# broadinstitute/delphy

Hardware: AMD Instinct MI355X
Metric: MCMC moves/sec on 100k-tip SARS-CoV-2 EMAT at 1/2/4/8 MI355X (higher is better)
Workload: dtype f64; 1 GPU; C4: synthetic 100000-tip EMAT, 29903 sites, HKY(kappa=5) + skygrid, 8092 partition parts (199999 nodes), 1000 moves/part/step, move mix 7.5/7.5/15/1/1; parts_per_gpu=8092, parts_requested=8192, max_part_nodes=-1, lds_staging=True, tickets_per_part_and_pass=4, parallelism=parts sharded over 1 GPU(s), one wavefront per part, collectives=none (one rank), emat_build_id=ea4b271524154c43

## Files before the change

### delphy_amd/csrc/emat_debug_host.hpp

```cpp
#ifndef EMAT_DEBUG_HOST_HPP_
#define EMAT_DEBUG_HOST_HPP_

namespace {

emat_status debug_settle(emat_backend* h, bool need_derived) {
  emat_status st = emat_synchronize(h); if (st) return st;
  st = sync_model_to_device(h); if (st) return st;
  st = materialize(h); if (st) return st;
  return need_derived && !h->derived_valid ? launch_recalc(h) : EMAT_OK;
}

}

extern "C" {

emat_status emat_debug_slab_layout(emat_backend* h, int32_t part_id, uint32_t* out8) {
  if (!h || !out8 || part_id < 0 || part_id >= (int)h->parts.size()) return EMAT_ERR_INVALID_ARGUMENT;
  if (!h->have_coal) return fail(h, EMAT_ERR_STATE, "no coalescent parts built");
  const PartHost& ph = h->parts[part_id];
  const int trace_cap = h->cfg.trace_moves > 0 ? h->cfg.trace_moves : 0;
  const uint32_t content = heap_content_bytes(ph.tree);
  const SlabGeo g = slab_geometry(h, ph.tree.num_nodes(), ph.tree.num_muts(), content, (int)ph.coal.k_bar_p.size(), ph.includes_run_root, ph.space_boost, ph.cell_boost);
  out8[0] = (uint32_t)sizeof(SlabHeader); out8[1] = (uint32_t)ph.tree.num_nodes() * (uint32_t)sizeof(NodeRec) + miss_dl_bytes_for((uint32_t)ph.tree.num_nodes()); out8[2] = a16((uint32_t)g.cell_cap * cell_bytes_for(ph.includes_run_root));
  out8[3] = a16((uint32_t)trace_cap * 32u); out8[4] = content; out8[5] = g.heap; out8[6] = g.scratch; out8[7] = (uint32_t)g.cell_cap;
// ... 5 lines not shown
  if (!bind_device(h)) return fail(h, EMAT_ERR_HIP, "hipSetDevice failed");
  if (n == 0) return EMAT_OK;
  DevBuf<double> da, dx, dout;
  HIP_TRY(da.upload(a, (size_t)n)); HIP_TRY(dx.upload(x_or_q, (size_t)n)); HIP_TRY(dout.upload(x_or_q, (size_t)n));
  hipLaunchKernelGGL(k_debug_gamma, dim3((unsigned)((n + 63) / 64)), dim3(64), 0, h->stream, da.p, dx.p, dout.p, n, mode);
  HIP_TRY(hipGetLastError());
  HIP_TRY(hipStreamSynchronize(h->stream));
  HIP_TRY(hipMemcpy(out, dout.p, (size_t)n * sizeof(double), hipMemcpyDeviceToHost));
  return EMAT_OK;
}
emat_status emat_debug_pop(emat_backend* h, const emat_pop_model* pm, int32_t op, int32_t n, const double* a, const double* b, double* out) {
  if (!h || !pm || n < 0 || op < 0 || op > 2 || (n > 0 && (!a || !b || !out))) return EMAT_ERR_INVALID_ARGUMENT;
  if (h->host_only) return no_device(h);
  if (!bind_device(h)) return fail(h, EMAT_ERR_HIP, "hipSetDevice failed");
  if (n == 0) return EMAT_OK;
  HostPopModel hp;
  try { hp = HostPopModel::from_c(*pm); } catch (const std::exception& ex) { return fail(h, EMAT_ERR_INVALID_ARGUMENT, ex.what()); }
  DevBuf<double> dx, dg, da, db, dout;
  HIP_TRY(dx.upload(hp.x.data(), hp.x.size())); HIP_TRY(dg.upload(hp.gamma.data(), hp.gamma.size()));
  HIP_TRY(da.upload(a, (size_t)n)); HIP_TRY(db.upload(b, (size_t)n)); HIP_TRY(dout.alloc((size_t)n));
  PopTable pt{};
  pt.kind = hp.kind; pt.skygrid_type = hp.skygrid_type; pt.skygrid_num_knots = (int)hp.x.size();
  for (int i = 0; i < 4; ++i) pt.p[i] = hp.p[i];
  pt.t_c = hp.t_c; pt.skygrid_x = dx.p; pt.skygrid_gamma = dg.p;
  pt.skygrid_inv_dx = (hp.x.size() >= 2 && hp.x.back() > hp.x.front()) ? (double)(hp.x.size() - 1) / (hp.x.back() - hp.x.front()) : 0.0;
  hipLaunchKernelGGL(k_debug_pop, dim3((unsigned)((n + 63) / 64)), dim3(64), 0, h->stream, pt, (int)op, da.p, db.p, dout.p, (int)n);
  HIP_TRY(hipGetLastError());
  HIP_TRY(hipStreamSynchronize(h->stream));
  HIP_TRY(hipMemcpy(out, dout.p, (size_t)n * sizeof(double), hipMemcpyDeviceToHost));
  return EMAT_OK;
}
emat_status emat_debug_interval_op(emat_backend* h, int32_t op, const int32_t* a, int32_t na, const int32_t* b, int32_t nb, int32_t* out, int32_t* n_out) {
  if (!h || !n_out || na < 0 || nb < 0 || (na > 0 && !a) || (nb > 0 && !b) || !out) return EMAT_ERR_INVALID_ARGUMENT;
  if (h->host_only) return no_device(h);
  if (!bind_device(h)) return fail(h, EMAT_ERR_HIP, "hipSetDevice failed");
  DevBuf<IvRec> dA, dB, dO; DevBuf<int> dn;
  HIP_TRY(dA.upload((const IvRec*)a, (size_t)na)); HIP_TRY(dB.upload((const IvRec*)b, (size_t)(op == 5 ? 0 : nb))); HIP_TRY(dO.alloc(2 * (size_t)(na + nb + 1))); HIP_TRY(dn.alloc(1));
  hipLaunchKernelGGL(k_debug_interval_op, dim3(1), dim3(64), 0, h->stream, (int)op, dA.p, (int)na, dB.p, (int)(op == 5 ? 0 : nb), op == 5 && nb > 0 ? b[0] : 0, dO.p, dn.p);
  HIP_TRY(hipGetLastError());
  HIP_TRY(hipStreamSynchronize(h->stream));
  int cnt = 0;
  HIP_TRY(hipMemcpy(&cnt, dn.p, sizeof(int), hipMemcpyDeviceToHost));
  if (cnt < 0) return fail(h, EMAT_ERR_INVALID_ARGUMENT, "emat_debug_interval_op: unknown op");
  *n_out = cnt;
  if ((op <= 3 || op == 7 || op == 8) && cnt > 0) HIP_TRY(hipMemcpy(out, dO.p, (size_t)cnt * sizeof(IvRec), hipMemcpyDeviceToHost));
  return EMAT_OK;
}
emat_status emat_debug_tree_query(emat_backend* h, int32_t part_id, int32_t op, int32_t n, const int32_t* a, const int32_t* b, int32_t* out) {
  if (!h || n < 0 || (op != 0 && op != 1) || (n > 0 && (!a || !b || !out))) return EMAT_ERR_INVALID_ARGUMENT;
  if (h->host_only) return no_device(h);
  if (!bind_device(h)) return fail(h, EMAT_ERR_HIP, "hipSetDevice failed");
  if (part_id < 0 || part_id >= (int)h->parts.size()) return EMAT_ERR_INVALID_ARGUMENT;
  const int nn = h->parts[part_id].n_nodes;
  for (int i = 0; i < n; ++i) if (a[i] < -1 || a[i] >= nn || b[i] < -1 || b[i] >= nn) return fail(h, EMAT_ERR_INVALID_ARGUMENT, "emat_debug_tree_query: node index out of range");
  if (n == 0) return EMAT_OK;
  emat_status st = debug_settle(h, false); if (st) return st;
  DevBuf<int32_t> da, db, dout;
  HIP_TRY(da.upload(a, (size_t)n)); HIP_TRY(db.upload(b, (size_t)n)); HIP_TRY(dout.alloc((size_t)n));
  KernelArgs ka = make_args(h);
  hipLaunchKernelGGL(k_debug_tree_query, dim3(1), dim3(k_wave), 0, h->stream, ka, (int)part_id, (int)op, da.p, db.p, dout.p, (int)n);
  HIP_TRY(hipGetLastError());
  HIP_TRY(hipStreamSynchronize(h->stream));
  HIP_TRY(hipMemcpy(out, dout.p, (size_t)n * sizeof(int32_t), hipMemcpyDeviceToHost));
  return EMAT_OK;
}
emat_status emat_debug_miss_dl_check(emat_backend* h, int32_t* out_2n) {
  if (!h || !out_2n) return EMAT_ERR_INVALID_ARGUMENT;
  if (h->host_only) return no_device(h);
  if (!bind_device(h)) return fail(h, EMAT_ERR_HIP, "hipSetDevice failed");
  if (h->parts.empty()) return EMAT_OK;
  emat_status st = debug_settle(h, false); if (st) return st;
  DevBuf<int32_t> dout;
  HIP_TRY(dout.alloc(2 * h->parts.size()));
  return run_over_parts(h, k_debug_miss_dl_check, dout.p, out_2n, 2 * h->parts.size(), dout.p);
}
emat_status emat_debug_graft(emat_backend* h, int32_t part_id, int32_t X, double mu_proposal, int32_t mode, int32_t new_sibling, double new_t_P,
                             double* out, int32_t out_cap, int32_t* out_len) {
  if (!h || !out || !out_len || out_cap < 2 || mode < 0 || mode > 3) return EMAT_ERR_INVALID_ARGUMENT;
  if (h->host_only) return no_device(h);
  if (!bind_device(h)) return fail(h, EMAT_ERR_HIP, "hipSetDevice failed");
  if (part_id < 0 || part_id >= (int)h->parts.size()) return EMAT_ERR_INVALID_ARGUMENT;
  const int nn = h->parts[part_id].n_nodes;
  if (X < 0 || X >= nn || (mode == 3 && (new_sibling < 0 || new_sibling >= nn))) return fail(h, EMAT_ERR_INVALID_ARGUMENT, "emat_debug_graft: node index out of range");
  emat_status st = debug_settle(h, true); if (st) return st;
  DevBuf<double> dout; DevBuf<int32_t> dlen;
  HIP_TRY(dout.alloc((size_t)out_cap)); HIP_TRY(dlen.alloc(1));
  KernelArgs ka = make_args(h);
  hipLaunchKernelGGL(k_debug_graft, dim3(1), dim3(k_wave), 0, h->stream, ka, (int)part_id, (int)X, mu_proposal, (int)mode, (int)new_sibling, new_t_P, dout.p, (int)out_cap, dlen.p);
  HIP_TRY(hipGetLastError());
  HIP_TRY(hipStreamSynchronize(h->stream));
  HIP_TRY(hipMemcpy(out_len, dlen.p, sizeof(int32_t), hipMemcpyDeviceToHost));
  HIP_TRY(hipMemcpy(out, dout.p, (size_t)std::min(*out_len, out_cap) * sizeof(double), hipMemcpyDeviceToHost));
  if (mode >= 1) h->device_wrote_slabs();
  if (out[0] != 0.0) return fail(h, EMAT_ERR_INTERNAL, "emat_debug_graft: the device code stopped with part status " + std::to_string((int)out[0]));
  return *out_len > out_cap ? fail(h, EMAT_ERR_CAPACITY, "emat_debug_graft: out_cap too small") : EMAT_OK;
}
emat_status emat_debug_sample_history(emat_backend* h, int32_t part_id, int32_t n, const int32_t* branch, const double* t_end, const uint8_t* start_seq, double T, double mu,
                                      int32_t* counts, double* muts, int32_t muts_cap, int32_t* num_muts) {
  if (!h || n < 0 || !branch || !t_end || !start_seq || !counts || !muts || muts_cap < 0 || !num_muts) return EMAT_ERR_INVALID_ARGUMENT;
  if (h->host_only) return no_device(h);
  if (!bind_device(h)) return fail(h, EMAT_ERR_HIP, "hipSetDevice failed");
  if (part_id < 0 || part_id >= (int)h->parts.size()) return EMAT_ERR_INVALID_ARGUMENT;
  const int nn = h->parts[part_id].n_nodes;
  for (int i = 0; i < n; ++i) if (branch[i] < 0 || branch[i] >= nn) return fail(h, EMAT_ERR_INVALID_ARGUMENT, "emat_debug_sample_history: node index out of range");
  emat_status st = debug_settle(h, true); if (st) return st;
  DevBuf<int32_t> db, dc, ds; DevBuf<double> dt, dm; DevBuf<uint8_t> dseq;
  HIP_TRY(db.upload(branch, (size_t)std::max(n, 1))); HIP_TRY(dt.upload(t_end, (size_t)std::max(n, 1))); HIP_TRY(dseq.upload(start_seq, (size_t)h->cfg.num_sites));
  HIP_TRY(dc.alloc((size_t)std::max(n, 1))); HIP_TRY(dm.alloc((size_t)std::max(muts_cap, 1) * 4)); HIP_TRY(ds.alloc(2));
  KernelArgs ka = make_args(h);
  hipLaunchKernelGGL(k_debug_sample_history, dim3(1), dim3(k_wave), 0, h->stream, ka, (int)part_id, (int)n, db.p, dt.p, dseq.p, T, mu, dc.p, dm.p, (int)muts_cap, ds.p);
  HIP_TRY(hipGetLastError());
  HIP_TRY(hipStreamSynchronize(h->stream));
  int32_t status[2];
  HIP_TRY(hipMemcpy(status, ds.p, sizeof status, hipMemcpyDeviceToHost));
  h->device_wrote_slabs();
  if (status[0] != 0) return fail(h, EMAT_ERR_INTERNAL, "emat_debug_sample_history: the device code stopped with part status " + std::to_string(status[0]));
  *num_muts = status[1];
  if (n > 0) HIP_TRY(hipMemcpy(counts, dc.p, (size_t)n * sizeof(int32_t), hipMemcpyDeviceToHost));
  if (status[1] > 0) HIP_TRY(hipMemcpy(muts, dm.p, (size_t)std::min(status[1], muts_cap) * 4 * sizeof(double), hipMemcpyDeviceToHost));
  return status[1] > muts_cap ? fail(h, EMAT_ERR_CAPACITY, "emat_debug_sample_history: muts_cap too small") : EMAT_OK;
}
emat_status emat_debug_edit(emat_backend* h, int32_t part_id, int32_t X, int32_t n_ops, const int32_t* op_kind, const int32_t* op_node, const double* op_t) {
  if (!h || n_ops < 0 || (n_ops > 0 && (!op_kind || !op_node || !op_t))) return EMAT_ERR_INVALID_ARGUMENT;
  if (h->host_only) return no_device(h);
  if (!bind_device(h)) return fail(h, EMAT_ERR_HIP, "hipSetDevice failed");
  if (part_id < 0 || part_id >= (int)h->parts.size()) return EMAT_ERR_INVALID_ARGUMENT;
  const int nn = h->parts[part_id].n_nodes;
  if (X < 0 || X >= nn) return fail(h, EMAT_ERR_INVALID_ARGUMENT, "emat_debug_edit: node index out of range");
  for (int i = 0; i < n_ops; ++i) if (op_kind[i] < 0 || op_kind[i] > 3 || (op_kind[i] == 3 && (op_node[i] < 0 || op_node[i] >= nn))) return fail(h, EMAT_ERR_INVALID_ARGUMENT, "emat_debug_edit: bad step");
  emat_status st = debug_settle(h, true); if (st) return st;
  DevBuf<int32_t> dk, dn, ds; DevBuf<double> dt;
  HIP_TRY(dk.upload(op_kind, (size_t)std::max(n_ops, 1))); HIP_TRY(dn.upload(op_node, (size_t)std::max(n_ops, 1))); HIP_TRY(dt.upload(op_t, (size_t)std::max(n_ops, 1))); HIP_TRY(ds.alloc(1));
  KernelArgs ka = make_args(h);
  hipLaunchKernelGGL(k_debug_edit, dim3(1), dim3(k_wave), 0, h->stream, ka, (int)part_id, (int)X, (int)n_ops, dk.p, dn.p, dt.p, ds.p);
  HIP_TRY(hipGetLastError());
  HIP_TRY(hipStreamSynchronize(h->stream));
  int32_t status = 0;
  HIP_TRY(hipMemcpy(&status, ds.p, sizeof status, hipMemcpyDeviceToHost));
  h->device_wrote_slabs();
  if (status != 0) return fail(h, EMAT_ERR_INTERNAL, "emat_debug_edit: the device code stopped with part status " + std::to_string(status));
  return EMAT_OK;
}
emat_status emat_debug_variant_counts(emat_backend* h, int32_t* out3) {
  if (!h || !out3 || h->host_only) return EMAT_ERR_INVALID_ARGUMENT;
  emat_status st = sync_model_to_device(h); if (st) return st;
  st = materialize(h); if (st) return st;
  st = pull_from_device(h); if (st) return st;
  out3[0] = out3[1] = out3[2] = 0;
  const uint32_t area = h->class_lds[h->num_classes - 1];
  const bool tables = h->num_partitions <= k_max_lds_partitions;
  for (auto& ph : h->parts) {
    const SlabHeader* H = (const SlabHeader*)(h->h_slabs.data() + ph.slab_off);
    const bool can = tables && area != 0 && H->off_nodes == (uint32_t)sizeof(SlabHeader);
    if (can && (H->heap_end <= area || H->heap_top + k_lds_heap_room <= area)) ++out3[0]; else if (can && H->heap_begin <= area) ++out3[1]; else ++out3[2];
  }
  return EMAT_OK;
}
emat_status emat_debug_arena_sites(emat_backend* h, uint64_t* out_4096) {
  if (!h || !out_4096 || h->host_only) return EMAT_ERR_INVALID_ARGUMENT;
#ifdef EMAT_PROFILE_PHASES
  HIP_TRY(hipStreamSynchronize(h->stream));
  HIP_TRY(hipMemcpyFromSymbol(out_4096, HIP_SYMBOL(::emat::g_arena_site_bytes), sizeof(unsigned long long) * 4096));
  return EMAT_OK;
#else
  return fail(h, EMAT_ERR_STATE, "built without -DEMAT_PROFILE_PHASES");
#endif
}
emat_status emat_debug_fn_ticks(emat_backend* h, uint64_t* out_12288) {
  if (!h || !out_12288 || h->host_only) return EMAT_ERR_INVALID_ARGUMENT;
#if defined(EMAT_PROFILE_PHASES) || defined(EMAT_COUNT_CALLS)
  HIP_TRY(hipStreamSynchronize(h->stream));
  std::vector<unsigned long long> z((size_t)12288 * ::emat::k_fn_replicas, 0);
  HIP_TRY(hipMemcpyFromSymbol(z.data(), HIP_SYMBOL(::emat::g_fn_ticks), sizeof(unsigned long long) * z.size()));
  for (int k = 0; k < 12288; ++k) { unsigned long long sum = 0; for (int r = 0; r < ::emat::k_fn_replicas; ++r) sum += z[(size_t)r * 12288 + k]; out_12288[k] = sum; }
  std::fill(z.begin(), z.end(), 0ull);
  HIP_TRY(hipMemcpyToSymbol(HIP_SYMBOL(::emat::g_fn_ticks), z.data(), sizeof(unsigned long long) * z.size()));
  const unsigned min_lists = h->cfg_fn_min_lists;
  HIP_TRY(hipMemcpyToSymbol(HIP_SYMBOL(::emat::g_fn_min_list_bytes), &min_lists, sizeof(min_lists)));
  return EMAT_OK;
#else
  return fail(h, EMAT_ERR_STATE, "built without -DEMAT_PROFILE_PHASES");
#endif
}
emat_status emat_debug_arena_bytes(emat_backend* h, int32_t* out_n) {
  if (!h || !out_n || h->host_only) return EMAT_ERR_INVALID_ARGUMENT;
  emat_status st = sync_model_to_device(h); if (st) return st;
  st = materialize(h); if (st) return st;
  st = pull_from_device(h); if (st) return st;
  const uint32_t area = h->class_lds[h->num_classes - 1];
  for (size_t p = 0; p < h->parts.size(); ++p) {
    const SlabHeader* H = (const SlabHeader*)(h->h_slabs.data() + h->parts[p].slab_off);
    if (h->class_of[p] != h->num_classes - 1) { out_n[p] = -1; continue; }
    const uint32_t want = (H->heap_top + k_lds_heap_room + 15u) & ~15u;
    uint32_t used;
    if (H->heap_end <= area) used = std::min(H->heap_end, want); else if (want <= area) used = want; else used = (H->heap_begin + 15u) & ~15u;
    out_n[p] = used <= area ? (int32_t)(area - ((used + 15u) & ~15u)) : 0;
  }
  return EMAT_OK;
}
emat_status emat_debug_part_ticks(emat_backend* h, int64_t* out_2n) {
  if (!h || !out_2n || h->host_only || !h->slabs_on_device) return EMAT_ERR_INVALID_ARGUMENT;
  if (!bind_device(h)) return fail(h, EMAT_ERR_HIP, "hipSetDevice failed");
  { emat_status js = wait_for_side_classes(h); if (js) return js; }
  HIP_TRY(hipStreamSynchronize(h->stream));
  HIP_TRY(hipMemcpy(out_2n, h->d_part_ticks.p, sizeof(int64_t) * 2 * h->parts.size(), hipMemcpyDeviceToHost));
  return EMAT_OK;
}
emat_status emat_debug_ticket_ticks(emat_backend* h, int64_t* out_16n) {
  if (!h || !out_16n || h->host_only || !h->slabs_on_device) return EMAT_ERR_INVALID_ARGUMENT;
  if (!bind_device(h)) return fail(h, EMAT_ERR_HIP, "hipSetDevice failed");
  { emat_status js = wait_for_side_classes(h); if (js) return js; }
  HIP_TRY(hipStreamSynchronize(h->stream));
  HIP_TRY(hipMemcpy(out_16n, h->d_part_ticks.p + 2 * h->parts.size(), sizeof(int64_t) * 2 * k_ticket_log * h->parts.size(), hipMemcpyDeviceToHost));
  return EMAT_OK;
}
emat_status emat_debug_phase_ticks(emat_backend* h, int32_t part_id, int64_t* out16) {
  if (!h || !out16 || part_id < 0 || part_id >= (int)h->parts.size()) return EMAT_ERR_INVALID_ARGUMENT;
  emat_status st = pull_from_device(h); if (st) return st;
  const SlabHeader* H = (const SlabHeader*)(h->h_slabs.data() + h->parts[part_id].slab_off);
#ifdef EMAT_PROFILE_PHASES
  for (int i = 0; i < 16; ++i) out16[i] = H->phase_ticks[i];
  if (h->cfg_phase_extra) for (int i = 0; i < 16; ++i) out16[i] = ((const int64_t*)H->reserved)[i];
#else
  (void)H; for (int i = 0; i < 16; ++i) out16[i] = 0;
#endif
  return EMAT_OK;
}

}

#endif
```

### delphy_amd/csrc/emat_device_core.hpp

```cpp
#ifndef EMAT_DEV_NS
#error "define EMAT_DEV_NS and EMAT_VARIANT_LDS before including the device headers"
#endif

#include <hip/hip_runtime.h>
#include <cfloat>
#include <cstdint>

#include "emat_slab.hpp"
#include "emat_reform_pure.hpp"
#include "emat_rng_pos.hpp"
#include "emat_gamma_pure.hpp"

#ifndef EMAT_DEVICE_COMMON_ONCE_
#define EMAT_DEVICE_COMMON_ONCE_
namespace emat {
extern __shared__ __attribute__((aligned(16))) uint8_t emat_lds[];
constexpr uint32_t k_lds_tables_bytes = k_max_lds_partitions * (1 + 4 + 16) * 8;
constexpr uint32_t k_lds_ctx_bytes = 288;
#ifndef EMAT_RNG_BLOCKS
#define EMAT_RNG_BLOCKS 32
#endif
constexpr uint32_t k_rng_blocks = EMAT_RNG_BLOCKS;
static_assert(k_rng_blocks == 0 || (k_rng_blocks <= 64 && (k_rng_blocks & (k_rng_blocks - 1)) == 0), "one block per lane, a power of two");
constexpr uint32_t k_lds_rng_bytes = k_rng_blocks * 16;
constexpr uint32_t k_lds_static_bytes = k_lds_tables_bytes + k_lds_ctx_bytes + k_lds_rng_bytes + k_max_lds_partitions * 16 * 8;
__shared__ __attribute__((aligned(16))) uint8_t emat_lds_tables[k_lds_tables_bytes];
__shared__ __attribute__((aligned(16))) uint8_t emat_lds_ctx[k_lds_ctx_bytes];
__shared__ __attribute__((aligned(16))) uint32_t emat_lds_rng[k_rng_blocks ? k_rng_blocks * 4 : 4];
constexpr uint32_t k_lds_logq_bytes = k_max_lds_partitions * 16 * 8;
__shared__ __attribute__((aligned(16))) double emat_lds_logq[k_max_lds_partitions * 16];
__shared__ __attribute__((aligned(16))) uint8_t emat_lds_hdr[sizeof(SlabHeader)];
constexpr uint32_t k_lds_dyn_base = k_lds_tables_bytes + k_lds_ctx_bytes + (k_rng_blocks ? k_rng_blocks * 16 : 16) + k_lds_logq_bytes + (uint32_t)sizeof(SlabHeader);
}
#if defined(EMAT_PROFILE_PHASES) || defined(EMAT_COUNT_CALLS)
#define EMAT_DYN_LDS ::emat::emat_lds
#else
#define EMAT_DYN_LDS ((uint8_t*)(__attribute__((address_space(3))) uint8_t*)(uintptr_t)::emat::k_lds_dyn_base)
#endif
#define EMAT_D static __device__ inline
#define EMAT_DN static __device__ __noinline__
#define EMAT_DF static __device__ __forceinline__
#define EMAT_NOTAIL __attribute__((disable_tail_calls))
#ifdef EMAT_COUNT_CALLS
#define EMAT_CALLED(file_id) do { if (threadIdx.x == 0) atomicAdd(&::emat::g_fn_ticks[(blockIdx.x & 63) * (3 * 2048) + (file_id) * 2048 + (__LINE__ & 2047)][1], 1ull); } while (0)
#endif
#endif

namespace emat {
namespace EMAT_DEV_NS {

constexpr double k_neg_dbl_max = -1.7976931348623157e308;
constexpr double k_inf = __builtin_huge_val();
constexpr int k_no_node = -1;

#ifndef EMAT_CONST_AS
#define EMAT_CONST_AS __attribute__((address_space(4)))
#endif
template <class T> EMAT_DF const EMAT_CONST_AS T* uniform_const_ptr(const T* p) {
  const uint64_t a = (uint64_t)p;
  const uint32_t lo = __builtin_amdgcn_readfirstlane((uint32_t)a), hi = __builtin_amdgcn_readfirstlane((uint32_t)(a >> 32));
  return (const EMAT_CONST_AS T*)(((uint64_t)hi << 32) | lo);
}

EMAT_DF uint32_t uniform_u32(uint32_t v) { return __builtin_amdgcn_readfirstlane(v); }
EMAT_DF bool uniform_flag(bool b) { return __builtin_amdgcn_ballot_w64(b) != 0ull; }

struct Ctx {
  uint8_t* S;
  uint8_t* G;
  SlabHeader* H;
  NodeRec* N;
  int L;
  uint32_t heap_limit;
  const __attribute__((address_space(1))) uint8_t* ref;
  const __attribute__((address_space(1))) uint8_t* part;
  const __attribute__((address_space(1))) double* nu;
  const __attribute__((address_space(1))) double* cumQ;
  const double* mu;
  const double* pi;
  const double* q;
  const PopTable* pop;
  double t_max_tip;
  bool only_displacing_inner_nodes;
  bool topology_moves_enabled;
  bool includes_run_root;
  bool uniform_sites;
  bool have_logq;
  uint8_t phase, svc;
  uint64_t rng_key;
  uint32_t rng_pos;
  uint32_t mv_rng_pos;
  uint64_t rng_base;
  uint64_t rng_spare;
  uint8_t* frame;
  double mu_prop;
  uint8_t* A;
  uint32_t a_top, a_end;
  uint32_t sc_top;
  bool failed;
  int64_t bytes;
  int64_t bytes_w;
  double tr_log_mh; int32_t tr_node; int16_t tr_kind, tr_acc;
  int64_t moves_left;
  double mix_total;
  const double* sh_ktw; const double* sh_tsop; const int32_t* sh_nact;
};

static_assert(sizeof(Ctx) + 16 <= k_lds_ctx_bytes, "context outgrew its LDS slot (the last 16 bytes are the kernel's flag word)");
#if EMAT_VARIANT_LDS
EMAT_DF uint8_t* slab_at(const Ctx&, uint32_t off) { return EMAT_DYN_LDS + (off - (uint32_t)sizeof(SlabHeader)); }
EMAT_DF SlabHeader* hdr_of(const Ctx&) { return (SlabHeader*)emat_lds_hdr; }
EMAT_DF NodeRec* nodes_of(const Ctx&) { return (NodeRec*)EMAT_DYN_LDS; }
EMAT_DF const double* mu_of(const Ctx&) { return (const double*)emat_lds_tables; }
EMAT_DF const double* pi_of(const Ctx&) { return (const double*)emat_lds_tables + k_max_lds_partitions; }
EMAT_DF const double* q_of(const Ctx&) { return (const double*)emat_lds_tables + k_max_lds_partitions * 5; }
#if EMAT_VARIANT_LDS == 2
EMAT_DF uint8_t* heap_at(const Ctx& c, uint32_t off) { return c.G + off; }
#else
EMAT_DF uint8_t* heap_at(const Ctx& c, uint32_t off) { return slab_at(c, off); }
#endif
#else
EMAT_DF uint8_t* heap_at(const Ctx& c, uint32_t off) { return c.S + off; }
EMAT_DF uint8_t* slab_at(const Ctx& c, uint32_t off) { return c.S + off; }
EMAT_DF SlabHeader* hdr_of(const Ctx& c) { return c.H; }
EMAT_DF NodeRec* nodes_of(const Ctx& c) { return c.N; }
EMAT_DF const double* mu_of(const Ctx& c) { return c.mu; }
EMAT_DF const double* pi_of(const Ctx& c) { return c.pi; }
EMAT_DF const double* q_of(const Ctx& c) { return c.q; }
#endif

EMAT_D void fail_at(Ctx& c, int status, int line) {
  if (!c.failed) { c.failed = true; if (hdr_of(c)->status == 0) { hdr_of(c)->status = status; hdr_of(c)->fail_line = line; } }
}
#ifndef EMAT_FAIL
#define EMAT_FAIL(c, st) fail_at((c), (st), __LINE__)
#define EMAT_CHECK(c, cond) do { if (!(cond)) fail_at((c), ::emat::k_part_internal, __LINE__); } while (0)
#ifdef EMAT_PROFILE_PHASES
#define EMAT_SITE(line, hbm, v) atomicAdd(&::emat::g_arena_site_bytes[(line) & 2047][(hbm) ? 1 : 0], (unsigned long long)(v))
#define EMAT_COUNT(c, k, v) (((int64_t*)hdr_of(c)->reserved)[k] += (int64_t)(v))
#define EMAT_PHASE_BEGIN() long long _ph_t0 = clock64()
#define EMAT_PHASE(c, k) do { long long _t = clock64(); hdr_of(c)->phase_ticks[k] += _t - _ph_t0; _ph_t0 = _t; } while (0)
#define EMAT_TIMED(file_id) ::emat::FnTimer _fn_timer((file_id) * 2048 + (__LINE__ & 2047))
#define EMAT_TIMED_BLOCK(file_id, name) ::emat::FnTimer name((file_id) * 2048 + (__LINE__ & 2047))
#define EMAT_TIMED_END(name) name.stop()
#else
#define EMAT_TIMED(file_id) do {} while (0)
#define EMAT_TIMED_BLOCK(file_id, name) do {} while (0)
#define EMAT_TIMED_END(name) do {} while (0)
#define EMAT_SITE(line, hbm, v) do {} while (0)
#define EMAT_COUNT(c, k, v) do {} while (0)
#define EMAT_PHASE_BEGIN() do {} while (0)
#define EMAT_PHASE(c, k) do {} while (0)
#endif
#endif

EMAT_DN double m_log(double x) { return ::log(x); }
EMAT_DN double m_exp(double x) { return ::exp(x); }
EMAT_DN double m_log1p(double x) { return ::log1p(x); }
EMAT_DN double m_expm1(double x) { return ::expm1(x); }
EMAT_D void philox4x32_10(uint64_t ctr, uint64_t key, uint32_t out[4]) {
  uint32_t c0 = (uint32_t)ctr, c1 = (uint32_t)(ctr >> 32), c2 = 0, c3 = 0;
  uint32_t k0 = (uint32_t)key, k1 = (uint32_t)(key >> 32);
#pragma unroll
  for (int r = 0; r < 10; ++r) {
    const uint32_t M0 = 0xD2511F53u, M1 = 0xCD9E8D57u;
    uint32_t hi0 = __umulhi(M0, c0), lo0 = M0 * c0;
    uint32_t hi1 = __umulhi(M1, c2), lo1 = M1 * c2;
    uint32_t n0 = hi1 ^ c1 ^ k0, n1 = lo1, n2 = hi0 ^ c3 ^ k1, n3 = lo0;
    c0 = n0; c1 = n1; c2 = n2; c3 = n3;
    k0 += 0x9E3779B9u; k1 += 0xBB67AE85u;
  }
  out[0] = c0; out[1] = c1; out[2] = c2; out[3] = c3;
}
constexpr uint32_t k_rng_fold_at = 1u << 30;
EMAT_DN uint64_t rng_next64_computed(Ctx& c) {
  const RngPos at = rng_pos_folded(c.rng_base, c.rng_pos, k_rng_blocks, k_rng_fold_at);
  if (at.pos != c.rng_pos) c.rng_base = at.base;
  c.rng_pos = at.pos + 1u;
  if (at.pos & 1u) return c.rng_spare;
  uint32_t w[4];
  philox4x32_10(rng_pos_block(at.base, at.pos), c.rng_key, w);
  c.rng_spare = (uint64_t)w[2] | ((uint64_t)w[3] << 32);
  return (uint64_t)w[0] | ((uint64_t)w[1] << 32);
}
EMAT_DF uint64_t rng_buffer_word(uint32_t i) { return ((const uint64_t*)emat_lds_rng)[i]; }
EMAT_D uint64_t rng_next64(Ctx& c) {
  const uint32_t pos = c.rng_pos;
  if (rng_pos_in_buffer(pos, k_rng_blocks)) { c.rng_pos = pos + 1u; return rng_buffer_word(pos); }
  return rng_next64_computed(c);
}
EMAT_D void rng_fill(Ctx& c, int lane) {
  if (k_rng_blocks == 0) return;
  const uint32_t pos = c.rng_pos;
  const RngPos to = rng_pos_after_fill(c.rng_base, pos);
  if (lane == 0 && (pos & 1u) == 0 && rng_pos_in_buffer(rng_pos_spare_word(pos), k_rng_blocks)) c.rng_spare = rng_buffer_word(rng_pos_spare_word(pos));
  if (lane < (int)k_rng_blocks) { uint32_t w[4]; philox4x32_10(to.base + (uint64_t)lane, c.rng_key, w); *(uint4*)&emat_lds_rng[(uint32_t)lane * 4u] = make_uint4(w[0], w[1], w[2], w[3]); }
  if (lane == 0) { c.rng_base = to.base; c.rng_pos = to.pos; }
}
#ifndef EMAT_RNG_MARGIN
#define EMAT_RNG_MARGIN 8
#endif
EMAT_D bool rng_wants_fill(const Ctx& c) { return rng_pos_wants_fill(c.rng_pos, k_rng_blocks, (uint32_t)EMAT_RNG_MARGIN); }
EMAT_D void rng_rewind_to_move_start(Ctx& c) {
  const uint32_t pos = c.mv_rng_pos;
  c.rng_pos = pos;
  if ((pos & 1u) != 0 && !rng_pos_in_buffer(pos, k_rng_blocks)) { uint32_t w[4]; philox4x32_10(rng_pos_block(c.rng_base, pos), c.rng_key, w); c.rng_spare = (uint64_t)w[2] | ((uint64_t)w[3] << 32); }
}
EMAT_D void rng_enter_leg(Ctx& c, const SlabHeader& h) {
  const RngPos at = rng_pos_enter(h.rng_counter, h.rng_has_spare, k_rng_blocks);
  c.rng_key = h.rng_key; c.rng_base = at.base; c.rng_pos = at.pos; c.mv_rng_pos = at.pos; c.rng_spare = h.rng_spare;
}
EMAT_D void rng_leave_leg(const Ctx& c, SlabHeader& h) {
  const uint32_t pos = c.rng_pos, sw = rng_pos_spare_word(pos);
  h.rng_counter = rng_pos_counter(c.rng_base, pos); h.rng_has_spare = rng_pos_has_spare(pos);
  h.rng_spare = rng_pos_in_buffer(sw, k_rng_blocks) ? rng_buffer_word(sw) : c.rng_spare;
}
using ::emat::to_co; using ::emat::to_oo; using ::emat::to_oc;
EMAT_D double u01_co(Ctx& c) { return to_co(rng_next64(c)); }
EMAT_D double u01_oo(Ctx& c) { return to_oo(rng_next64(c)); }
EMAT_D double u01_oc(Ctx& c) { return to_oc(rng_next64(c)); }
EMAT_D double uniform_co(Ctx& c, double lo, double hi) { return lo + (hi - lo) * u01_co(c); }
EMAT_D double uniform_oc(Ctx& c, double lo, double hi) { return lo + (hi - lo) * u01_oc(c); }
EMAT_D int uniform_int(Ctx& c, int n) { return (int)__umul64hi(rng_next64(c), (uint64_t)n); }
EMAT_D double gaussian(Ctx& c, double mean, double sigma) {
  uint64_t a = rng_next64(c), b = rng_next64(c);
  double u1 = to_oc(a), u2 = to_co(b);
  double r = sqrt(-2.0 * m_log(u1));
  return mean + sigma * (r * cos(6.283185307179586476925 * u2));
}
EMAT_D double exponential(Ctx& c, double rate) { return -m_log(u01_oc(c)) / rate; }
EMAT_D int poisson(Ctx& c, double lambda) {
  double u = u01_co(c);
  double p = m_exp(-lambda), F = p;
  int k = 0;
  while (u >= F && k < 100000) { ++k; p *= lambda / k; F += p; }
  return k;
}

struct ByteCount { int all = 0, written = 0; };
EMAT_DF void count_bytes(Ctx& c, const ByteCount& n) { c.bytes += n.all; if (n.written != 0) c.bytes_w += n.written; }

template <class T> struct SVec { T* p; int n; int cap; };
struct ScMark { uint32_t a, g; };
EMAT_D ScMark sc_mark(const Ctx& c) { ScMark m; m.a = c.a_top; m.g = c.sc_top; return m; }
EMAT_D void sc_release(Ctx& c, ScMark m) { c.a_top = m.a; c.sc_top = m.g; }
EMAT_D void sc_reset(Ctx& c) { c.a_top = 0; c.sc_top = hdr_of(c)->scratch_begin; }
EMAT_D bool sc_in_lds(const Ctx& c, const void* p) { return c.A != nullptr && (const uint8_t*)p >= c.A && (const uint8_t*)p < c.A + c.a_end; }
EMAT_D uint8_t* sc_alloc(Ctx& c, uint32_t bytes, int line = __builtin_LINE()) {
  uint32_t b = (bytes + 15u) & ~15u;
  if (c.a_top + b <= c.a_end) { uint8_t* p = c.A + c.a_top; c.a_top += b; EMAT_COUNT(c, 9, b); EMAT_SITE(line, 0, b); return p; }
  if (c.sc_top + b > hdr_of(c)->scratch_end) { EMAT_FAIL(c, k_part_overflow); return c.G + hdr_of(c)->scratch_begin; }
  EMAT_COUNT(c, 8, b); EMAT_SITE(line, 1, b);
  uint8_t* p = c.G + c.sc_top;
  c.sc_top += b;
  return p;
}
template <class T> EMAT_D SVec<T> sc_vec(Ctx& c, int cap, int line = __builtin_LINE()) {
  SVec<T> v; v.n = 0;
  uint32_t bytes = (uint32_t)cap * (uint32_t)sizeof(T);
  uint32_t b = (bytes + 15u) & ~15u;
  if (cap >= 0 && c.a_top + b <= c.a_end) { v.p = (T*)(c.A + c.a_top); v.cap = cap; c.a_top += b; EMAT_COUNT(c, 9, b); EMAT_SITE(line, 0, b); return v; }
  if (cap < 0 || c.sc_top + b > hdr_of(c)->scratch_end) { EMAT_FAIL(c, k_part_overflow); v.p = (T*)(c.G + hdr_of(c)->scratch_begin); v.cap = 0; return v; }
  EMAT_COUNT(c, 8, b); EMAT_SITE(line, 1, b);
  v.p = (T*)(c.G + c.sc_top); v.cap = cap; c.sc_top += b;
  return v;
}
template <class T> EMAT_DF void push(Ctx& c, SVec<T>& v, const T& x, int line = __builtin_LINE()) { if (v.n < v.cap) v.p[v.n++] = x; else fail_at(c, k_part_overflow, line); }
template <class T> EMAT_D SVec<T> sc_open(Ctx& c, int max_elems, int min_lds_elems) {
  SVec<T> v; v.n = 0;
  uint32_t a0 = (c.a_top + 15u) & ~15u;
  int room_a = c.a_end > a0 ? (int)((c.a_end - a0) / sizeof(T)) : 0;
  if (room_a >= min_lds_elems) { v.p = (T*)(c.A + a0); v.cap = room_a < max_elems ? room_a : max_elems; c.a_top = c.a_end; return v; }
  uint32_t g0 = (c.sc_top + 15u) & ~15u;
  int room_g = hdr_of(c)->scratch_end > g0 ? (int)((hdr_of(c)->scratch_end - g0) / sizeof(T)) : 0;
  v.p = (T*)(c.G + g0); v.cap = room_g < max_elems ? room_g : max_elems; c.sc_top = hdr_of(c)->scratch_end;
  if (v.cap <= 0) { v.cap = 0; EMAT_FAIL(c, k_part_overflow); }
  return v;
}
template <class T> EMAT_DF bool sc_open_migrate(Ctx& c, SVec<T>& v, int max_elems) {
  if (!sc_in_lds(c, v.p)) return false;
  uint32_t g0 = (c.sc_top + 15u) & ~15u;
  int room_g = hdr_of(c)->scratch_end > g0 ? (int)((hdr_of(c)->scratch_end - g0) / sizeof(T)) : 0;
// ... 771 lines not shown
```

### delphy_amd/csrc/emat_device_moves.hpp

```cpp

#include "emat_device_spr.hpp"

namespace emat {
namespace EMAT_DEV_NS {

#ifndef EMAT_HOT_BYTES
#define EMAT_HOT_BYTES 1536
#endif
enum { k_inner_node_displace = 0, k_tip_displace = 1, k_branch_reform = 2, k_subtree_slide = 3, k_spr1 = 4 };

EMAT_D void trace_nothing(Ctx& c, int kind) { c.tr_node = -1; c.tr_kind = (int16_t)kind; c.tr_acc = -1; }
EMAT_D void begin_move(Ctx& c, int kind) { hdr_of(c)->proposed[kind]++; trace_nothing(c, kind); }
EMAT_D void note_move(Ctx& c, double log_mh, bool acc, int kind) { c.tr_log_mh = log_mh; c.tr_acc = acc ? 1 : 0; if (acc) hdr_of(c)->accepted[kind]++; }
EMAT_D bool mh_accept(Ctx& c, double log_mh) { return log_mh >= 0.0 || uniform_co(c, 0.0, 1.0) < m_exp(log_mh); }

EMAT_DF double bounded_exponential(Ctx& c, double lambda, double a, double b) {
  double u = u01_oo(c);
  double ltr = lambda * (b - a);
  double x;
  if (lambda == 0.0) x = a + u * (b - a);
  else if (lambda > 0 && ltr > 100) x = b + m_log(u) / lambda;
  else if (lambda < 0 && ltr < -100) x = a + m_log(u) / lambda;
  else x = a + m_log1p(u * (m_exp(ltr) - 1)) / lambda;
  return x < a ? a : (b < x ? b : x);
}
EMAT_DF int pick_random_node(Ctx& c) { return uniform_int(c, hdr_of(c)->n_nodes); }

struct CoreFrame {
  int X, new_branch, P, old_S;
  double new_t, alpha_ratio, old_t_P, d_prior, log_mh;
  Graft old_graft, new_graft;
};
#ifndef EMAT_CF
#define EMAT_CF(c) (*(CoreFrame*)(c).frame)
#endif
EMAT_NOTAIL EMAT_DN void spr_move_core(Ctx& c, int X, int new_branch, double new_t, double alpha_ratio) { EMAT_TIMED(2);
  if (X == hdr_of(c)->root) return;
  if (!c.includes_run_root) if (nodes_of(c)[X].parent == hdr_of(c)->root || new_branch == hdr_of(c)->root) return;
  {
    const double t_X = nodes_of(c)[X].t;
    const int P = nodes_of(c)[X].parent;
    const double new_t_P = new_t;
    if (new_t_P == t_X || new_t_P == nodes_of(c)[new_branch].t || (P != hdr_of(c)->root && new_t_P == nodes_of(c)[nodes_of(c)[P].parent].t)) return;
    if (coal_needs_cells(c, new_t_P)) { stop_for_cells(c, c.tr_kind); return; }
    CoreFrame* f = (CoreFrame*)sc_alloc(c, (uint32_t)sizeof(CoreFrame));
    if (c.failed) return;
    c.frame = (uint8_t*)f;
    f->X = X; f->new_branch = new_branch; f->P = P; f->old_S = sibling_of(c, P, X);
    f->new_t = new_t; f->alpha_ratio = alpha_ratio; f->old_t_P = nodes_of(c)[P].t;
  }
  c.mu_prop = nodes_of(c)[hdr_of(c)->root].lambda / (c.L - nodes_of(c)[hdr_of(c)->root].n_missing);
  EMAT_PHASE_BEGIN();
  analyze_graft(c, EMAT_CF(c).X, EMAT_CF(c).old_graft);
  peel_graft(c, EMAT_CF(c).old_graft);
  EMAT_PHASE(c, 0);
  spr_move_topology(c, EMAT_CF(c).X, EMAT_CF(c).new_branch, EMAT_CF(c).new_t);
  EMAT_PHASE(c, 1);
  propose_new_graft(c, EMAT_CF(c).X, EMAT_CF(c).new_graft);
  EMAT_PHASE(c, 2);
  if (c.failed) return;
  EMAT_CF(c).d_prior = coal_delta_displace_coalescence(c, EMAT_CF(c).old_t_P, EMAT_CF(c).new_t);
  {
    const CoreFrame& f = EMAT_CF(c);
    EMAT_CF(c).log_mh = (f.new_graft.delta_log_G - f.new_graft.log_alpha_mut) - (f.old_graft.delta_log_G - f.old_graft.log_alpha_mut) + m_log(f.alpha_ratio) + f.d_prior;
  }
  if (c.failed) return;
  const bool acc = mh_accept(c, EMAT_CF(c).log_mh);
  if (c.tr_kind == k_subtree_slide) note_move(c, EMAT_CF(c).log_mh, acc, k_subtree_slide);
  if (acc) {
    apply_graft(c, EMAT_CF(c).new_graft);
    hdr_of(c)->log_G -= EMAT_CF(c).old_graft.delta_log_G; hdr_of(c)->log_G += EMAT_CF(c).new_graft.delta_log_G;
    hdr_of(c)->log_aug_prior += EMAT_CF(c).d_prior;
    coal_coalescence_displaced(c, EMAT_CF(c).old_t_P, EMAT_CF(c).new_t);
  } else {
    spr_move_topology(c, EMAT_CF(c).X, EMAT_CF(c).old_S, EMAT_CF(c).old_t_P);
    apply_graft(c, EMAT_CF(c).old_graft);
  }
  EMAT_PHASE(c, 4);
}

template <bool kRoot> EMAT_DF void inner_node_displace_body(Ctx& c, ByteCount& n) {
  begin_move(c, k_inner_node_displace);
  int node;
  { EMAT_TIMED(2);
    int guard = 0; do { node = pick_random_node(c); } while (is_tip(c, node) && guard++ < (1 << 26)); }
  c.tr_node = node;
  const int root = hdr_of(c)->root;
  if (!kRoot && node == root) return;
  const NodeRec nd = nodes_of(c)[node];
  double t_min = -k_inf;
  if (!kRoot || node != root) {
    t_min = nodes_of(c)[nd.parent].t;
    const MutRec* m = muts_of(c, node);
    for (int i = 0; i < (int)nd.muts.cnt; ++i) t_min = t_min > m[i].t ? t_min : m[i].t;
  }
  double t_max = k_inf;
  const int ch[2] = {nd.child0, nd.child1};
  const double lambda_at_node = nd.lambda;
  double d_logG_dt = 0.0;
  if (!kRoot || node != root) d_logG_dt += -lambda_at_node;
  for (int k = 0; k < 2; ++k) {
    const int cc = ch[k];
    t_max = t_max < nodes_of(c)[cc].t ? t_max : nodes_of(c)[cc].t;
    const MutRec* m = muts_of(c, cc);
    const int nm = nmuts(c, cc);
    for (int i = 0; i < nm; ++i) t_max = t_max < m[i].t ? t_max : m[i].t;
    n.all += 64 + 16 * nm + 24 * (int)nodes_of(c)[cc].miss.cnt;
  }
  { EMAT_TIMED(2);
  for (int k = 0; k < 2; ++k) {
    double lambda_just_below = lambda_at_node + delta_lambda_across_node_missations(c, ch[k]);
    d_logG_dt -= -lambda_just_below;
  } }
  n.all += 2 * 64 + 16 * (int)nd.muts.cnt;
  const double old_t = nd.t;
  double log_alpha_ratio = 0.0, new_t = old_t;
  if (kRoot && node == root) {
    double tree_span = c.t_max_tip - t_max;
    EMAT_CHECK(c, tree_span >= 0.0);
    double ds = (1 / nd.lambda) / 2;
    double delta_scale;
    if (tree_span < ds) delta_scale = tree_span; else delta_scale = ds;
    new_t = old_t + gaussian(c, 0.0, delta_scale);
    if (new_t < t_min || new_t > t_max) return;
    log_alpha_ratio = 0.0;
  } else {
    EMAT_TIMED(2);
    new_t = bounded_exponential(c, d_logG_dt, t_min, t_max);
    log_alpha_ratio = d_logG_dt * (new_t - old_t);
  }
  if (new_t == t_min || new_t == t_max) return;
  if (kRoot) { if (coal_needs_cells(c, new_t)) { stop_for_cells(c, k_inner_node_displace); return; } }
  double delta_log_G = d_logG_dt * (new_t - old_t);
  double delta_log_prior = coal_delta_displace_coalescence<kRoot>(c, old_t, new_t, n);
  if (c.failed) return;
  double log_mh = delta_log_G + delta_log_prior - log_alpha_ratio;
  bool acc;
  { EMAT_TIMED(2);
  acc = mh_accept(c, log_mh);
  note_move(c, log_mh, acc, k_inner_node_displace); }
  if (acc) {
    EMAT_TIMED(2);
    coal_coalescence_displaced<kRoot>(c, old_t, new_t, n);
    nodes_of(c)[node].t = new_t;
    hdr_of(c)->log_G += d_logG_dt * (new_t - old_t);
    hdr_of(c)->log_aug_prior += delta_log_prior;
  }
}
template <bool kRoot> EMAT_NOTAIL EMAT_DN void inner_node_displace_move(Ctx& c) { EMAT_TIMED(2); ByteCount n; inner_node_displace_body<kRoot>(c, n); count_bytes(c, n); }

template <bool kRoot> EMAT_DF void tip_displace_body(Ctx& c, ByteCount& n) {
  begin_move(c, k_tip_displace);
  int node;
  { int guard = 0; do { node = pick_random_node(c); } while (!is_tip(c, node) && guard++ < (1 << 26)); }
  c.tr_node = node;
  const NodeRec nd = nodes_of(c)[node];
  if (nd.t_min == nd.t_max) return;
  double t_min;
  if ((double)nd.t_min < nodes_of(c)[nd.parent].t) t_min = nodes_of(c)[nd.parent].t; else t_min = (double)nd.t_min;
  const MutRec* m = muts_of(c, node);
  for (int i = 0; i < (int)nd.muts.cnt; ++i) t_min = t_min > m[i].t ? t_min : m[i].t;
  const double t_max = (double)nd.t_max;
  const double d_logG_dt = -nd.lambda;
  const double old_t = nd.t;
  n.all += 2 * 64 + 16 * (int)nd.muts.cnt;
  double new_t = bounded_exponential(c, d_logG_dt, t_min, t_max);
  double log_alpha_ratio = d_logG_dt * (new_t - old_t);
  if (new_t == t_min || new_t == t_max) return;
  double delta_log_G = d_logG_dt * (new_t - old_t);
  double delta_log_prior = coal_delta_displace_tip<kRoot>(c, old_t, new_t, n);
  if (c.failed) return;
  double log_mh = delta_log_G + delta_log_prior - log_alpha_ratio;
  bool acc = mh_accept(c, log_mh);
  note_move(c, log_mh, acc, k_tip_displace);
  if (acc) {
    coal_tip_displaced<kRoot>(c, old_t, new_t, n);
    nodes_of(c)[node].t = new_t;
    hdr_of(c)->log_G += d_logG_dt * (new_t - old_t);
    hdr_of(c)->log_aug_prior += delta_log_prior;
  }
}
template <bool kRoot> EMAT_NOTAIL EMAT_DN void tip_displace_move(Ctx& c) { EMAT_TIMED(2); ByteCount n; tip_displace_body<kRoot>(c, n); count_bytes(c, n); }

EMAT_DF SVec<MutRec> randomize_branch_mutation_times(Ctx& c, int X) { EMAT_TIMED(2);
  const int n = nmuts(c, X);
  SVec<MutRec> out = sc_vec<MutRec>(c, n);
  if (c.failed) return out;
  const MutRec* old = muts_of(c, X);
  if (X == hdr_of(c)->root) { for (int i = 0; i < n; ++i) push(c, out, old[i]); return out; }
  const double t_X = nodes_of(c)[X].t, t_P = nodes_of(c)[nodes_of(c)[X].parent].t;
  bool complicated = false;
  for (int i = 0; i < n && !complicated; ++i) for (int j = i + 1; j < n; ++j) if (old[i].site == old[j].site) { complicated = true; break; }
  if (!complicated) {
    for (int i = 0; i < n; ++i) { MutRec r = make_mut(old[i].from, old[i].site, old[i].to, uniform_oc(c, t_P, t_X)); r.pad = (uint16_t)i; push(c, out, r); }
  } else {
    int prev_site = -1;
    while (true) {
      int l = 0x7fffffff;
      for (int i = 0; i < n; ++i) if (old[i].site > prev_site && old[i].site < l) l = old[i].site;
      if (l == 0x7fffffff) break;
      prev_site = l;
      int first = out.n, k = 0;
      for (int i = 0; i < n; ++i) if (old[i].site == l) { MutRec r = make_mut(old[i].from, old[i].site, old[i].to, uniform_oc(c, t_P, t_X)); r.pad = (uint16_t)i; push(c, out, r); ++k; }
      for (int a = first + 1; a < first + k && a < out.n; ++a) { double x = out.p[a].t; int b = a - 1; while (b >= first && out.p[b].t > x) { out.p[b + 1].t = out.p[b].t; --b; } out.p[b + 1].t = x; }
    }
  }
  sort_muts(out.p, out.n);
  return out;
}

struct ReformFactors { double* A; double* B; };
EMAT_DF bool mut_factors(const Ctx& c, int pa, double nu, int from, int to, double& A, double& B) {
  const double mn = mu_of(c)[pa] * nu;
  const double* q = q_of(c) + pa * 16;
  A = mn * (-q[from * 5] - -q[to * 5]);
  if (c.have_logq && nu == 1.0) { B = emat_lds_logq[pa * 16 + from * 4 + to]; return false; }
// ... 54 lines not shown
  hdr_of(c)->log_G += delta_log_G;
  return 16 * N;
}
#ifndef EMAT_REFORM_SMALL_MAX
#define EMAT_REFORM_SMALL_MAX 4
#endif
template <bool kRoot> EMAT_DF void branch_reform_body(Ctx& c, ByteCount& n_bytes) {
  begin_move(c, k_branch_reform);
  if (hdr_of(c)->n_nodes < 3) return;
  const int X = pick_random_node(c);
  c.tr_node = X;
  if (X == hdr_of(c)->root) return;
  const int P = nodes_of(c)[X].parent;
  const int S = sibling_of(c, P, X);
  const double t_X = nodes_of(c)[X].t, t_P = nodes_of(c)[P].t;
  if (kRoot) { if (P == hdr_of(c)->root) { spr_move_core(c, X, S, t_P, 1.0); if (c.failed) return; } }
  const double lam = nodes_of(c)[X].lambda;
  const int n = nmuts(c, X);
  if (n == 0) {
    const double g = -lam * (t_X - t_P), delta_log_G = g - g;
    n_bytes.all += 2 * 64;
    const bool acc = mh_accept(c, delta_log_G);
    note_move(c, delta_log_G, acc, k_branch_reform);
    if (acc) hdr_of(c)->log_G += delta_log_G;
    return;
  }
  if (n <= EMAT_REFORM_SMALL_MAX) {
    int stored = -1;
    switch (n) {
#if EMAT_REFORM_SMALL_MAX >= 1
      case 1: stored = branch_reform_small<1>(c, X, lam, t_X, t_P); break;
#endif
#if EMAT_REFORM_SMALL_MAX >= 2
      case 2: stored = branch_reform_small<2>(c, X, lam, t_X, t_P); break;
#endif
#if EMAT_REFORM_SMALL_MAX >= 3
      case 3: stored = branch_reform_small<3>(c, X, lam, t_X, t_P); break;
#endif
#if EMAT_REFORM_SMALL_MAX >= 4
      case 4: stored = branch_reform_small<4>(c, X, lam, t_X, t_P); break;
#endif
      default: break;
    }
    if (stored >= 0) { n_bytes.all += 2 * 64 + 2 * 16 * n + stored; n_bytes.written += stored; return; }
  }
  const ReformFactors f = reform_factors(c, muts_of(c, X), n);
  SVec<MutRec> nm = randomize_branch_mutation_times(c, X);
  if (c.failed) return;
  double g_new = -lam * (t_X - t_P), g_old = g_new;
  { const MutRec* m = nm.p; for (int i = nm.n - 1; i >= 0; --i) { const int j = (int)m[i].pad; g_new -= f.A[j] * (m[i].t - t_P); g_new += f.B[j]; } }
  { const MutRec* m = muts_of(c, X); for (int i = n - 1; i >= 0; --i) { g_old -= f.A[i] * (m[i].t - t_P); g_old += f.B[i]; } }
  const double delta_log_G = g_new - g_old;
  n_bytes.all += 2 * 64 + 2 * 16 * nm.n;
  double log_mh = delta_log_G;
  bool acc = mh_accept(c, log_mh);
  note_move(c, log_mh, acc, k_branch_reform);
  if (acc) {
    for (int i = 0; i < nm.n; ++i) nm.p[i].pad = 0;
    list_assign<MutRec>(c, nodes_of(c)[X].muts, nm.p, nm.n); hdr_of(c)->log_G += delta_log_G; n_bytes.all += 16 * nm.n; n_bytes.written += 16 * nm.n;
  }
}
template <bool kRoot> EMAT_NOTAIL EMAT_DN void branch_reform_move(Ctx& c) { EMAT_TIMED(2); ByteCount n; branch_reform_body<kRoot>(c, n); count_bytes(c, n); }

EMAT_DN SVec<int> enumerate_descendant_branches_straddling(Ctx& c, int P, double t, int X) {
  SVec<int> out; out.n = 0;
  ScSpan span = sc_span(c, 512);
  out.p = (int*)span.lo; out.cap = 0;
  int* stack_base = (int*)span.hi;
  int sp = 0;
  auto room = [&](int er, int es) -> bool {
    if (span.lo + (size_t)(out.n + er) * 4 + 16 <= span.hi - (size_t)(sp + es) * 4) return true;
    if (!span.lds) return false;
    ScSpan big = sc_span_hbm(c);
    if (big.lo + (size_t)(out.n + er) * 4 + 16 > big.hi - (size_t)(sp + es) * 4) return false;
    int* no = (int*)big.lo; int* nb = (int*)big.hi;
    for (int i = 0; i < out.n; ++i) no[i] = out.p[i];
    for (int i = 1; i <= sp; ++i) nb[-i] = stack_base[-i];
    span = big; out.p = no; stack_base = nb;
    return true;
  };
  if (!room(0, 1)) { EMAT_FAIL(c, k_part_overflow); return out; }
  stack_base[-(++sp)] = P;
  while (sp > 0 && !c.failed) {
    int n = stack_base[-sp]; --sp;
    if (n == X) continue;
    if (t <= nodes_of(c)[n].t) { if (!room(1, 0)) { EMAT_FAIL(c, k_part_overflow); break; } out.p[out.n++] = n; }
    else if (!is_tip(c, n)) {
      if (!room(0, 2)) { EMAT_FAIL(c, k_part_overflow); break; }
      stack_base[-(++sp)] = nodes_of(c)[n].child1;
      stack_base[-(++sp)] = nodes_of(c)[n].child0;
    }
  }
  out.cap = out.n;
  sc_span_commit(c, span, (uint32_t)out.n * 4u);
  return out;
}

EMAT_NOTAIL EMAT_DN void subtree_slide_move(Ctx& c) { EMAT_TIMED(2);
  begin_move(c, k_subtree_slide);
  if (hdr_of(c)->n_nodes < 2) return;
  const int X = pick_random_node(c);
  c.tr_node = X;
  const int root = hdr_of(c)->root;
  if (X == root) return;
  const int P = nodes_of(c)[X].parent, S = sibling_of(c, P, X);
  double t_early = (P == root) ? (nodes_of(c)[X].t < nodes_of(c)[S].t ? nodes_of(c)[X].t : nodes_of(c)[S].t) : nodes_of(c)[root].t;
  if (P == root) { if (nodes_of(c)[S].t < nodes_of(c)[X].t) t_early = nodes_of(c)[S].t; else t_early = nodes_of(c)[X].t; }
  double tree_span = c.t_max_tip - t_early;
  EMAT_CHECK(c, tree_span >= 0.0);
  double ds = (1 / nodes_of(c)[X].lambda) / 2;
  double delta_scale = tree_span < ds ? tree_span : ds;
  double delta_t = gaussian(c, 0.0, delta_scale);
  const double old_P_t = nodes_of(c)[P].t, new_P_t = old_P_t + delta_t;
  if (delta_t < 0.0) {
    if (P != root && new_P_t < nodes_of(c)[nodes_of(c)[P].parent].t) {
      int GG = nodes_of(c)[P].parent, SS = P;
      while (new_P_t < nodes_of(c)[GG].t) { SS = GG; GG = nodes_of(c)[GG].parent; if (GG == k_no_node) break; }
      SVec<int> branches = enumerate_descendant_branches_straddling(c, SS, old_P_t, X);
      if (c.failed) return;
      double a_o2n = 1.0, a_n2o = 1.0 / (double)branches.n;
      spr_move_core(c, X, SS, new_P_t, a_n2o / a_o2n);
    } else spr_move_core(c, X, S, new_P_t, 1.0);
  } else {
    if (new_P_t > nodes_of(c)[X].t) return;
    if (new_P_t > nodes_of(c)[S].t) {
      SVec<int> branches = enumerate_descendant_branches_straddling(c, P, new_P_t, X);
      if (c.failed) return;
      if (branches.n == 0) return;
      int bi = uniform_int(c, branches.n);
      int SS = branches.p[bi];
      double a_o2n = 1.0 / (double)branches.n, a_n2o = 1.0;
      spr_move_core(c, X, SS, new_P_t, a_n2o / a_o2n);
    } else spr_move_core(c, X, S, new_P_t, 1.0);
  }
}

EMAT_D void spr1_park(Ctx& c, int phase) { c.phase = (uint8_t)phase; c.svc = 1; }
EMAT_NOTAIL EMAT_DN void spr1_move_begin(Ctx& c) { EMAT_TIMED(2);
  begin_move(c, k_spr1);
  c.phase = 0;
  if (hdr_of(c)->n_nodes < 2) return;
  const double chooser = uniform_co(c, 0.0, 1.0);
  const int limit = chooser < 0.01 ? 0x7fffffff : 1;
  const int root0 = hdr_of(c)->root;
  c.mu_prop = nodes_of(c)[root0].lambda / (c.L - nodes_of(c)[root0].n_missing);
  int X;
  { int guard = 0; do { X = pick_random_node(c); } while (hdr_of(c)->root == X && guard++ < (1 << 26)); }
  c.tr_node = X;
  if (nodes_of(c)[X].lambda == 0.0) return;
  const int P = nodes_of(c)[X].parent;
  const bool pruning_changes_root = P == hdr_of(c)->root;
  if (pruning_changes_root && !c.includes_run_root) return;
  EMAT_PHASE_BEGIN();
  Spr1Frame* frp = (Spr1Frame*)sc_alloc(c, (uint32_t)sizeof(Spr1Frame));
  if (c.failed) return;
  Spr1Frame& fr = *frp;
  c.frame = (uint8_t*)frp;
  fr.X = X; fr.t_X = nodes_of(c)[X].t; fr.P = P; fr.old_t_P = nodes_of(c)[P].t; fr.old_S = sibling_of(c, P, X); fr.old_G = nodes_of(c)[P].parent;
  fr.limit = limit; fr.f = 0.8 ; fr.t_max_tip = c.t_max_tip; fr.can_change_root = c.includes_run_root;
  {
    const uint32_t a0 = (c.a_top + 15u) & ~15u, free_b = c.a_end > a0 ? c.a_end - a0 : 0u;
    uint32_t hot_b = EMAT_HOT_BYTES;
    if (free_b / 2 > hot_b) hot_b = (free_b / 2 < 32768u ? free_b / 2 : 32768u) & ~15u;
    fr.hot = (limit == 1) ? sc_reserve_hot(c, hot_b) : HotBlock{nullptr, 0};
  }
  analyze_graft(c, X, fr.old_graft);
  peel_graft(c, fr.old_graft);
  EMAT_PHASE(c, 5);
  if (c.failed) return;
  fr.old_min_muts = count_min_mutations(c, fr.old_graft);
  int extra = 4;
  if (limit != 1) { extra = 8; for (int n = 0; n < hdr_of(c)->n_nodes; ++n) if (c.includes_run_root || n != hdr_of(c)->root) extra += nmuts(c, n); }
  fr.extra = extra;
  fr.deltas = summarize_closed_mutations(c, fr.old_graft, extra);
  fr.missing_at_X = reconstruct_missing_sites_at(c, X);
  fr.n_missing_at_X = iv_num_sites(fr.missing_at_X.p, fr.missing_at_X.n);
  fr.lambda_X = nodes_of(c)[X].lambda;
  fr.init_branch = fr.old_S;
  if (c.failed) return;
  spr1_park(c, 1);
}
EMAT_NOTAIL EMAT_DN void spr1_move_propose(Ctx& c) { EMAT_TIMED(2);
  Spr1Frame& fr = *(Spr1Frame*)c.frame;
  c.phase = 0;
  if (c.failed) return;
  EMAT_PHASE_BEGIN();
  const Study& pre = fr.study;
  const int X = fr.X, P = fr.P;
  int new_region; double new_t_P;
  { EMAT_TIMED(2);
  new_region = study_pick_nexus_region(c, pre);
  new_t_P = study_pick_time_in_region(c, pre, new_region);
  fr.log_alpha_o2n = study_log_alpha_in_region(c, pre, new_region, new_t_P); }
  const int new_S = pre.regions.p[new_region].branch;
  EMAT_CHECK(c, new_S != P);
  fr.pre_new_region_min_muts = pre.regions.p[new_region].min_muts;
  fr.new_S = new_S; fr.new_t_P = new_t_P;
  const double t_new_S = nodes_of(c)[new_S].t;
  int new_G = nodes_of(c)[new_S].parent;
  if (new_G == P) new_G = fr.old_G;
  const double t_new_G = (new_G == k_no_node) ? k_neg_dbl_max : nodes_of(c)[new_G].t;
  if (c.failed) return;
  EMAT_PHASE(c, 7);
  if (new_t_P == fr.t_X || new_t_P == t_new_S || new_t_P == t_new_G) { apply_graft(c, fr.old_graft); return; }
  if (coal_needs_cells(c, new_t_P)) { apply_graft(c, fr.old_graft); if (!c.failed) stop_for_cells(c, k_spr1); return; }
  spr_move_topology(c, X, new_S, new_t_P);
  EMAT_PHASE(c, 8);
  propose_new_graft(c, X, fr.new_graft);
  EMAT_PHASE(c, 9);
  if (c.failed) return;
  EMAT_CHECK(c, nodes_of(c)[X].parent == P);
  fr.new_min_muts = count_min_mutations(c, fr.new_graft);
  fr.deltas = summarize_closed_mutations(c, fr.new_graft, fr.extra);
  fr.init_branch = new_S;
  if (c.failed) return;
  spr1_park(c, 2);
}
EMAT_NOTAIL EMAT_DN void spr1_move_finish(Ctx& c) { EMAT_TIMED(2);
  Spr1Frame& fr = *(Spr1Frame*)c.frame;
  c.phase = 0;
  if (c.failed) return;
  EMAT_PHASE_BEGIN();
  const Study& post = fr.study;
  const int X = fr.X;
  const int old_region = study_find_region(post, fr.old_S, fr.old_t_P);
  EMAT_CHECK(c, old_region != -1);
  if (c.failed) return;
  const double log_alpha_n2o = study_log_alpha_in_region(c, post, old_region, fr.old_t_P);
  EMAT_CHECK(c, fr.new_min_muts == fr.pre_new_region_min_muts);
  EMAT_CHECK(c, fr.old_min_muts == post.regions.p[old_region].min_muts);
  EMAT_PHASE(c, 11);
  const double d_prior = coal_delta_displace_coalescence(c, fr.old_t_P, fr.new_t_P);
  if (c.failed) return;
  const double log_mh = (fr.new_graft.delta_log_G - fr.new_graft.log_alpha_mut) - (fr.old_graft.delta_log_G - fr.old_graft.log_alpha_mut)
      + log_alpha_n2o - fr.log_alpha_o2n + d_prior;
  const bool acc = mh_accept(c, log_mh);
  note_move(c, log_mh, acc, k_spr1);
  if (acc) {
    apply_graft(c, fr.new_graft);
    hdr_of(c)->log_G -= fr.old_graft.delta_log_G; hdr_of(c)->log_G += fr.new_graft.delta_log_G;
    hdr_of(c)->log_aug_prior += d_prior;
    coal_coalescence_displaced(c, fr.old_t_P, fr.new_t_P);
  } else {
    EMAT_TIMED(2);
    spr_move_topology(c, X, fr.old_S, fr.old_t_P);
    apply_graft(c, fr.old_graft);
  }
  EMAT_PHASE(c, 12);
}

EMAT_DN bool compact_heap(Ctx& c) {
  uint32_t live = 0;
  const int n = hdr_of(c)->n_nodes;
  for (int i = 0; i < n; ++i) {
    live += (((uint32_t)nodes_of(c)[i].muts.cnt * 16u) + 15u) & ~15u;
    live += (((uint32_t)nodes_of(c)[i].miss.cnt * 8u) + 15u) & ~15u;
    live += (((uint32_t)nodes_of(c)[i].mfs.cnt * 8u) + 15u) & ~15u;
  }
  if (live > hdr_of(c)->scratch_end - hdr_of(c)->scratch_begin) return false;
  uint8_t* stage = c.G + hdr_of(c)->scratch_begin;
  uint32_t w = 0;
  for (int i = 0; i < n; ++i) {
    ListRef* refs[3] = {&nodes_of(c)[i].muts, &nodes_of(c)[i].miss, &nodes_of(c)[i].mfs};
    const uint32_t es[3] = {16u, 8u, 8u};
    for (int k = 0; k < 3; ++k) {
      uint32_t bytes = (uint32_t)refs[k]->cnt * es[k];
      const uint64_t* src = (const uint64_t*)heap_at(c, refs[k]->off); uint64_t* dst = (uint64_t*)(stage + w);
      for (uint32_t q = 0; q < bytes / 8; ++q) dst[q] = src[q];
      w += (bytes + 15u) & ~15u;
    }
  }
  uint32_t top = hdr_of(c)->heap_begin, r = 0;
  for (int i = 0; i < n; ++i) {
    ListRef* refs[3] = {&nodes_of(c)[i].muts, &nodes_of(c)[i].miss, &nodes_of(c)[i].mfs};
    const uint32_t es[3] = {16u, 8u, 8u};
    for (int k = 0; k < 3; ++k) {
      uint32_t bytes = (uint32_t)refs[k]->cnt * es[k], padded = (bytes + 15u) & ~15u;
      const uint64_t* src = (const uint64_t*)(stage + r); uint64_t* dst = (uint64_t*)heap_at(c, top);
      for (uint32_t q = 0; q < bytes / 8; ++q) dst[q] = src[q];
      refs[k]->off = top; refs[k]->cap = list_cap_for(padded, es[k]);
      top += padded; r += padded;
    }
  }
  hdr_of(c)->heap_top = top;
  return true;
}

EMAT_D uint32_t heap_reserve(const Ctx& c) {
  const uint32_t heap_size = hdr_of(c)->heap_end - hdr_of(c)->heap_begin;
  uint32_t reserve = heap_size / 4 > 1024u ? heap_size / 4 : 1024u;
  if (reserve > heap_size / 2) reserve = heap_size / 2;
  return reserve;
}
EMAT_D void begin_leg(Ctx& c) {
  c.heap_limit = hdr_of(c)->heap_end - heap_reserve(c);
  double total_weight = 15.0 + 15.0;
  if (c.topology_moves_enabled) total_weight += 1.0 + 1.0;
  c.mix_total = total_weight;
}
EMAT_DN bool make_heap_room(Ctx& c) {
  const uint32_t reserve = heap_reserve(c), free_b = hdr_of(c)->heap_end - hdr_of(c)->heap_top;
  if (free_b < reserve) {
    if (!compact_heap(c) || hdr_of(c)->heap_end - hdr_of(c)->heap_top < reserve) { if (hdr_of(c)->status == 0) hdr_of(c)->status = k_part_need_space; return false; }
  }
  return true;
}

template <bool kRoot> EMAT_NOTAIL EMAT_D bool mcmc_sub_iteration(Ctx& c) {
#ifdef EMAT_PROFILE_PHASES
  const long long _mv0 = clock64();
#endif
  const uint32_t phase = uniform_u32(c.phase);
  if (phase == 1) spr1_move_propose(c);
  else if (phase == 2) spr1_move_finish(c);
  else {
  if (uniform_flag(hdr_of(c)->heap_top > c.heap_limit)) { if (!uniform_flag(make_heap_room(c))) return false; }
  sc_reset(c);
  if (kRoot) c.mv_rng_pos = c.rng_pos;
  if (c.only_displacing_inner_nodes) inner_node_displace_move<kRoot>(c);
  else {
    double r = uniform_co(c, 0.0, c.mix_total);
    if (r < 7.5) inner_node_displace_move<kRoot>(c);
    else if (r < 15.0) tip_displace_move<kRoot>(c);
    else if (r < 30.0) branch_reform_move<kRoot>(c);
    else if (c.topology_moves_enabled) { if (r < 31.0) subtree_slide_move(c); else spr1_move_begin(c); }
    else trace_nothing(c, -1);
  }
  }
#ifdef EMAT_PROFILE_PHASES
  { const long long _dt = clock64() - _mv0; hdr_of(c)->phase_ticks[(c.tr_kind >= 3) ? 15 : 14] += _dt; if (c.tr_kind == 0) EMAT_COUNT(c, 10, _dt); else if (c.tr_kind == 1) EMAT_COUNT(c, 15, _dt); }
#endif
  if (uniform_u32(c.svc) != 0 && !uniform_flag(c.failed)) return true;
  c.phase = 0; c.svc = 0;
  if (uniform_flag(hdr_of(c)->status == k_part_need_cells)) return false;
  if (uniform_flag(hdr_of(c)->trace_len < hdr_of(c)->trace_cap)) {
    double* tr = (double*)slab_at(c, hdr_of(c)->off_trace) + 4 * hdr_of(c)->trace_len;
    const bool noted = c.tr_acc >= 0;
    tr[0] = (double)c.tr_kind; tr[1] = (double)c.tr_node; tr[2] = noted ? (double)c.tr_acc : 0.0; tr[3] = noted ? c.tr_log_mh : __builtin_nan("");
    hdr_of(c)->trace_len++;
  }
  hdr_of(c)->moves_done++;
  return !uniform_flag(c.failed);
}

template <bool kRoot> EMAT_NOTAIL EMAT_DN void run_chain(Ctx& c) {
  c.svc = 0;
  for (;;) {
    if (uniform_u32(c.phase) == 0) {
      if (uniform_flag(c.moves_left <= 0)) return;
      if (uniform_flag(rng_wants_fill(c))) { c.svc = 2; return; }
      c.moves_left -= 1;
    }
    if (!uniform_flag(mcmc_sub_iteration<kRoot>(c))) { c.moves_left = 0; c.phase = 0; c.svc = 0; return; }
    if (uniform_u32(c.svc) != 0) return;
  }
}
EMAT_DF void run_chain_loop(Ctx& c) { if (c.includes_run_root) run_chain<true>(c); else run_chain<false>(c); }

EMAT_DN double calc_log_root_prior(Ctx& c, const int32_t* ref_freqs, int P) {
  const int root = hdr_of(c)->root;
  double result = 0.0;
  for (int p = 0; p < P; ++p) {
    for (int a = 0; a < 4; ++a) {
      int f = ref_freqs[p * 4 + a];
      const MutRec* m = muts_of(c, root);
      for (int i = 0; i < nmuts(c, root); ++i) if (site_part(c, m[i].site) == p) { if (m[i].from == a) --f; if (m[i].to == a) ++f; }
      const IvRec* iv = miss_of(c, root);
      for (int i = 0; i < (int)nodes_of(c)[root].miss.cnt; ++i) for (int l = iv[i].start; l < iv[i].end; ++l) if (site_part(c, l) == p && (int)c.ref[l] == a) --f;
      const FsRec* fs = mfs_of(c, root);
      for (int i = 0; i < (int)nodes_of(c)[root].mfs.cnt; ++i) if (site_part(c, fs[i].site) == p) { if ((int)c.ref[fs[i].site] == a) ++f; if ((int)fs[i].state == a) --f; }
      double pa = pi_of(c)[p * 4 + a];
      if (pa != 0.0) result += f * m_log(pa);
      else if (f != 0) return -k_inf;
    }
  }
  return result;
// ... 5 lines not shown
```

### delphy_amd/csrc/emat_device_spr.hpp

```cpp

#include "emat_device_core.hpp"

namespace emat {
namespace EMAT_DEV_NS {

EMAT_DN SVec<FsRec> fsv_set_v(Ctx& c, SVec<FsRec> v, int l, int from) {
  int k = fs_lower_bound(v.p, v.n, l);
  bool present = (k < v.n && v.p[k].site == l);
  if (from != (int)c.ref[l]) {
    if (present) { v.p[k].state = (uint8_t)from; return v; }
    if (v.n >= v.cap) { EMAT_FAIL(c, k_part_overflow); return v; }
    for (int i = v.n; i > k; --i) v.p[i] = v.p[i - 1];
    v.p[k].site = l; v.p[k].state = (uint8_t)from; v.p[k].pad[0] = v.p[k].pad[1] = v.p[k].pad[2] = 0; v.n++;
  } else if (present) { for (int i = k; i + 1 < v.n; ++i) v.p[i] = v.p[i + 1]; v.n--; }
  return v;
}
EMAT_DF void fsv_set(Ctx& c, SVec<FsRec>& v, int l, int from) { v = fsv_set_v(c, v, l, from); }

EMAT_DN void set_root_muts_from_deltas(Ctx& c, int root, const SVec<SdRec> d) { EMAT_TIMED(1);
  ListRef& r = nodes_of(c)[root].muts;
  list_reserve<MutRec>(c, r, d.n);
  if (c.failed) return;
  MutRec* m = list_ptr<MutRec>(c, r);
  for (int i = 0; i < d.n; ++i) { EMAT_CHECK(c, c.ref[d.p[i].site] == d.p[i].from); m[i] = make_mut(d.p[i].from, d.p[i].site, d.p[i].to, k_neg_dbl_max); }
// ... 267 lines not shown
  edit_end(c, e);
  sc_release(c, mark);
}

EMAT_D int choose_different_state(Ctx& c, int s) { int delta = 1 + uniform_int(c, 3); return (s + delta) % 4; }

struct KTruncPoisson { double lambda; int min_k; double normalization, term_before_min_k, max_k; };
EMAT_DF KTruncPoisson ktp_make(double lambda, int min_k) {
  KTruncPoisson d; d.lambda = lambda; d.min_k = min_k; d.normalization = 0.0; d.term_before_min_k = 0.0; d.max_k = 0.0;
  if ((double)min_k <= lambda) return d;
  d.max_k = (10.0 * min_k > 10.0 * lambda) ? 10.0 * min_k : 10.0 * lambda;
  double last_term = 1.0, em1 = m_expm1(lambda);
  d.normalization = em1;
  for (int k = 1; k < min_k; ++k) { last_term *= lambda / k; d.normalization -= last_term; }
  d.term_before_min_k = last_term;
  if (d.normalization <= 0.0 || fabs(d.normalization) < 1e-10 * em1) {
    d.normalization = 0.0;
    double nlt = last_term;
    for (int k = min_k; k < d.max_k; ++k) { nlt *= lambda / k; d.normalization += nlt; }
  }
  return d;
}
EMAT_DF int ktp_sample_s(Ctx& c, double lambda, int min_k, double normalization, double term_before_min_k, double max_k) {
  KTruncPoisson d; d.lambda = lambda; d.min_k = min_k; d.normalization = normalization; d.term_before_min_k = term_before_min_k; d.max_k = max_k;
  if (d.normalization == 0.0) { int guard = 0; while (guard++ < (1 << 26)) { int k = poisson(c, d.lambda); if (k >= d.min_k) return k; } return d.min_k; }
  double u = uniform_co(c, 0.0, d.normalization);
  double cum = 0.0; int k = d.min_k; double term = d.term_before_min_k;
  while (k < d.max_k) { term *= d.lambda / k; cum += term; if (cum > u) break; ++k; }
  return k;
}
EMAT_DF int ktp_sample(Ctx& c, const KTruncPoisson& d) { return ktp_sample_s(c, d.lambda, d.min_k, d.normalization, d.term_before_min_k, d.max_k); }

constexpr int k_open_max = 1 << 20;
EMAT_DF bool open_room(Ctx& c, SVec<MutRec>& out, int extra) {
  if (out.cap - out.n >= extra) return true;
  if (sc_open_migrate(c, out, k_open_max) && out.cap - out.n >= extra) return true;
  EMAT_FAIL(c, k_part_overflow); return false;
}
EMAT_DF SVec<MutRec> sample_site_trajectory_v(Ctx& c, SVec<MutRec> out, int l, int from, int to, double d_lambda, int d_min_k, double d_normalization, double d_term_before_min_k, double d_max_k,
                                              double T, bool accept_only_if_match) {
  int n = 0; int s = from;
  int guard = 0;
  while (guard++ < (1 << 26)) { EMAT_TIMED(1);
    { EMAT_TIMED(1);
    n = ktp_sample_s(c, d_lambda, d_min_k, d_normalization, d_term_before_min_k, d_max_k); }
    if (!open_room(c, out, n)) return out;
    MutRec* rec = out.p + out.n;
    s = from;
    for (int i = 0; i < n; ++i) { s = choose_different_state(c, s); rec[i].to = (uint8_t)s; }
    if (s == to) break;
    if (!accept_only_if_match) return out;
  }
  MutRec* rec = out.p + out.n;
  EMAT_TIMED(1);
  for (int i = 0; i < n; ++i) rec[i].t = uniform_co(c, -T, 0.0);
  for (int i = 1; i < n; ++i) { double x = rec[i].t; int j = i - 1; while (j >= 0 && rec[j].t > x) { rec[j + 1].t = rec[j].t; --j; } rec[j + 1].t = x; }
  int prev = from;
  for (int i = 0; i < n; ++i) { const int st = rec[i].to; rec[i] = make_mut((uint8_t)prev, l, (uint8_t)st, rec[i].t); prev = st; }
  out.n += n;
  return out;
}
EMAT_DF void sample_site_trajectory(Ctx& c, SVec<MutRec>& out, int l, int from, int to, const KTruncPoisson& dist, double T, bool accept_only_if_match, bool& accepted) {
  const SVec<MutRec> r = sample_site_trajectory_v(c, out, l, from, to, dist.lambda, dist.min_k, dist.normalization, dist.term_before_min_k, dist.max_k, T, accept_only_if_match);
  accepted = r.n > out.n;
  out = r;
}
EMAT_DF SVec<MutRec> sample_mutational_history(Ctx& c, int L, double T, double mu, const SVec<SdRec>& deltas) { EMAT_TIMED(1);
  const double twice = 0.5 * (double)L * (mu * T) * (mu * T);
  const int want = 2 * deltas.n + 8 + (twice < 1e6 ? (int)(3.0 * twice + 6.0 * sqrt(3.0 * twice)) : (1 << 20));
  SVec<MutRec> out = sc_open<MutRec>(c, k_open_max, want);
  if (c.failed) return out;
  if (deltas.n != 0) { EMAT_TIMED(1);
    KTruncPoisson ge1 = ktp_make(mu * T, 1);
    for (int i = 0; i < deltas.n && !c.failed; ++i) { EMAT_TIMED(1);
      bool acc; sample_site_trajectory(c, out, deltas.p[i].site, deltas.p[i].from, deltas.p[i].to, ge1, T, true, acc); }
  }
  double muT = mu * T;
  int l = 0;
  if ((double)L * muT * muT < 2e-6) l = L;
  double log_one_minus_p_tricky = 0.0;
  if (l < L) { const double p_0 = m_exp(-muT), p_1 = muT * p_0; log_one_minus_p_tricky = (muT < 1e-4) ? -0.5 * muT * muT : -muT - m_log1p(-p_1); }
  int guard = 0;
  EMAT_TIMED_BLOCK(1, skip_timer);
  while (l < L && !c.failed && guard++ < (1 << 26)) {
    double u = exponential(c, -log_one_minus_p_tricky);
    if (!(u >= 0 && u < (double)L)) break;
    l += (int)floor(u);
    if (l >= L) break;
    if (sd_contains(deltas, l)) { ++l; continue; }
    KTruncPoisson ge2 = ktp_make(mu * T, 2);
    bool acc = false;
    sample_site_trajectory(c, out, l, 0, 0, ge2, T, false, acc);
    if (acc) ++l;
  }
  EMAT_TIMED_END(skip_timer);
  sort_muts(out.p, out.n);
  sc_trim(c, out);
  return out;
}
EMAT_DN SVec<MutRec> sample_unconstrained_mutational_history(Ctx& c, int L, double T, double mu) { EMAT_TIMED(1);
  const double expect = mu * (double)L * T;
  const int want = expect < 1e6 ? (int)(expect + 6.0 * sqrt(expect)) + 8 : (1 << 20);
  SVec<MutRec> out = sc_open<MutRec>(c, k_open_max, want);
  if (c.failed) return out;
  double t = 0.0;
  int guard = 0;
  while (!c.failed && guard++ < (1 << 26)) {
    t -= exponential(c, mu * (double)L);
    if (t <= -T) break;
    int l = uniform_int(c, L);
    int s = 0;
    for (int i = out.n - 1; i >= 0; --i) if (out.p[i].site == l) { s = out.p[i].from; break; }
    int ns = choose_different_state(c, s);
    if (out.n == out.cap && !sc_open_migrate(c, out, k_open_max)) { EMAT_FAIL(c, k_part_overflow); break; }
    push(c, out, make_mut((uint8_t)ns, l, (uint8_t)s, t));
  }
  for (int i = 0, j = out.n - 1; i < j; ++i, --j) { MutRec tmp = out.p[i]; out.p[i] = out.p[j]; out.p[j] = tmp; }
  sc_trim(c, out);
  return out;
}
EMAT_DF void adjust_mutational_history(Ctx& c, const SVec<MutRec> h, const SVec<SdRec> deltas, int end_branch, double end_t) { EMAT_TIMED(1);
  for (int i = h.n - 1; i >= 0; --i) {
    MutRec& m = h.p[i];
    m.t += end_t;
    if (!sd_contains(deltas, m.site)) {
      int end_state = calc_site_state_at(c, end_branch, end_t, m.site);
      int delta = end_state;
      m.from = (uint8_t)((m.from + delta) % 4);
      m.to = (uint8_t)((m.to + delta) % 4);
    }
  }
}

struct BranchInfo {
  int A, B; bool is_open; double T_to_X, pl_A, pl_X;
  SVec<IvRec> warm, hot;
  SVec<MutRec> hot_muts;
  SVec<SdRec> hot_deltas;
};
struct Graft { int X, S; double t_P; BranchInfo* bi; int nbi; double delta_log_G, log_alpha_mut; bool rooty; };
enum { k_PX = 0, k_PS = 1, k_SPX = 2 };

EMAT_D void bi_init(BranchInfo& b) { b.A = b.B = k_no_node; b.is_open = false; b.T_to_X = b.pl_A = b.pl_X = 0.0; b.warm.p = nullptr; b.warm.n = b.warm.cap = 0; b.hot = b.warm; b.hot_muts.p = nullptr; b.hot_muts.n = b.hot_muts.cap = 0; b.hot_deltas.p = nullptr; b.hot_deltas.n = b.hot_deltas.cap = 0; }
EMAT_D double log_alpha_mut_term(double mu_p, int L, double T, int M, bool is_open, int d) {
  const double a3 = mu_p / 3;
  double r = -mu_p * L * T + ((M != 0 || !(a3 > 0.0 && a3 < k_inf)) ? M * m_log(a3) : (a3 < 1.0 ? -0.0 : 0.0));
  if (!is_open) {
    double P_AC = -0.25 * m_expm1(-4. / 3. * mu_p * T);
    r -= (L - d) * m_log1p(-3 * P_AC) + ((d != 0 || !(P_AC > 0.0 && P_AC < 1.0)) ? d * m_log(P_AC) : -0.0);
  }
  return r;
}

EMAT_DN void start_rooty_graft_analysis(Ctx& c, int X, Graft& g) { EMAT_TIMED(1);
  g.X = X; g.rooty = true; g.delta_log_G = g.log_alpha_mut = 0.0;
  const int P = nodes_of(c)[X].parent, S = sibling_of(c, P, X);
  const double t_X = nodes_of(c)[X].t, t_P = nodes_of(c)[P].t, t_S = nodes_of(c)[S].t;
  g.S = S; g.t_P = t_P;
  EMAT_CHECK(c, P == hdr_of(c)->root && c.includes_run_root);
  g.bi = (BranchInfo*)sc_alloc(c, 3 * sizeof(BranchInfo)); g.nbi = 3;
  if (c.failed) { g.nbi = 0; return; }
  for (int i = 0; i < 3; ++i) bi_init(g.bi[i]);
  const MutRec* mX = muts_of(c, X); const int nX = nmuts(c, X);
  const MutRec* mS = muts_of(c, S); const int nS = nmuts(c, S);
  BranchInfo& PX = g.bi[k_PX];
  PX.A = P; PX.B = X; PX.is_open = true; PX.T_to_X = t_X - t_P;
  PX.pl_A = -1 * delta_lambda_across_node_missations(c, S);
  PX.warm = iv_copy_sc(c, miss_of(c, S), (int)nodes_of(c)[S].miss.cnt); PX.hot = PX.warm;
  PX.pl_X = PX.pl_A;
  PX.hot_muts = sc_vec<MutRec>(c, nX);
  for (int i = 0; i < nX; ++i) if (iv_contains(PX.hot.p, PX.hot.n, mX[i].site)) { push(c, PX.hot_muts, mX[i]); PX.pl_X += dq(c, mX[i].site, mX[i].from, mX[i].to); }
  BranchInfo& PS = g.bi[k_PS];
  PS.A = P; PS.B = S; PS.is_open = true; PS.T_to_X = t_S - t_P;
  PS.pl_A = -1 * delta_lambda_across_node_missations(c, X);
  PS.warm = iv_copy_sc(c, miss_of(c, X), (int)nodes_of(c)[X].miss.cnt); PS.hot = PS.warm;
  PS.pl_X = PS.pl_A;
  PS.hot_muts = sc_vec<MutRec>(c, nS);
  for (int i = 0; i < nS; ++i) if (iv_contains(PS.hot.p, PS.hot.n, mS[i].site)) { push(c, PS.hot_muts, mS[i]); PS.pl_X += dq(c, mS[i].site, mS[i].from, mS[i].to); }
  BranchInfo& SPX = g.bi[k_SPX];
  SPX.A = S; SPX.B = P; SPX.is_open = false; SPX.T_to_X = (t_S - t_P) + (t_X - t_P);
  SPX.pl_X = nodes_of(c)[X].lambda - PX.pl_X;
  SPX.pl_A = nodes_of(c)[S].lambda - PS.pl_X;
  {
    IvRec all; all.start = 0; all.end = c.L;
    SVec<IvRec> s1 = iv_subtract_sc(c, &all, 1, miss_of(c, P), (int)nodes_of(c)[P].miss.cnt);
    SVec<IvRec> s2 = iv_subtract_sc(c, s1.p, s1.n, miss_of(c, X), (int)nodes_of(c)[X].miss.cnt);
    SVec<IvRec> s3 = iv_subtract_sc(c, s2.p, s2.n, miss_of(c, S), (int)nodes_of(c)[S].miss.cnt);
    SPX.warm = s3; SPX.hot = s3;
  }
  SPX.hot_muts = sc_vec<MutRec>(c, nS + nX);
  SPX.hot_deltas = sc_vec<SdRec>(c, nS + nX);
  for (int i = nS - 1; i >= 0; --i) if (iv_contains(SPX.hot.p, SPX.hot.n, mS[i].site)) {
    MutRec rm = make_mut(mS[i].to, mS[i].site, mS[i].from, t_P - (mS[i].t - t_P));
    push(c, SPX.hot_muts, rm); sd_push_back(c, SPX.hot_deltas, rm.site, rm.from, rm.to);
  }
  for (int i = 0; i < nX; ++i) if (iv_contains(SPX.hot.p, SPX.hot.n, mX[i].site)) { push(c, SPX.hot_muts, mX[i]); sd_push_back(c, SPX.hot_deltas, mX[i].site, mX[i].from, mX[i].to); }
  c.bytes += 3 * 64 + 16 * (nX + nS) + 24 * ((int)nodes_of(c)[X].miss.cnt + (int)nodes_of(c)[S].miss.cnt + (int)nodes_of(c)[P].miss.cnt);
  return;
}
EMAT_D void filter_not_hot(SVec<MutRec>& v, const SVec<IvRec>& hot) { int w = 0; for (int i = 0; i < v.n; ++i) if (iv_contains(hot.p, hot.n, v.p[i].site)) v.p[w++] = v.p[i]; v.n = w; }
EMAT_DN SVec<MutRec> sample_history_for(Ctx& c, const BranchInfo& bi) {
  return bi.is_open ? sample_unconstrained_mutational_history(c, c.L, bi.T_to_X, c.mu_prop)
                    : sample_mutational_history(c, c.L, bi.T_to_X, c.mu_prop, bi.hot_deltas);
}
EMAT_D void recompute_open_pl_A(Ctx& c, BranchInfo& bi) {
  if (!bi.is_open) return;
  bi.pl_A = bi.pl_X;
  for (int i = bi.hot_muts.n - 1; i >= 0; --i) bi.pl_A += dq(c, bi.hot_muts.p[i].site, bi.hot_muts.p[i].to, bi.hot_muts.p[i].from);
}
EMAT_DN void propose_new_rooty_graft_mutations(Ctx& c, Graft& g) { EMAT_TIMED(1);
  const int X = g.X, P = nodes_of(c)[X].parent, S = sibling_of(c, P, X);
  for (int idx = 0; idx < g.nbi && !c.failed; ++idx) {
    BranchInfo& bi = g.bi[idx];
    EMAT_CHECK(c, !bi.is_open || bi.hot_deltas.n == 0);
    if (bi.hot.n != 0) {
      SVec<MutRec> nm = sample_history_for(c, bi);
      if (nm.n != 0) {
        filter_not_hot(nm, bi.hot);
        int end_branch = (idx == k_PS) ? S : X;
        adjust_mutational_history(c, nm, bi.hot_deltas, end_branch, nodes_of(c)[end_branch].t);
      }
      bi.hot_muts = nm;
      recompute_open_pl_A(c, bi);
    }
  }
}
EMAT_D double log_pi_ratio(const Ctx& c, const MutRec& m) { return m_log(pi_a(c, m.site, m.from) / pi_a(c, m.site, m.to)); }
EMAT_DN void finish_rooty_graft_analysis(Ctx& c, Graft& g) { EMAT_TIMED(1);
  if (c.failed) return;
  const int X = g.X, P = nodes_of(c)[X].parent, S = sibling_of(c, P, X);
  const double t_X = nodes_of(c)[X].t, t_P = nodes_of(c)[P].t, t_S = nodes_of(c)[S].t;
  BranchInfo& PX = g.bi[k_PX]; BranchInfo& PS = g.bi[k_PS]; BranchInfo& SPX = g.bi[k_SPX];
  g.delta_log_G = 0.0;
  g.delta_log_G += branch_log_G(c, t_P, t_X, PX.pl_X, PX.hot_muts.p, PX.hot_muts.n);
  g.delta_log_G += branch_log_G(c, t_P, t_S, PS.pl_X, PS.hot_muts.p, PS.hot_muts.n);
  ScMark mark = sc_mark(c);
  SVec<MutRec> on_PS = sc_vec<MutRec>(c, SPX.hot_muts.n), on_PX = sc_vec<MutRec>(c, SPX.hot_muts.n);
  for (int i = SPX.hot_muts.n - 1; i >= 0; --i) { const MutRec& m = SPX.hot_muts.p[i]; if (m.t < t_P) push(c, on_PS, make_mut(m.to, m.site, m.from, t_P + (t_P - m.t))); }
  for (int i = 0; i < SPX.hot_muts.n; ++i) if (SPX.hot_muts.p[i].t >= t_P) push(c, on_PX, SPX.hot_muts.p[i]);
  g.delta_log_G += branch_log_G(c, t_P, t_X, SPX.pl_X, on_PX.p, on_PX.n);
  g.delta_log_G += branch_log_G(c, t_P, t_S, SPX.pl_A, on_PS.p, on_PS.n);
  for (int i = 0; i < PX.hot_muts.n; ++i) g.delta_log_G += log_pi_ratio(c, PX.hot_muts.p[i]);
  for (int i = 0; i < PS.hot_muts.n; ++i) g.delta_log_G += log_pi_ratio(c, PS.hot_muts.p[i]);
  for (int i = 0; i < on_PS.n; ++i) g.delta_log_G += log_pi_ratio(c, on_PS.p[i]);
  sc_release(c, mark);
  g.log_alpha_mut = 0.0;
  for (int i = 0; i < g.nbi; ++i) {
    BranchInfo& bi = g.bi[i];
    g.log_alpha_mut += log_alpha_mut_term(c.mu_prop, iv_num_sites(bi.hot.p, bi.hot.n), bi.T_to_X, bi.hot_muts.n, bi.is_open, bi.hot_deltas.n);
  }
}
EMAT_DN void peel_rooty_graft(Ctx& c, const Graft& g) { EMAT_TIMED(1);
  if (c.failed) return;
  const int X = g.X, P = nodes_of(c)[X].parent, S = sibling_of(c, P, X);
  const double t_X = nodes_of(c)[X].t, t_P = nodes_of(c)[P].t;
  const BranchInfo& PX = g.bi[k_PX]; const BranchInfo& PS = g.bi[k_PS]; const BranchInfo& SPX = g.bi[k_SPX];
  ScMark mark = sc_mark(c);
  const int nX = nmuts(c, X), nS = nmuts(c, S);
  SVec<SdRec> r2r = deltas_from_root_muts(c, P, nX + 2 * nS);
  const MutRec* mX = muts_of(c, X); const MutRec* mS = muts_of(c, S);
  for (int i = 0; i < nX && !c.failed; ++i) if (iv_contains(PX.hot.p, PX.hot.n, mX[i].site)) { sd_push_back(c, r2r, mX[i].site, mX[i].from, mX[i].to); miss_set_from_state(c, S, mX[i].site, mX[i].to); }
  for (int i = 0; i < nS && !c.failed; ++i) if (iv_contains(PS.hot.p, PS.hot.n, mS[i].site)) { sd_push_back(c, r2r, mS[i].site, mS[i].from, mS[i].to); miss_set_from_state(c, X, mS[i].site, mS[i].to); }
  for (int i = 0; i < nS && !c.failed; ++i) if (iv_contains(SPX.hot.p, SPX.hot.n, mS[i].site)) sd_push_back(c, r2r, mS[i].site, mS[i].from, mS[i].to);
  nodes_of(c)[X].muts.cnt = 0; nodes_of(c)[S].muts.cnt = 0; nodes_of(c)[P].muts.cnt = 0;
  const double t_mut_X = 0.5 * (t_P + t_X);
  list_reserve<MutRec>(c, nodes_of(c)[X].muts, SPX.hot_deltas.n);
  if (!c.failed) {
    MutRec* m = muts_of(c, X);
    for (int i = 0; i < SPX.hot_deltas.n; ++i) m[i] = make_mut(SPX.hot_deltas.p[i].from, SPX.hot_deltas.p[i].site, SPX.hot_deltas.p[i].to, t_mut_X);
    set_list_cnt(c, nodes_of(c)[X].muts, SPX.hot_deltas.n);
  }
  set_root_muts_from_deltas(c, P, r2r);
  nodes_of(c)[P].lambda = calc_lambda_at_node(c, P);
  sc_release(c, mark);
}
EMAT_DN void apply_rooty_graft(Ctx& c, const Graft& g) { EMAT_TIMED(1);
  if (c.failed) return;
  const int X = g.X, P = nodes_of(c)[X].parent, S = sibling_of(c, P, X);
  const double t_X = nodes_of(c)[X].t, t_P = nodes_of(c)[P].t, t_S = nodes_of(c)[S].t;
  const BranchInfo& PX = g.bi[k_PX]; const BranchInfo& PS = g.bi[k_PS]; const BranchInfo& SPX = g.bi[k_SPX];
  EMAT_CHECK(c, nmuts(c, S) == 0);
  ScMark mark = sc_mark(c);
  nodes_of(c)[X].muts.cnt = 0;
  SVec<SdRec> r2r = deltas_from_root_muts(c, P, PX.hot_muts.n + PS.hot_muts.n + SPX.hot_muts.n);
  nodes_of(c)[P].muts.cnt = 0;
  for (int i = PX.hot_muts.n - 1; i >= 0 && !c.failed; --i) {
    const MutRec& m = PX.hot_muts.p[i];
    list_push<MutRec>(c, nodes_of(c)[X].muts, m);
    sd_push_back(c, r2r, m.site, m.to, m.from);
    miss_set_from_state(c, S, m.site, m.from);
  }
  for (int i = PS.hot_muts.n - 1; i >= 0 && !c.failed; --i) {
    const MutRec& m = PS.hot_muts.p[i];
    list_push<MutRec>(c, nodes_of(c)[S].muts, m);
    sd_push_back(c, r2r, m.site, m.to, m.from);
    miss_set_from_state(c, X, m.site, m.from);
  }
  for (int i = 0; i < SPX.hot_muts.n && !c.failed; ++i) {
    const MutRec& m = SPX.hot_muts.p[i];
    if (m.t > t_P) list_push<MutRec>(c, nodes_of(c)[X].muts, m);
    else { list_push<MutRec>(c, nodes_of(c)[S].muts, make_mut(m.to, m.site, m.from, t_P + (t_P - m.t))); sd_push_back(c, r2r, m.site, m.from, m.to); }
  }
  sort_muts(muts_of(c, X), nmuts(c, X)); sort_muts(muts_of(c, S), nmuts(c, S));
  set_root_muts_from_deltas(c, P, r2r);
  clamp_mut_times(muts_of(c, X), nmuts(c, X), t_P, t_X); clamp_mut_times(muts_of(c, S), nmuts(c, S), t_P, t_S);
  nodes_of(c)[P].lambda = nodes_of(c)[X].lambda - delta_lambda_across_branch(c, X);
  sc_release(c, mark);
}

EMAT_DN void start_inner_graft_analysis(Ctx& c, int X, Graft& g) { EMAT_TIMED(1);
  g.X = X; g.rooty = false; g.delta_log_G = g.log_alpha_mut = 0.0; g.nbi = 0; g.bi = nullptr;
  const int P = nodes_of(c)[X].parent;
  EMAT_CHECK(c, X != hdr_of(c)->root && P != hdr_of(c)->root);
  if (c.failed) return;
  const int S = sibling_of(c, P, X);
  const double t_X = nodes_of(c)[X].t, t_P = nodes_of(c)[P].t;
  g.S = S; g.t_P = t_P;
  int bi_cap = 4;
  EMAT_TIMED_BLOCK(1, setup_timer);
  g.bi = (BranchInfo*)sc_alloc(c, (uint32_t)bi_cap * (uint32_t)sizeof(BranchInfo));
  if (c.failed) return;
  auto bi_room = [&]() {
    if (g.nbi < bi_cap) return;
    const int ncap = 2 * bi_cap;
    BranchInfo* nb = (BranchInfo*)sc_alloc(c, (uint32_t)ncap * (uint32_t)sizeof(BranchInfo));
    if (c.failed) return;
    for (int i = 0; i < g.nbi; ++i) nb[i] = g.bi[i];
    g.bi = nb; bi_cap = ncap;
  };
  SVec<IvRec> sl_iv;
  {
    BranchInfo& PX = g.bi[g.nbi++]; bi_init(PX);
    PX.A = P; PX.B = X; PX.is_open = false; PX.T_to_X = t_X - t_P;
    PX.warm = sc_vec<IvRec>(c, 1); { IvRec all; all.start = 0; all.end = c.L; push(c, PX.warm, all); }
    iv_split_sc(c, PX.hot, sl_iv, PX.warm.p, PX.warm.n, miss_of(c, S), (int)nodes_of(c)[S].miss.cnt);
  }
  int path_muts = nmuts(c, X);
  SVec<FsRec> sl_fs;
  { const int nf = (int)nodes_of(c)[S].mfs.cnt;
    sl_fs = sc_vec<FsRec>(c, nf + nmuts(c, P) + 1);
    if (!c.failed) { const FsRec* f = mfs_of(c, S); for (int i = 0; i < nf; ++i) sl_fs.p[i] = f[i]; sl_fs.n = nf; } }
  auto fs_room = [&](int more) {
    if (sl_fs.n + more <= sl_fs.cap) return;
    SVec<FsRec> nv = sc_vec<FsRec>(c, 2 * sl_fs.cap > sl_fs.n + more ? 2 * sl_fs.cap : sl_fs.n + more);
    if (c.failed) return;
    for (int i = 0; i < sl_fs.n; ++i) nv.p[i] = sl_fs.p[i];
    nv.n = sl_fs.n; sl_fs = nv;
  };
  {
    BranchInfo& PX = g.bi[0];
    PX.pl_A = nodes_of(c)[X].lambda;
    const MutRec* m = muts_of(c, X);
    for (int i = nmuts(c, X) - 1; i >= 0; --i) PX.pl_A += dq(c, m[i].site, m[i].to, m[i].from);
  }
  EMAT_TIMED_END(setup_timer);
  if (c.failed) return;
  double next_pl_B;
  { EMAT_TIMED(1);
  next_pl_B = -1 * delta_lambda_across_node_missations(c, S); }
  g.bi[0].pl_A -= next_pl_B;
  int cur = P, parent = nodes_of(c)[cur].parent, sibling = sibling_of(c, parent, cur);
  double partial_lambda = next_pl_B;
  { EMAT_TIMED(1);
  while (sl_iv.n != 0 && !c.failed) {
    bi_room(); if (c.failed) break;
    BranchInfo& bi = g.bi[g.nbi++]; bi_init(bi);
    bi.A = parent; bi.B = cur; bi.is_open = false; bi.T_to_X = t_X - nodes_of(c)[parent].t;
    bi.warm = sl_iv;
    const MutRec* mc = muts_of(c, cur); const int nc = nmuts(c, cur);
    path_muts += nc;
    fs_room(nc); if (c.failed) break;
    for (int i = nc - 1; i >= 0; --i) {
      if (iv_contains(sl_iv.p, sl_iv.n, mc[i].site)) { partial_lambda += dq(c, mc[i].site, mc[i].to, mc[i].from); fsv_set(c, sl_fs, mc[i].site, mc[i].from); }
    }
    iv_split_sc(c, bi.hot, sl_iv, bi.warm.p, bi.warm.n, miss_of(c, sibling), (int)nodes_of(c)[sibling].miss.cnt);
    { int w = 0, k = 0;
      for (int i = 0; i < sl_fs.n; ++i) {
        const int l = sl_fs.p[i].site;
        while (k < sl_iv.n && sl_iv.p[k].end <= l) ++k;
        if (k < sl_iv.n && sl_iv.p[k].start <= l) sl_fs.p[w++] = sl_fs.p[i];
      }
      sl_fs.n = w; }
    next_pl_B = -1 * delta_lambda_across_missations(c, sl_iv.p, sl_iv.n, sl_fs.p, sl_fs.n);
    bi.pl_A = partial_lambda - next_pl_B;
    partial_lambda = next_pl_B;
    c.bytes += 64 + 16 * nc + 24 * ((int)nodes_of(c)[sibling].miss.cnt + bi.warm.n);
    if (parent != hdr_of(c)->root) {
      cur = parent; parent = nodes_of(c)[cur].parent; sibling = sibling_of(c, parent, cur);
    } else {
      if (!c.includes_run_root) { bi.hot = bi.warm; bi.pl_A += partial_lambda; }
      else if (sl_iv.n != 0) {
        bi_room(); if (c.failed) break;
        BranchInfo& fo = g.bi[g.nbi++]; bi_init(fo);
        fo.A = k_no_node; fo.B = hdr_of(c)->root; fo.is_open = true; fo.T_to_X = t_X - nodes_of(c)[parent].t;
        fo.warm = sl_iv; fo.hot = sl_iv; fo.pl_A = partial_lambda;
      }
      sl_iv.n = 0; sl_fs.n = 0;
    }
  } }
  if (c.failed) return;
  { EMAT_TIMED(1);
  struct Owned { MutRec m; int owner; int pad; };
  SVec<Owned> tmp = sc_vec<Owned>(c, path_muts + 1);
  for (int i = 0; i < g.nbi; ++i) {
    BranchInfo& bi_i = g.bi[i];
    if (bi_i.B == hdr_of(c)->root) continue;
    const MutRec* mb = muts_of(c, bi_i.B);
    for (int k = nmuts(c, bi_i.B) - 1; k >= 0; --k) {
      if (iv_contains(bi_i.warm.p, bi_i.warm.n, mb[k].site)) {
        bool found = false;
        for (int j = i; j < g.nbi; ++j) if (iv_contains(g.bi[j].hot.p, g.bi[j].hot.n, mb[k].site)) { Owned o; o.m = mb[k]; o.owner = j; o.pad = 0; push(c, tmp, o); ++g.bi[j].hot_muts.cap; found = true; break; }
        EMAT_CHECK(c, found);
      }
    }
  }
  if (tmp.n == 0) {
    for (int j = 0; j < g.nbi; ++j) { BranchInfo& bi = g.bi[j]; bi.hot_muts.p = nullptr; bi.hot_muts.n = bi.hot_muts.cap = 0; bi.hot_deltas.p = nullptr; bi.hot_deltas.n = bi.hot_deltas.cap = 0; bi.pl_X = bi.pl_A; }
  } else if (!c.failed) {
    for (int j = 0; j < g.nbi; ++j) {
      BranchInfo& bi = g.bi[j];
      const int cnt = bi.hot_muts.cap;
      bi.hot_muts = sc_vec<MutRec>(c, cnt);
      bi.hot_deltas = sc_vec<SdRec>(c, cnt);
    }
    if (c.failed) return;
    for (int k = tmp.n - 1; k >= 0; --k) { SVec<MutRec>& v = g.bi[tmp.p[k].owner].hot_muts; v.p[v.n++] = tmp.p[k].m; }
    for (int j = 0; j < g.nbi && !c.failed; ++j) {
      BranchInfo& bi = g.bi[j];
      bi.pl_X = bi.pl_A;
      for (int k = 0; k < bi.hot_muts.n; ++k) {
        const MutRec& m = bi.hot_muts.p[k];
        if (!bi.is_open) sd_push_back(c, bi.hot_deltas, m.site, m.from, m.to);
        bi.pl_X += dq(c, m.site, m.from, m.to);
      }
    }
  } }
  return;
}
EMAT_DF void propose_new_inner_graft_mutations(Ctx& c, Graft& g) { EMAT_TIMED(1);
  const int X = g.X;
  for (int idx = 0; idx < g.nbi && !c.failed; ++idx) {
    BranchInfo& bi = g.bi[idx];
    if (bi.hot.n == 0) { EMAT_CHECK(c, bi.hot_muts.n == 0); continue; }
    SVec<MutRec> nm = sample_history_for(c, bi);
    if (nm.n != 0) { EMAT_TIMED(1);
      filter_not_hot(nm, bi.hot);
      if (bi.B == X) {
        int w = 0;
        for (int i = 0; i < nm.n; ++i) {
          bool drop = !sd_contains(bi.hot_deltas, nm.p[i].site) && is_site_missing_at(c, X, nm.p[i].site);
          if (!drop) nm.p[w++] = nm.p[i];
        }
        nm.n = w;
      }
      adjust_mutational_history(c, nm, bi.hot_deltas, X, nodes_of(c)[X].t);
    }
    bi.hot_muts = nm;
    recompute_open_pl_A(c, bi);
  }
}
EMAT_DF void finish_inner_graft_analysis(Ctx& c, Graft& g) { EMAT_TIMED(1);
  if (c.failed || g.nbi == 0) return;
  const int X = g.X; const double t_X = nodes_of(c)[X].t;
  g.delta_log_G = 0.0;
  for (int i = 0; i < g.nbi; ++i) { BranchInfo& bi = g.bi[i]; g.delta_log_G += branch_log_G(c, t_X - bi.T_to_X, t_X, bi.pl_X, bi.hot_muts.p, bi.hot_muts.n); }
  BranchInfo& last = g.bi[g.nbi - 1];
  if (last.is_open) for (int i = 0; i < last.hot_muts.n; ++i) g.delta_log_G += log_pi_ratio(c, last.hot_muts.p[i]);
  g.log_alpha_mut = 0.0;
  for (int i = 0; i < g.nbi; ++i) {
    BranchInfo& bi = g.bi[i];
    int Ls = iv_num_sites(bi.hot.p, bi.hot.n);
    if (bi.B == X) Ls = (c.L - nodes_of(c)[X].n_missing) - (iv_num_sites(bi.warm.p, bi.warm.n) - iv_num_sites(bi.hot.p, bi.hot.n));
    g.log_alpha_mut += log_alpha_mut_term(c.mu_prop, Ls, bi.T_to_X, bi.hot_muts.n, bi.is_open, bi.hot_deltas.n);
  }
}
EMAT_D void recalc_lambda_along_hot_path(Ctx& c, const Graft& g) {
  for (int i = 0; i + 1 < g.nbi; ++i) { int A = g.bi[i].A, B = g.bi[i].B; nodes_of(c)[A].lambda = nodes_of(c)[B].lambda - delta_lambda_across_branch(c, B); }
}
EMAT_D void erase_marked_muts(Ctx& c, int node) { MutRec* m = muts_of(c, node); int n = nmuts(c, node), w = 0; for (int i = 0; i < n; ++i) if (m[i].site != -1) m[w++] = m[i]; set_list_cnt(c, nodes_of(c)[node].muts, w); }
EMAT_DF void peel_inner_graft(Ctx& c, const Graft& g) { EMAT_TIMED(1);
  if (c.failed || g.nbi == 0) return;
  const int X = g.X, P = nodes_of(c)[X].parent, root = hdr_of(c)->root;
  const double t_X = nodes_of(c)[X].t, t_P = nodes_of(c)[P].t;
  const BranchInfo& fin = g.bi[g.nbi - 1];
  ScMark mark = sc_mark(c);
  SVec<SdRec> r2r; r2r.p = nullptr; r2r.n = r2r.cap = 0;
  if (fin.is_open) r2r = deltas_from_root_muts(c, root, path_mut_count(c, X));
  for (int i = 0; i < g.nbi && !c.failed; ++i) {
    const BranchInfo& bi = g.bi[i];
    if (bi.B == root) continue;
    if (bi.B == X && !fin.is_open) { nodes_of(c)[X].muts.cnt = 0; continue; }
    MutRec* mb = muts_of(c, bi.B);
    for (int k = nmuts(c, bi.B) - 1; k >= 0 && !c.failed; --k) {
      MutRec& m = mb[k];
      if (m.site < 0) continue;
      if (iv_contains(bi.warm.p, bi.warm.n, m.site) && (!fin.is_open || !iv_contains(fin.hot.p, fin.hot.n, m.site))) {
        for (int cur = X; cur != bi.B; cur = nodes_of(c)[cur].parent) { int par = nodes_of(c)[cur].parent; miss_set_from_state(c, sibling_of(c, par, cur), m.site, m.from); }
        m.site = -1;
      }
    }
  }
  if (fin.is_open) {
    for (int i = g.nbi - 1; i >= 0 && !c.failed; --i) {
      const BranchInfo& bi = g.bi[i];
      if (bi.B == root) continue;
      MutRec* mb = muts_of(c, bi.B);
      for (int k = 0; k < nmuts(c, bi.B) && !c.failed; ++k) {
        MutRec& m = mb[k];
        if (m.site < 0) continue;
        if (iv_contains(fin.hot.p, fin.hot.n, m.site)) {
          for (int cur = bi.B; cur != root; cur = nodes_of(c)[cur].parent) { int par = nodes_of(c)[cur].parent; miss_set_from_state(c, sibling_of(c, par, cur), m.site, m.to); }
          sd_push_back(c, r2r, m.site, m.from, m.to);
          m.site = -1;
        }
      }
    }
  }
  for (int i = 0; i < g.nbi; ++i) if (g.bi[i].B != root) erase_marked_muts(c, g.bi[i].B);
  const double t_mut_X = 0.5 * (t_P + t_X);
  for (int i = 0; i < g.nbi && !c.failed; ++i) {
    const BranchInfo& bi = g.bi[i];
    if (bi.B == root) continue;
    for (int k = 0; k < bi.hot_deltas.n; ++k) list_push<MutRec>(c, nodes_of(c)[X].muts, make_mut(bi.hot_deltas.p[k].from, bi.hot_deltas.p[k].site, bi.hot_deltas.p[k].to, t_mut_X));
  }
  if (fin.is_open) set_root_muts_from_deltas(c, root, r2r);
  recalc_lambda_along_hot_path(c, g);
  sc_release(c, mark);
}
EMAT_DF void apply_inner_graft(Ctx& c, const Graft& g) { EMAT_TIMED(1);
  if (c.failed || g.nbi == 0) return;
  const int X = g.X, root = hdr_of(c)->root;
  const BranchInfo& fin = g.bi[g.nbi - 1];
  ScMark mark = sc_mark(c);
  nodes_of(c)[X].muts.cnt = 0;
  SVec<SdRec> r2r; r2r.p = nullptr; r2r.n = r2r.cap = 0;
  if (fin.is_open) r2r = deltas_from_root_muts(c, root, fin.hot_muts.n);
  for (int i = 0; i < g.nbi && !c.failed; ++i) {
    const BranchInfo& bi = g.bi[i];
    if (bi.B == X) { list_assign<MutRec>(c, nodes_of(c)[X].muts, bi.hot_muts.p, bi.hot_muts.n); continue; }
    if (!bi.is_open) {
      for (int k = 0; k < bi.hot_muts.n && !c.failed; ++k) {
        const MutRec m = bi.hot_muts.p[k];
        for (int cur = X; cur != bi.A; cur = nodes_of(c)[cur].parent) {
          int par = nodes_of(c)[cur].parent;
          if (nodes_of(c)[par].t <= m.t && m.t < nodes_of(c)[cur].t) { list_push<MutRec>(c, nodes_of(c)[cur].muts, m); break; }
          miss_set_from_state(c, sibling_of(c, par, cur), m.site, m.to);
        }
      }
    } else {
      for (int k = bi.hot_muts.n - 1; k >= 0 && !c.failed; --k) {
        const MutRec m = bi.hot_muts.p[k];
        for (int cur = X; cur != root; cur = nodes_of(c)[cur].parent) {
          int par = nodes_of(c)[cur].parent;
          if (nodes_of(c)[par].t <= m.t && m.t < nodes_of(c)[cur].t) list_push<MutRec>(c, nodes_of(c)[cur].muts, m);
          if (nodes_of(c)[par].t <= m.t) miss_set_from_state(c, sibling_of(c, par, cur), m.site, m.from);
        }
        sd_push_back(c, r2r, m.site, m.to, m.from);
      }
    }
  }
  for (int i = 0; i < g.nbi; ++i) {
    const BranchInfo& bi = g.bi[i];
    if (!bi.is_open) { sort_muts(muts_of(c, bi.B), nmuts(c, bi.B)); clamp_mut_times(muts_of(c, bi.B), nmuts(c, bi.B), nodes_of(c)[bi.A].t, nodes_of(c)[bi.B].t); }
  }
  if (fin.is_open) set_root_muts_from_deltas(c, root, r2r);
  recalc_lambda_along_hot_path(c, g);
  sc_release(c, mark);
}

EMAT_D bool is_rooty(const Ctx& c, int X) { return nodes_of(c)[X].parent == hdr_of(c)->root; }
EMAT_D void analyze_graft(Ctx& c, int X, Graft& g) {
  if (is_rooty(c, X)) { start_rooty_graft_analysis(c, X, g); finish_rooty_graft_analysis(c, g); }
  else { start_inner_graft_analysis(c, X, g); finish_inner_graft_analysis(c, g); }
}
EMAT_D void propose_new_graft(Ctx& c, int X, Graft& g) {
  if (is_rooty(c, X)) { start_rooty_graft_analysis(c, X, g); if (!c.failed) propose_new_rooty_graft_mutations(c, g); finish_rooty_graft_analysis(c, g); }
  else { start_inner_graft_analysis(c, X, g); if (!c.failed) propose_new_inner_graft_mutations(c, g); finish_inner_graft_analysis(c, g); }
}
EMAT_D void peel_graft(Ctx& c, const Graft& g) { if (is_rooty(c, g.X)) peel_rooty_graft(c, g); else peel_inner_graft(c, g); }
EMAT_D void apply_graft(Ctx& c, const Graft& g) { if (is_rooty(c, g.X)) apply_rooty_graft(c, g); else apply_inner_graft(c, g); }
EMAT_D int count_min_mutations(const Ctx& c, const Graft& g) {
  if (g.rooty) return g.bi[k_SPX].hot_deltas.n;
  int r = 0; for (int i = 0; i < g.nbi; ++i) if (!g.bi[i].is_open) r += g.bi[i].hot_deltas.n; return r;
}
EMAT_DF SVec<SdRec> summarize_closed_mutations(Ctx& c, const Graft& g, int extra) { EMAT_TIMED(1);
  int tot = 0;
  if (g.rooty) tot = g.bi[k_SPX].hot_deltas.n; else for (int i = 0; i < g.nbi; ++i) if (!g.bi[i].is_open) tot += g.bi[i].hot_deltas.n;
  SVec<SdRec> r = sc_vec<SdRec>(c, tot + extra + 1);
  if (g.rooty) { const SVec<SdRec>& d = g.bi[k_SPX].hot_deltas; for (int k = 0; k < d.n; ++k) sd_push_back(c, r, d.p[k].site, d.p[k].from, d.p[k].to); }
  else for (int i = 0; i < g.nbi; ++i) if (!g.bi[i].is_open) { const SVec<SdRec>& d = g.bi[i].hot_deltas; for (int k = 0; k < d.n; ++k) sd_push_back(c, r, d.p[k].site, d.p[k].from, d.p[k].to); }
  return r;
}

struct alignas(16) Region { int branch, mut_idx, min_muts, pad; double t_min, t_max; double logW, W; };
struct Study {
  SVec<Region> regions;
  double lambda_X, mu, f, t_X, t_max_tip, log_Wmax, sum_W;
};
typedef uint64_t WorkItem;
EMAT_DF WorkItem wi_make(int branch, int mut_idx, int backtracking) { return ((uint64_t)(uint32_t)branch << 32) | ((uint64_t)(uint32_t)mut_idx << 1) | (uint64_t)(backtracking & 1); }
EMAT_DF int wi_branch(WorkItem w) { return (int)(uint32_t)(w >> 32); }
EMAT_DF int wi_mut_idx(WorkItem w) { return (int)((uint32_t)w >> 1); }
EMAT_DF int wi_backtracking(WorkItem w) { return (int)(w & 1u); }

EMAT_D double region_t_min(Ctx& c, int b, int mi) { if (b == hdr_of(c)->root) return k_neg_dbl_max; if (mi == 0) return nodes_of(c)[nodes_of(c)[b].parent].t; return muts_of(c, b)[mi - 1].t; }
EMAT_D double region_t_max(Ctx& c, int b, int mi) { if (b == hdr_of(c)->root) return nodes_of(c)[b].t; if (mi == nmuts(c, b)) return nodes_of(c)[b].t; return muts_of(c, b)[mi].t; }

EMAT_DN SVec<Region> study_seed_fill(Ctx& c, int X, double t_X, const SVec<IvRec>& missing_at_X_in, int max_muts_from_start,
                                    int init_branch, int init_mut_idx, SVec<SdRec>& deltas_in, bool can_change_root, HotBlock hot) {
  SVec<Region> res; res.p = nullptr; res.n = 0; res.cap = 0;
  if (c.failed) return res;
  SVec<IvRec> missing_at_X = missing_at_X_in;
  SVec<SdRec> deltas_local = deltas_in;
  const bool local_scan = (max_muts_from_start == 1);
  ScSpan span;
  uint32_t front = 0;
  bool in_block = false;
  if (local_scan && hot.p != nullptr) {
    const uint32_t need = (((uint32_t)missing_at_X_in.n * (uint32_t)sizeof(IvRec) + 15u) & ~15u) + (((uint32_t)deltas_in.n * (uint32_t)sizeof(SdRec) + 15u) & ~15u);
    if (need + 512u <= hot.bytes) {
      IvRec* mi = (IvRec*)hot.p; for (int i = 0; i < missing_at_X_in.n; ++i) mi[i] = missing_at_X_in.p[i];
      front = ((uint32_t)missing_at_X_in.n * (uint32_t)sizeof(IvRec) + 15u) & ~15u;
      SdRec* di = (SdRec*)(hot.p + front); for (int i = 0; i < deltas_in.n; ++i) di[i] = deltas_in.p[i];
      missing_at_X.p = mi; deltas_local.p = di; deltas_local.cap = deltas_in.n;
      front = need; in_block = true;
    }
  }
  SVec<SdRec>& deltas = in_block ? deltas_local : deltas_in;
  if (in_block) { span.lo = hot.p + front; span.hi = hot.p + (hot.bytes & ~15u); span.lds = true; span.reserved = true; }
  else span = local_scan ? sc_span(c, 1024) : sc_span_hbm(c);
#ifdef EMAT_PROFILE_PHASES
  if (span.lds) hdr_of(c)->phase_ticks[3] += 1;
#endif
  res.p = (Region*)span.lo;
  const int root = hdr_of(c)->root;
  if (local_scan && deltas.n < k_scan_max_deltas) {
    int4* stack_top = (int4*)span.hi;
    int sp = 0;
    auto room = [&](int extra_regions, int extra_items) -> bool {
      const uint8_t* lo = span.lo + (size_t)(res.n + extra_regions) * sizeof(Region);
      const uint8_t* hi = span.hi - (size_t)(sp + extra_items) * sizeof(int4);
      if (lo + 16 <= hi) return true;
      if (!span.lds) return false;
      ScSpan big = sc_span_hbm(c);
      if (big.lo + (size_t)(res.n + extra_regions) * sizeof(Region) + 16 > big.hi - (size_t)(sp + extra_items) * sizeof(int4)) return false;
      Region* nr = (Region*)big.lo; int4* nb = (int4*)big.hi;
      for (int i = 0; i < res.n; ++i) nr[i] = res.p[i];
      for (int i = 1; i <= sp; ++i) nb[-i] = stack_top[-i];
      span = big; res.p = nr; stack_top = nb;
      return true;
    };
    auto push_item = [&](int tb, int tmi, int pb, int pmi, int fs, int size) {
      if (!room(0, 1)) { EMAT_FAIL(c, k_part_overflow); return; }
      ++sp; stack_top[-sp] = make_int4(tb, tmi, pb, (pmi & 0xffff) | (fs << 16) | (size << 18));
    };
    push_item(init_branch, init_mut_idx, k_no_node, -1, 0, deltas.n);
    while (sp > 0 && !c.failed) {
      const int4 it = stack_top[-sp]; --sp;
      const int branch = it.x, mut_idx = it.y, pb = it.z, pmi = (int)(it.w & 0xffff);
      int fs = (it.w >> 16) & 3, size = (int)((uint32_t)it.w >> 18);
      if (pb != k_no_node && branch == pb) {
        const MutRec* m = muts_of(c, branch);
        const bool down = (mut_idx == pmi + 1);
        if (!down && mut_idx != pmi - 1) EMAT_FAIL(c, k_part_internal);
        const MutRec mm = m[down ? pmi : mut_idx];
        if (!iv_contains(missing_at_X.p, missing_at_X.n, mm.site)) {
          if (fs == 0) {
            const int new_from = down ? (int)mm.to : (int)mm.from;
            const int kk = sd_lower_bound(deltas.p, deltas.n, mm.site);
            const bool present = kk < deltas.n && deltas.p[kk].site == mm.site;
            size = deltas.n + (present ? (new_from == (int)deltas.p[kk].to ? -1 : 0) : +1);
          }
          fs += 1;
        }
      }
      if (branch == X || fs > 1) continue;
      if (!room(1, 0)) { EMAT_FAIL(c, k_part_overflow); break; }
      {
        Region* r = &res.p[res.n++];
        const int4 head = make_int4(branch, mut_idx, size, 0);
        const double2 times = make_double2(region_t_min(c, branch, mut_idx), region_t_max(c, branch, mut_idx));
        *(int4*)r = head; *(double2*)&r->t_min = times;
      }
      c.bytes += 64 + 16;
      const int nm = nmuts(c, branch);
      if (branch != root) {
        if (mut_idx > 0) { if (!(branch == pb && mut_idx - 1 == pmi)) push_item(branch, mut_idx - 1, branch, mut_idx, fs, size); }
        else { const int ub = nodes_of(c)[branch].parent, umi = nmuts(c, ub); if (!(ub == pb && umi == pmi)) push_item(ub, umi, branch, mut_idx, fs, size); }
      }
      if (mut_idx < nm) { if (!(branch == pb && mut_idx + 1 == pmi)) push_item(branch, mut_idx + 1, branch, mut_idx, fs, size); }
      else if (!is_tip(c, branch)) {
        const int c0 = nodes_of(c)[branch].child0, c1 = nodes_of(c)[branch].child1;
        if (!(c0 == pb && 0 == pmi)) push_item(c0, 0, branch, mut_idx, fs, size);
        if (!(c1 == pb && 0 == pmi)) push_item(c1, 0, branch, mut_idx, fs, size);
      }
    }
  } else {
  WorkItem* stack_base = (WorkItem*)span.hi;
  int sp = 0;
  auto room = [&](int extra_regions, int extra_items) -> bool {
    const uint8_t* lo = span.lo + (size_t)(res.n + extra_regions) * sizeof(Region);
    const uint8_t* hi = span.hi - (size_t)(sp + extra_items) * sizeof(WorkItem);
    if (lo + 16 <= hi) return true;
    if (!span.lds) return false;
    ScSpan big = sc_span_hbm(c);
    if (big.lo + (size_t)(res.n + extra_regions) * sizeof(Region) + 16 > big.hi - (size_t)(sp + extra_items) * sizeof(WorkItem)) return false;
    Region* nr = (Region*)big.lo; WorkItem* nb = (WorkItem*)big.hi;
    for (int i = 0; i < res.n; ++i) nr[i] = res.p[i];
    for (int i = 1; i <= sp; ++i) nb[-i] = stack_base[-i];
    span = big; res.p = nr; stack_base = nb;
    return true;
  };
  int cur_branch = k_no_node, cur_mut_idx = -1, cur_from_start = 0;
  int cur_size = deltas.n;
  auto add_forward = [&](int tb, int tmi) {
    if (!room(0, 2)) { EMAT_FAIL(c, k_part_overflow); return; }
    stack_base[-(sp + 1)] = wi_make(cur_branch, cur_mut_idx, 1);
    stack_base[-(sp + 2)] = wi_make(tb, tmi, 0);
    sp += 2;
  };
  add_forward(init_branch, init_mut_idx);
  while (sp > 0 && !c.failed) {
    const WorkItem wi = stack_base[-sp]; --sp;
    struct { int branch, mut_idx, backtracking; } w = {wi_branch(wi), wi_mut_idx(wi), wi_backtracking(wi)};
    const int ob = cur_branch, omi = cur_mut_idx;
    if (cur_branch != k_no_node && w.branch == cur_branch) {
      const MutRec* m = muts_of(c, cur_branch);
      const bool down = (w.mut_idx == cur_mut_idx + 1);
      if (!down && w.mut_idx != cur_mut_idx - 1) EMAT_FAIL(c, k_part_internal);
      const MutRec mm = m[down ? cur_mut_idx : w.mut_idx];
      if (!iv_contains(missing_at_X.p, missing_at_X.n, mm.site)) {
        if (down) sd_pop_front(c, deltas, mm.site, mm.from, mm.to); else sd_push_front(c, deltas, mm.site, mm.from, mm.to);
        cur_from_start += w.backtracking ? -1 : +1;
        cur_size = deltas.n;
      }
    }
    cur_branch = w.branch; cur_mut_idx = w.mut_idx;
    if (!w.backtracking && cur_branch != X && cur_from_start <= max_muts_from_start) {
      if (!room(1, 0)) { EMAT_FAIL(c, k_part_overflow); break; }
      {
        Region* r = &res.p[res.n++];
        const int4 head = make_int4(cur_branch, cur_mut_idx, cur_size, 0);
        const double2 times = make_double2(region_t_min(c, cur_branch, cur_mut_idx), region_t_max(c, cur_branch, cur_mut_idx));
        *(int4*)r = head; *(double2*)&r->t_min = times;
      }
      c.bytes += 64 + 16;
      if (cur_branch != root) {
        if (cur_mut_idx > 0) { if (!(cur_branch == ob && cur_mut_idx - 1 == omi)) add_forward(cur_branch, cur_mut_idx - 1); }
        else { int pb = nodes_of(c)[cur_branch].parent, pmi = nmuts(c, pb); if (!(pb == ob && pmi == omi)) add_forward(pb, pmi); }
      }
      if (cur_mut_idx < nmuts(c, cur_branch)) { if (!(cur_branch == ob && cur_mut_idx + 1 == omi)) add_forward(cur_branch, cur_mut_idx + 1); }
      else if (!is_tip(c, cur_branch)) {
        int c0 = nodes_of(c)[cur_branch].child0, c1 = nodes_of(c)[cur_branch].child1;
        if (!(c0 == ob && 0 == omi)) add_forward(c0, 0);
        if (!(c1 == ob && 0 == omi)) add_forward(c1, 0);
      }
    }
  }
  }
  int w = 0;
  {
    const bool have_X = X != k_no_node;
    const int P = have_X ? nodes_of(c)[X].parent : k_no_node, S = have_X ? sibling_of(c, P, X) : k_no_node;
    const int nGP = have_X ? nmuts(c, P) : 0;
    const int nS = (have_X && P == root) ? nmuts(c, S) : 0;
    const double t_min_P_end = (have_X && P != root) ? region_t_min(c, P, nGP) : 0.0;
    for (int i = 0; i < res.n; ++i) {
      int4 head = *(const int4*)&res.p[i];
      double2 times = *(const double2*)&res.p[i].t_min;
      int branch = head.x, mut_idx = head.y;
      if (!can_change_root && branch == root) continue;
      if (have_X && (branch == S || branch == P)) {
        if (P != root) {
          if (branch == S) { if (mut_idx == 0) times.x = t_min_P_end; mut_idx += nGP; }
          else { if (mut_idx == nGP) continue; branch = S; }
        } else {
          if (!can_change_root) { if (branch == P) continue; }
          else {
            if (branch == S && mut_idx == nS) { mut_idx += nGP; times.x = k_neg_dbl_max; }
            else continue;
          }
        }
      }
      if (times.x >= t_X) continue;
      if (times.y > t_X) times.y = t_X;
      head.x = branch; head.y = mut_idx;
      *(int4*)&res.p[w] = head; *(double2*)&res.p[w].t_min = times;
      ++w;
    }
  }
  res.n = w; res.cap = w;
  sc_span_commit(c, span, (uint32_t)w * (uint32_t)sizeof(Region));
  return res;
}
struct RootRegionParams { double f, t_S, s_min, s_max, x_min, x_max; int m; };
EMAT_D RootRegionParams root_region_params(Ctx& c, const Study& st, const Region& r) {
  RootRegionParams p; p.f = st.f; p.m = r.min_muts; p.t_S = nodes_of(c)[r.branch].t;
  p.s_min = fabs(st.t_X - p.t_S);
  double t_early = st.t_X < p.t_S ? st.t_X : p.t_S;
  double tree_span = st.t_max_tip - t_early;
  EMAT_CHECK(c, tree_span >= 0.0);
  p.s_max = p.s_min + 20.0 * tree_span;
  p.x_min = st.lambda_X * p.f * p.s_min; p.x_max = st.lambda_X * p.f * p.s_max;
  return p;
}
EMAT_D double safe_log_gamma_integral(Ctx& c, double a, double x_min, double x_max) {
  EMAT_CHECK(c, x_min < x_max);
  double Q_hi = gamma_q(a, x_min), Q_lo = gamma_q(a, x_max);
  return m_log(Q_hi - Q_lo);
}
constexpr double k_ln2 = 0.693147180559945309417232121458176568;
EMAT_DN double root_region_log_weight(Ctx& c, const Study& st, const Region& r) {
  const double f = st.f, lambda_X = st.lambda_X;
  const int m = r.min_muts;
  RootRegionParams p = root_region_params(c, st, r);
  if (p.x_max < 0.01) {
    double alpha = f * m + 1;
    return -k_ln2 + m_log(f * lambda_X) + f * m * m_log(st.mu / 3) + alpha * m_log(p.s_max) + m_log1p(-pow(p.s_min / p.s_max, alpha)) - m_log(alpha);
  }
  return -k_ln2 + f * m * m_log(st.mu / (3 * lambda_X * f)) + lgamma(f * m + 1) + safe_log_gamma_integral(c, f * m + 1, p.x_min, p.x_max);
}
EMAT_DN Study make_study(Ctx& c, SVec<Region> regions, int num_missing_at_X, double lambda_X, double f, double t_X, double t_max_tip) { EMAT_TIMED(1);
  Study st; st.regions = regions; st.lambda_X = lambda_X; st.f = f; st.t_X = t_X; st.t_max_tip = t_max_tip; st.log_Wmax = 0.0; st.sum_W = 0.0;
  st.mu = lambda_X / (c.L - num_missing_at_X);
  if (c.failed) return st;
  EMAT_CHECK(c, regions.n > 0);
  double log_Wmax = 0.0;
  for (int i = 0; i < regions.n; ++i) {
    const Region r = regions.p[i];
    const int m = r.min_muts;
    double logW;
    if (r.t_min != k_neg_dbl_max) {
      double t_prime = 0.5 * (r.t_min + r.t_max);
      logW = m_log(f * lambda_X * (r.t_max - r.t_min)) + f * (-lambda_X * (t_X - t_prime) + m * m_log(st.mu * (t_X - t_prime) / 3));
    } else logW = root_region_log_weight(c, st, r);
    regions.p[i].logW = logW;
    if (i == 0) log_Wmax = logW; else if (log_Wmax < logW) log_Wmax = logW;
  }
  if (regions.n > 0) {
    st.log_Wmax = log_Wmax;
    for (int i = 0; i < regions.n; ++i) {
      const double lw = regions.p[i].logW - log_Wmax, W = m_exp(lw);
      *(double2*)&regions.p[i].logW = make_double2(lw, W);
      st.sum_W += W;
    }
  }
  c.bytes += 2 * 48 * (int64_t)regions.n; c.bytes_w += 48 * (int64_t)regions.n;
  return st;
}
EMAT_D int study_pick_nexus_region(Ctx& c, const Study& st) {
  double r = uniform_co(c, 0.0, st.sum_W);
  for (int i = 0; i < st.regions.n; ++i) { if (st.regions.p[i].W >= r) return i; r -= st.regions.p[i].W; }
  return 0;
}
EMAT_DF double study_pick_time_in_region(Ctx& c, const Study& st, int idx) {
  const Region& r = st.regions.p[idx];
  if (r.t_min != k_neg_dbl_max) return uniform_oc(c, r.t_min, r.t_max);
  RootRegionParams p = root_region_params(c, st, r);
  double rand_s;
  if (p.x_max < 0.01) {
    double alpha = p.f * p.m + 1;
    double U = u01_oo(c);
    double smin_a = pow(p.s_min, alpha), smax_a = pow(p.s_max, alpha);
    rand_s = pow(smin_a + U * (smax_a - smin_a), 1.0 / alpha);
  } else {
    double alpha = p.f * p.m + 1, beta = st.lambda_X * p.f;
    double y_lo = beta * p.s_min, y_hi = beta * p.s_max;
    double Q_hi = gamma_q(alpha, y_lo), Q_lo = gamma_q(alpha, y_hi);
    EMAT_CHECK(c, Q_lo < Q_hi);
    double rand_Q = uniform_oc(c, Q_lo, Q_hi);
    double y = gamma_q_inv(alpha, rand_Q);
    double x = y / beta;
    rand_s = x < p.s_min ? p.s_min : (p.s_max < x ? p.s_max : x);
  }
  double rand_t = 0.5 * (st.t_X + p.t_S - rand_s);
  double lo = r.t_max < rand_t ? r.t_max : rand_t;
  return r.t_min > lo ? r.t_min : lo;
}
EMAT_D int study_find_region(const Study& st, int branch, double t) {
  for (int i = 0; i < st.regions.n; ++i) { const Region& r = st.regions.p[i]; if (r.branch == branch && r.t_min < t && t <= r.t_max) return i; }
  return -1;
}
EMAT_DF double study_log_alpha_in_region(Ctx& c, const Study& st, int idx, double t) {
  const Region& r = st.regions.p[idx];
  double log_p_region = r.logW - m_log(st.sum_W);
  if (r.t_min != k_neg_dbl_max) return log_p_region - m_log(r.t_max - r.t_min);
  RootRegionParams p = root_region_params(c, st, r);
  double s = st.t_X - t + p.t_S - t;
  if (s > p.s_max + 1e-6) return -k_inf;
  if (p.x_max < 0.01) {
    double alpha = p.f * p.m + 1;
    return log_p_region + k_ln2 + m_log(alpha) + (alpha - 1) * m_log(s) + -alpha * m_log(p.s_max) + -m_log1p(-pow(p.s_min / p.s_max, alpha));
  }
  return log_p_region + k_ln2 + m_log(st.lambda_X * p.f) + p.f * p.m * m_log(st.lambda_X * p.f * s) + -st.lambda_X * p.f * s
      + -lgamma(p.f * p.m + 1) - safe_log_gamma_integral(c, p.f * p.m + 1, p.x_min, p.x_max);
}

struct Spr1Frame {
  int X, init_branch, limit, n_missing_at_X;
  double t_X, lambda_X, f, t_max_tip;
  SVec<IvRec> missing_at_X;
  SVec<SdRec> deltas;
  HotBlock hot;
  bool can_change_root;
  Study study;
  int P, old_S, old_G, extra, old_min_muts, new_min_muts, new_S, pre_new_region_min_muts;
  double old_t_P, new_t_P, log_alpha_o2n;
  Graft old_graft, new_graft;
};
EMAT_DF int wave_lane() { return (int)__builtin_amdgcn_mbcnt_hi(~0u, __builtin_amdgcn_mbcnt_lo(~0u, 0u)); }
EMAT_DF double wave_bcast(double x, int src) { return __shfl(x, src, 64); }

EMAT_D void wave_make_study(Ctx& c, Spr1Frame& fr, SVec<Region> regions) {
  const int lane = wave_lane();
  Study& st = fr.study;
  if (lane == 0) {
    st.regions = regions; st.lambda_X = fr.lambda_X; st.f = fr.f; st.t_X = fr.t_X; st.t_max_tip = fr.t_max_tip; st.log_Wmax = 0.0; st.sum_W = 0.0;
    st.mu = fr.lambda_X / (c.L - fr.n_missing_at_X);
    EMAT_CHECK(c, regions.n > 0);
  }
  __syncthreads();
  if (c.failed || regions.n <= 0) return;
  const double f = fr.f, lambda_X = fr.lambda_X, t_X = fr.t_X, mu = st.mu;
  double my_max = -k_inf; bool any = false;
  for (int i = lane; i < regions.n; i += 64) {
    const Region r = regions.p[i];
    const int m = r.min_muts;
    double logW;
    if (r.t_min != k_neg_dbl_max) {
      double t_prime = 0.5 * (r.t_min + r.t_max);
      logW = m_log(f * lambda_X * (r.t_max - r.t_min)) + f * (-lambda_X * (t_X - t_prime) + m * m_log(mu * (t_X - t_prime) / 3));
    } else logW = root_region_log_weight(c, st, r);
    regions.p[i].logW = logW;
    if (logW == logW) { if (!any || my_max < logW) my_max = logW; any = true; }
  }
  for (int off = 32; off > 0; off >>= 1) { const double o = __shfl_down(my_max, off, 64); if (my_max < o) my_max = o; }
  __syncthreads();
  double log_Wmax = wave_bcast(my_max, 0);
  { const double first = regions.p[0].logW; if (first != first) log_Wmax = first; }
  for (int i = lane; i < regions.n; i += 64) {
    const double lw = regions.p[i].logW - log_Wmax, W = m_exp(lw);
    *(double2*)&regions.p[i].logW = make_double2(lw, W);
  }
  __syncthreads();
  if (lane == 0) {
    double sum_W = 0.0;
    for (int i = 0; i < regions.n; ++i) sum_W += regions.p[i].W;
    st.log_Wmax = log_Wmax; st.sum_W = sum_W;
    c.bytes += 2 * 48 * (int64_t)regions.n; c.bytes_w += 48 * (int64_t)regions.n;
  }
  __syncthreads();
}

struct alignas(16) ScanItem {
  int branch, mut_idx, pb, w;
  int child_begin, nch_vis, sz, pos;
};
static_assert(sizeof(ScanItem) == 32, "ScanItem must be two 16-byte groups");

EMAT_D bool wave_local_scan(Ctx& c, Spr1Frame& fr) {
  const int lane = wave_lane();
  const uint64_t below = lane == 0 ? 0ull : (~0ull >> (64 - lane));
  const int X = fr.X, root = hdr_of(c)->root;
  SVec<IvRec> miss = fr.missing_at_X;
  SVec<SdRec> del = fr.deltas;
  if (del.n >= k_scan_max_deltas) return false;
  uint32_t front = 0;
  bool in_block = false;
  if (fr.hot.p != nullptr) {
    const uint32_t b_miss = ((uint32_t)miss.n * (uint32_t)sizeof(IvRec) + 15u) & ~15u, b_del = ((uint32_t)del.n * (uint32_t)sizeof(SdRec) + 15u) & ~15u;
    if (b_miss + b_del + 512u <= fr.hot.bytes) {
      IvRec* mi = (IvRec*)fr.hot.p; SdRec* di = (SdRec*)(fr.hot.p + b_miss);
      for (int i = lane; i < miss.n; i += 64) mi[i] = miss.p[i];
      for (int i = lane; i < del.n; i += 64) di[i] = del.p[i];
      miss.p = mi; del.p = di; front = b_miss + b_del; in_block = true;
      __syncthreads();
    }
  }
  bool done = false;
  ScanItem* items = nullptr; int* lvl = nullptr; int total = 0, nlev = 0;
  uint8_t* hbm_lo = nullptr;
  for (int attempt = 0; attempt < 2 && !done; ++attempt) {
    uint8_t* base; uint32_t bytes;
    if (attempt == 0) {
      if (fr.hot.p == nullptr || !in_block || fr.hot.bytes - front < 24u * 36u) continue;
      base = fr.hot.p + front; bytes = (fr.hot.bytes - front) & ~15u;
    } else {
      const uint32_t g0 = (c.sc_top + 15u) & ~15u, g1 = hdr_of(c)->scratch_end & ~15u;
      if (g1 < g0 + 8192u) return false;
      const uint32_t span = g1 - g0, skip = (span / 96u * 48u) & ~15u;
      base = c.G + g0 + skip; bytes = span - skip; hbm_lo = c.G + g0;
    }
    const int cap = (int)(bytes / 36u);
    items = (ScanItem*)base; lvl = (int*)(base + (size_t)cap * sizeof(ScanItem));
    if (lane == 0) { ScanItem it; it.branch = fr.init_branch; it.mut_idx = 0; it.pb = k_no_node; it.w = 0xffff | (0 << 16) | (del.n << 18); it.child_begin = 0; it.nch_vis = 0; it.sz = 0; it.pos = 0; items[0] = it; }
    __syncthreads();
    total = 1; nlev = 0;
    int lo = 0, hi = 1; bool overflow = false;
    while (lo < hi && !overflow) {
      if (nlev >= cap) { overflow = true; break; }
      if (lane == 0) lvl[nlev] = lo;
      ++nlev;
      int new_total = total;
      for (int chunk = lo; chunk < hi && !overflow; chunk += 64) {
        const int k = chunk + lane;
        const bool act = k < hi;
        int nch = 0, tb[3], tmi[3], branch = 0, mut_idx = 0, fs = 0, size = 0; bool visited = false;
        if (act) {
          const int4 a4 = *(const int4*)&items[k];
          branch = a4.x; mut_idx = a4.y;
          const int pb = a4.z, pmi = (int)(a4.w & 0xffff);
          fs = (a4.w >> 16) & 3; size = (int)((uint32_t)a4.w >> 18);
          if (pb != k_no_node && branch == pb) {
            const MutRec* m = muts_of(c, branch);
            const bool down = (mut_idx == pmi + 1);
            if (!down && mut_idx != pmi - 1) EMAT_FAIL(c, k_part_internal);
            const MutRec mm = m[down ? pmi : mut_idx];
            if (!iv_contains(miss.p, miss.n, mm.site)) {
              if (fs == 0) {
                const int new_from = down ? (int)mm.to : (int)mm.from;
                const int kk = sd_lower_bound(del.p, del.n, mm.site);
                const bool present = kk < del.n && del.p[kk].site == mm.site;
                size = del.n + (present ? (new_from == (int)del.p[kk].to ? -1 : 0) : +1);
              }
              fs += 1;
            }
          }
          visited = !(branch == X || fs > 1);
          if (visited) {
            const int nm = nmuts(c, branch);
            if (branch != root) {
              if (mut_idx > 0) { if (!(branch == pb && mut_idx - 1 == pmi)) { tb[nch] = branch; tmi[nch] = mut_idx - 1; ++nch; } }
              else { const int ub = nodes_of(c)[branch].parent, umi = nmuts(c, ub); if (!(ub == pb && umi == pmi)) { tb[nch] = ub; tmi[nch] = umi; ++nch; } }
            }
            if (mut_idx < nm) { if (!(branch == pb && mut_idx + 1 == pmi)) { tb[nch] = branch; tmi[nch] = mut_idx + 1; ++nch; } }
            else if (!is_tip(c, branch)) {
              const int c0 = nodes_of(c)[branch].child0, c1 = nodes_of(c)[branch].child1;
              if (!(c0 == pb && 0 == pmi)) { tb[nch] = c0; tmi[nch] = 0; ++nch; }
              if (!(c1 == pb && 0 == pmi)) { tb[nch] = c1; tmi[nch] = 0; ++nch; }
            }
          }
        }
        const uint64_t b0 = __ballot(act && (nch & 1)), b1 = __ballot(act && (nch & 2));
        const int off = __popcll(b0 & below) + 2 * __popcll(b1 & below);
        const int tot = __popcll(b0) + 2 * __popcll(b1);
        if (new_total + tot > cap) { overflow = true; break; }
        if (act) {
          const int w_own = (mut_idx & 0xffff) | (fs << 16) | (size << 18);
          for (int j = 0; j < nch; ++j) {
            ScanItem* ch = &items[new_total + off + j];
            *(int4*)ch = make_int4(tb[j], tmi[j], branch, w_own);
            *((int4*)ch + 1) = make_int4(0, 0, 0, 0);
          }
          items[k].w = w_own;
          *((int4*)&items[k] + 1) = make_int4(new_total + off, nch | (visited ? 256 : 0), 0, 0);
        }
        new_total += tot;
      }
      __syncthreads();
      lo = hi; hi = new_total; total = new_total;
    }
    done = !overflow;
  }
#ifdef EMAT_PROFILE_PHASES
  if (lane == 0) { int64_t* ex = (int64_t*)hdr_of(c)->reserved; ex[0] += 1; ex[1] += miss.n; ex[2] += del.n; ex[3] += total; ex[4] += nlev; ex[5] += (hbm_lo != nullptr) ? 1 : 0; ex[6] += done ? 0 : 1; ex[7] += in_block ? 0 : 1; }
#endif
  if (!done || c.failed) return false;
  for (int l = nlev - 1; l >= 0; --l) {
    const int lo = lvl[l], hi = l + 1 < nlev ? lvl[l + 1] : total;
    for (int k = lo + lane; k < hi; k += 64) {
      const int4 b4 = *((const int4*)&items[k] + 1);
      int sz = 0;
      if (b4.y & 256) { sz = 1; for (int j = 0; j < (b4.y & 3); ++j) sz += items[b4.x + j].sz; }
      items[k].sz = sz;
    }
    __syncthreads();
  }
  for (int l = 0; l < nlev; ++l) {
    const int lo = lvl[l], hi = l + 1 < nlev ? lvl[l + 1] : total;
    for (int k = lo + lane; k < hi; k += 64) {
      const int4 b4 = *((const int4*)&items[k] + 1);
      if (!(b4.y & 256)) continue;
      int running = b4.w + 1;
      for (int j = (b4.y & 3) - 1; j >= 0; --j) { const int szc = items[b4.x + j].sz; if (szc > 0) { items[b4.x + j].pos = running; running += szc; } }
    }
    __syncthreads();
  }
  const int V = items[0].sz;
  SVec<Region>* shared = &fr.study.regions;
  if (lane == 0) {
    SVec<Region> r; r.n = 0; r.cap = 0; r.p = nullptr;
    if (hbm_lo != nullptr) {
      if ((size_t)V * sizeof(Region) + 16 <= (size_t)((uint8_t*)items - hbm_lo)) { r.p = (Region*)hbm_lo; r.cap = V; c.sc_top = (uint32_t)(hbm_lo - c.G) + (((uint32_t)V * (uint32_t)sizeof(Region) + 15u) & ~15u); }
      else EMAT_FAIL(c, k_part_overflow);
    } else r = sc_vec<Region>(c, V);
    *shared = r;
  }
  __syncthreads();
  if (c.failed) return true;
  Region* res = shared->p;
  for (int k = lane; k < total; k += 64) {
    const ScanItem it = items[k];
    if (!(it.nch_vis & 256)) continue;
    Region* r = &res[it.pos];
    *(int4*)r = make_int4(it.branch, it.mut_idx, (int)((uint32_t)it.w >> 18), 0);
    *(double2*)&r->t_min = make_double2(region_t_min(c, it.branch, it.mut_idx), region_t_max(c, it.branch, it.mut_idx));
  }
  __syncthreads();
  int w = 0;
  {
    const bool can_change_root = fr.can_change_root;
    const int P = nodes_of(c)[X].parent, S = sibling_of(c, P, X);
    const int nGP = nmuts(c, P);
    const int nS = (P == root) ? nmuts(c, S) : 0;
    const double t_min_P_end = (P != root) ? region_t_min(c, P, nGP) : 0.0;
    const double t_X = fr.t_X;
    for (int chunk = 0; chunk < V; chunk += 64) {
      const int i = chunk + lane;
      bool keep = false; int4 head = make_int4(0, 0, 0, 0); double2 times = make_double2(0.0, 0.0);
      if (i < V) {
        head = *(const int4*)&res[i]; times = *(const double2*)&res[i].t_min;
        int branch = head.x, mut_idx = head.y;
        keep = true;
        if (!can_change_root && branch == root) keep = false;
        else if (branch == S || branch == P) {
          if (P != root) {
            if (branch == S) { if (mut_idx == 0) times.x = t_min_P_end; mut_idx += nGP; }
            else { if (mut_idx == nGP) keep = false; else branch = S; }
          } else {
            if (!can_change_root) { if (branch == P) keep = false; }
            else {
              if (branch == S && mut_idx == nS) { mut_idx += nGP; times.x = k_neg_dbl_max; }
              else keep = false;
            }
          }
        }
        if (keep) { if (times.x >= t_X) keep = false; else { if (times.y > t_X) times.y = t_X; head.x = branch; head.y = mut_idx; } }
      }
      const uint64_t m = __ballot(keep);
      if (keep) { Region* r = &res[w + __popcll(m & below)]; *(int4*)r = head; *(double2*)&r->t_min = times; }
      w += __popcll(m);
    }
  }
  __syncthreads();
  if (lane == 0) {
    shared->n = w;
    sc_trim(c, *shared);
    c.bytes += (int64_t)(64 + 16) * V;
  }
  __syncthreads();
  return true;
}

EMAT_DN void wave_scan_and_study(Ctx& c) {
  Spr1Frame& fr = *(Spr1Frame*)c.frame;
  const int lane = wave_lane();
  SVec<Region>* shared = &fr.study.regions;
#ifdef EMAT_PROFILE_PHASES
  const long long ph0 = clock64();
#endif
  bool scanned = false;
#ifndef EMAT_SERIAL_SCAN
  if (fr.limit == 1) scanned = wave_local_scan(c, fr);
#endif
  if (!scanned) {
    if (lane == 0) *shared = study_seed_fill(c, fr.X, fr.t_X, fr.missing_at_X, fr.limit, fr.init_branch, 0, fr.deltas, fr.can_change_root, fr.hot);
    __syncthreads();
  }
#ifdef EMAT_PROFILE_PHASES
  if (lane == 0) { hdr_of(c)->phase_ticks[6] += clock64() - ph0; hdr_of(c)->phase_ticks[13] += shared->n; }
#endif
  const SVec<Region> regions = *shared;
  wave_make_study(c, fr, regions);
}

}
}
```

### delphy_amd/csrc/emat_part_kernels.hpp

```cpp
#ifndef EMAT_PART_KERNELS_HPP_
#define EMAT_PART_KERNELS_HPP_

#if defined(EMAT_PROFILE_PHASES) || defined(EMAT_COUNT_CALLS)
namespace emat {
constexpr int k_fn_replicas = 64;
__device__ unsigned long long g_fn_ticks[k_fn_replicas * 3 * 2048][2];
__device__ unsigned g_fn_min_list_bytes = 0;
__shared__ int s_fn_count_me;
struct FnTimer {
  int key; long long t0;
  __device__ FnTimer(int k) : key(k), t0(clock64()) {}
  __device__ void stop() { if (key >= 0) { this->~FnTimer(); key = -1; } }
  __device__ ~FnTimer() { if (key >= 0 && threadIdx.x == 0 && s_fn_count_me) { const long long dt = clock64() - t0; unsigned long long* e = g_fn_ticks[(blockIdx.x & (k_fn_replicas - 1)) * (3 * 2048) + key]; atomicAdd(&e[0], (unsigned long long)dt); atomicAdd(&e[1], 1ull); } }
};
}
#endif
#ifdef EMAT_PROFILE_PHASES
namespace emat { __device__ unsigned long long g_arena_site_bytes[2048][2]; }
#endif
#define EMAT_DEV_NS dev_lds
#define EMAT_VARIANT_LDS 1
#include "emat_device_moves.hpp"
#undef EMAT_DEV_NS
#undef EMAT_VARIANT_LDS
#define EMAT_DEV_NS dev_mix
#define EMAT_VARIANT_LDS 2
#include "emat_device_moves.hpp"
#undef EMAT_DEV_NS
#undef EMAT_VARIANT_LDS
#define EMAT_DEV_NS dev
#define EMAT_VARIANT_LDS 0
#include "emat_device_moves.hpp"

namespace emat {

struct KernelArgs {
  uint8_t* slabs;
  const uint64_t* slab_off;
  const int32_t* order;
  int64_t* part_ticks;
  const int32_t* ref_freqs;
  const double* cum_nu;
  double* stats_out;
  EvoTable evo;
  const PopTable* pop;
  SharedCells shared;
  RunFlags flags;
  int32_t num_parts;
  uint32_t lds_slab_bytes;
  uint32_t lds_scratch_bytes;
  int64_t moves_per_part;
  const int64_t* moves_for_part;
  int32_t* part_status;
  int64_t extra_moves_part0;
  int32_t one_more_below;
  int32_t chunks, class_count, class_stride, taper;
  int32_t* side_started;
  int32_t single_below;
  int32_t full_release;
  int32_t cum_w[8];
  int32_t* chunk_done;
  uint8_t* snaps;
};

constexpr int k_wave = 64;
constexpr int k_ticket_log = 8;

__device__ inline void wave_copy16(uint8_t* dst, const uint8_t* src, uint32_t bytes, int lane) {
  const uint4* s = (const uint4*)src; uint4* d = (uint4*)dst;
  for (uint32_t i = lane; i < bytes / 16; i += k_wave) d[i] = s[i];
}
__device__ inline void wave_copy8_through(uint8_t* dst, const uint8_t* src, uint32_t bytes, int lane) {
  const uint64_t* s = (const uint64_t*)src; uint64_t* d = (uint64_t*)dst;
  for (uint32_t i = lane; i < bytes / 8; i += k_wave) __hip_atomic_store(&d[i], s[i], __ATOMIC_RELAXED, __HIP_MEMORY_SCOPE_AGENT);
}
__device__ inline double wave_sum(double x) {
  for (int off = 32; off > 0; off >>= 1) x += __shfl_down(x, off, k_wave);
  return __shfl(x, 0, k_wave);
}

template <class CtxT> __device__ inline void init_ctx(CtxT& c, uint8_t* slab, uint8_t* gslab, const KernelArgs& a, const double* lds_tables, SlabHeader* H = nullptr) {
  c.S = slab; c.G = gslab; c.H = H != nullptr ? H : (SlabHeader*)slab; c.N = (NodeRec*)(slab + c.H->off_nodes);
  c.L = a.evo.num_sites;
  c.ref = (const __attribute__((address_space(1))) uint8_t*)a.evo.ref_sequence; c.part = (const __attribute__((address_space(1))) uint8_t*)a.evo.partition_for_site;
  c.nu = (const __attribute__((address_space(1))) double*)a.evo.nu_l; c.cumQ = (const __attribute__((address_space(1))) double*)a.evo.cum_Q_l;
  c.have_logq = lds_tables != nullptr;
  c.uniform_sites = a.evo.uniform_sites != 0;
  if (lds_tables) { c.mu = lds_tables; c.pi = lds_tables + k_max_lds_partitions; c.q = lds_tables + k_max_lds_partitions * 5; }
  else { c.mu = a.evo.mu; c.pi = a.evo.pi; c.q = a.evo.q; }
  c.pop = a.pop;
  c.sh_ktw = a.shared.k_twiddle_bar; c.sh_tsop = a.shared.ts_over_pop; c.sh_nact = a.shared.num_active_parts;
  c.t_max_tip = a.flags.t_max_tip;
  c.only_displacing_inner_nodes = a.flags.only_displacing_inner_nodes != 0;
  c.topology_moves_enabled = a.flags.topology_moves_enabled != 0;
  c.includes_run_root = (c.H->flags & k_flag_includes_run_root) != 0;
  rng_enter_leg(c, *c.H);
  c.phase = 0; c.svc = 0; c.frame = nullptr;
  c.mu_prop = 0.0; c.sc_top = c.H->scratch_begin; c.A = nullptr; c.a_top = 0; c.a_end = 0; c.failed = false; c.bytes = 0; c.bytes_w = 0;
  c.tr_kind = -1; c.tr_node = -1; c.tr_acc = -1; c.tr_log_mh = 0.0; c.heap_limit = 0; c.mix_total = 0.0;
}
__device__ inline const double* stage_tables(const KernelArgs& a, double* lds_tables, int lane) {
  if (a.evo.num_partitions > k_max_lds_partitions) return nullptr;
  const int P = a.evo.num_partitions;
  for (int i = lane; i < P; i += k_wave) lds_tables[i] = a.evo.mu[i];
  for (int i = lane; i < P * 4; i += k_wave) lds_tables[k_max_lds_partitions + i] = a.evo.pi[i];
  for (int i = lane; i < P * 16; i += k_wave) lds_tables[k_max_lds_partitions * 5 + i] = a.evo.q[i];
  for (int i = lane; i < P * 16; i += k_wave) { const double arg = a.evo.mu[i / 16] * 1.0 * a.evo.q[i]; emat_lds_logq[i] = arg > 0.0 ? dev::m_log(arg) : 0.0; }
  return lds_tables;
}

#ifndef EMAT_WAVES_PER_EU
#define EMAT_WAVES_PER_EU 4
#endif
#define EMAT_OCCUPANCY __attribute__((amdgpu_waves_per_eu(EMAT_WAVES_PER_EU, EMAT_WAVES_PER_EU)))
constexpr uint32_t k_lds_heap_room = 1024;

__device__ __forceinline__ int xcc_id() { return (int)(__builtin_amdgcn_s_getreg(20 | (0 << 6) | ((4 - 1) << 11)) & 15u); }
__global__ void k_probe_xcc(int32_t* out) { if (threadIdx.x == 0) out[blockIdx.x] = xcc_id(); }

template <bool kSide> __device__ __forceinline__ void run_moves_body(const KernelArgs& a) {
  const int lane = threadIdx.x;
  if (kSide && a.side_started != nullptr && lane == 0) __hip_atomic_fetch_add(a.side_started, 1, __ATOMIC_RELAXED, __HIP_MEMORY_SCOPE_AGENT);
  double* lds_tables = (double*)emat_lds_tables;
  const bool tables_staged = stage_tables(a, lds_tables, lane) != nullptr;
  uint8_t* lds_slab = emat_lds;
  int* lds_flag = (int*)(emat_lds_ctx + k_lds_ctx_bytes - 16);
  const int chunk = a.chunks > 1 ? (int)blockIdx.x / a.class_stride : 0, slot = a.chunks > 1 ? (int)blockIdx.x % a.class_stride : (int)blockIdx.x;
  if (a.chunks > 1 && slot >= a.class_count) return;
  const bool single = a.chunks > 1 && slot < a.single_below;
  if (single && chunk > 0) return;
  const int part = a.order[slot];
  if (lane == 0 && chunk < k_ticket_log) a.part_ticks[(size_t)(2 + 2 * chunk) * a.num_parts + part] = (int64_t)wall_clock64();
  auto st_status = [&](int32_t v) { __hip_atomic_store(&a.part_status[part], v, __ATOMIC_RELAXED, __HIP_MEMORY_SCOPE_AGENT); };
  auto ld_status = [&]() -> int32_t { return __hip_atomic_load(&a.part_status[part], __ATOMIC_RELAXED, __HIP_MEMORY_SCOPE_AGENT); };
  auto st_ticks = [&](int64_t v) { __hip_atomic_store(&a.part_ticks[part], v, __ATOMIC_RELAXED, __HIP_MEMORY_SCOPE_AGENT); };
  auto ld_ticks = [&]() -> int64_t { return __hip_atomic_load(&a.part_ticks[part], __ATOMIC_RELAXED, __HIP_MEMORY_SCOPE_AGENT); };
  uint8_t* gslab = a.slabs + a.slab_off[part];
  SlabHeader* gh = (SlabHeader*)gslab;
#if !defined(EMAT_PROFILE_PHASES) && !defined(EMAT_COUNT_CALLS)
  if ((uint32_t)(uintptr_t)(__attribute__((address_space(3))) uint8_t*)emat_lds != k_lds_dyn_base) {
    if (lane == 0) { gh->fail_line = -3; st_status(k_part_internal); if (a.chunks > 1) __hip_atomic_store(&a.chunk_done[part], a.chunks, __ATOMIC_RELEASE, __HIP_MEMORY_SCOPE_AGENT); }
    return;
  }
#endif
  const int64_t pass_target = a.moves_for_part ? a.moves_for_part[part] : a.moves_per_part + (part == 0 ? a.extra_moves_part0 : 0) + (part < a.one_more_below ? 1 : 0);
  int64_t target = pass_target, done_at_start;
  if (a.chunks > 1) {
    if (chunk > 0) {
      if (lane == 0) {
        const uint64_t w0 = wall_clock64();
        bool waited = false, gave_up = false;
        int32_t seen;
        while (((seen = __hip_atomic_load(&a.chunk_done[part], __ATOMIC_ACQUIRE, __HIP_MEMORY_SCOPE_AGENT)) & 0xff) < chunk) {
          __builtin_amdgcn_s_sleep(64); waited = true;
          if (wall_clock64() - w0 > 12000000000ull) { gave_up = true; break; }
        }
        if (!gave_up && (seen & 0x100) != 0 && ((seen >> 12) & 15) != xcc_id()) { gave_up = true; gh->fail_line = k_fail_line_other_xcd; }
        if (waited) atomicAdd((unsigned long long*)&a.chunk_done[((a.num_parts + 1) & ~1) + 2 * (blockIdx.x & 63)], (unsigned long long)(wall_clock64() - w0));
        if (gave_up) { st_status(k_part_internal); __hip_atomic_store(&a.chunk_done[part], a.chunks, __ATOMIC_RELEASE, __HIP_MEMORY_SCOPE_AGENT); *lds_flag = -1; } else *lds_flag = 0;
      }
      __syncthreads();
      if (*lds_flag == -1) return;
    } else if (lane == 0) __hip_atomic_store(&gh->pad0, (uint32_t)gh->moves_done, __ATOMIC_RELAXED, __HIP_MEMORY_SCOPE_AGENT);
    __syncthreads();
    if (single) target = pass_target;
    else if (a.cum_w[0] > 0) target = chunk + 1 == a.chunks ? pass_target : pass_target * a.cum_w[chunk] / a.cum_w[a.chunks - 1];
    else if (a.taper) { const int64_t nn = a.chunks, done_w = (int64_t)(chunk + 1) * (2 * nn - chunk), all_w = nn * (nn + 1); target = chunk + 1 == a.chunks ? pass_target : pass_target * done_w / all_w; }
    else target = pass_target * (chunk + 1) / a.chunks;
    done_at_start = gh->moves_done - (int64_t)(uint32_t)((uint32_t)gh->moves_done - gh->pad0);
  } else done_at_start = gh->moves_done;
  const uint32_t area = a.lds_slab_bytes;
#if defined(EMAT_PROFILE_PHASES) || defined(EMAT_COUNT_CALLS)
  if (lane == 0) s_fn_count_me = (gh->heap_top - gh->heap_begin) >= g_fn_min_list_bytes ? 1 : 0;
#endif
  const bool can_stage = tables_staged && area != 0 && gh->off_nodes == (uint32_t)sizeof(SlabHeader);
  if (lane == 0 && chunk == 0) { st_ticks(0); a.part_ticks[a.num_parts + part] = (int64_t)wall_clock64(); }
  bool allow_whole = true;
  bool plain_hbm_writes = false;
  for (int leg = 0; leg < 2; ++leg) {
    __syncthreads();
    const uint32_t hbm_heap_end = gh->heap_end;
    uint32_t lds_heap_end = 0;
    if (can_stage && allow_whole) {
      const uint32_t want = (gh->heap_top + k_lds_heap_room + 15u) & ~15u;
      if (hbm_heap_end <= area) lds_heap_end = hbm_heap_end < want ? hbm_heap_end : want;
      else if (want <= area) lds_heap_end = want;
    }
    const bool staged = lds_heap_end != 0;
    if (!staged) plain_hbm_writes = true;
    const bool prefix = can_stage && !staged && gh->heap_begin <= area;
    const uint32_t staged_bytes = staged ? gh->heap_top : (prefix ? gh->heap_begin : 0u);
    if (staged_bytes) { wave_copy16(emat_lds_hdr, gslab, (uint32_t)sizeof(SlabHeader), lane); wave_copy16(lds_slab, gslab + sizeof(SlabHeader), staged_bytes - (uint32_t)sizeof(SlabHeader), lane); }
    uint8_t* const snap = (!staged && a.snaps != nullptr) ? a.snaps + a.slab_off[part] : nullptr;
    if (snap != nullptr) wave_copy16(snap, gslab, (gh->heap_top + 15u) & ~15u, lane);
    __syncthreads();
    SlabHeader* const lds_hdr = (SlabHeader*)emat_lds_hdr;
    SlabHeader* H = (staged || prefix) ? lds_hdr : gh;
    const bool raise_prio = kSide || (gh->flags & k_flag_includes_run_root) != 0;
    uint64_t tick0 = 0;
    if (lane == 0) {
      if (staged) {
        dev_lds::Ctx& c = *(dev_lds::Ctx*)(emat_lds_ctx);
        init_ctx(c, gslab, gslab, a, lds_tables, lds_hdr);
        H->heap_end = lds_heap_end;
        dev_lds::begin_leg(c);
        const uint32_t used = (lds_heap_end + 15u) & ~15u;
        c.A = lds_slab + (used - (uint32_t)sizeof(SlabHeader)); c.a_end = area + a.lds_scratch_bytes - used;
      } else if (prefix) {
        dev_mix::Ctx& c = *(dev_mix::Ctx*)(emat_lds_ctx);
        init_ctx(c, gslab, gslab, a, lds_tables, lds_hdr);
        dev_mix::begin_leg(c);
        const uint32_t used = (gh->heap_begin + 15u) & ~15u;
        c.A = lds_slab + (used - (uint32_t)sizeof(SlabHeader)); c.a_end = area + a.lds_scratch_bytes - used;
      } else {
        dev::Ctx& c = *(dev::Ctx*)(emat_lds_ctx);
        init_ctx(c, gslab, gslab, a, tables_staged ? lds_tables : nullptr);
        dev::begin_leg(c);
        if (area + a.lds_scratch_bytes > (uint32_t)sizeof(SlabHeader)) { c.A = lds_slab; c.a_end = area + a.lds_scratch_bytes - (uint32_t)sizeof(SlabHeader); }
      }
      const bool stopped_before = chunk > 0 && ld_status() != 0;
      ((dev::Ctx*)(emat_lds_ctx))->moves_left = (H->status == 0 && !stopped_before) ? target - (H->moves_done - done_at_start) : 0;
      tick0 = wall_clock64();
      if (raise_prio) __builtin_amdgcn_s_setprio(3);
    }
    __syncthreads();
    for (;;) {
      if (lane == 0) {
        if (staged) dev_lds::run_chain_loop(*(dev_lds::Ctx*)(emat_lds_ctx));
        else if (prefix) dev_mix::run_chain_loop(*(dev_mix::Ctx*)(emat_lds_ctx));
        else dev::run_chain_loop(*(dev::Ctx*)(emat_lds_ctx));
      }
      __syncthreads();
      const int svc = ((const dev::Ctx*)(emat_lds_ctx))->svc;
      if (svc == 0) break;
      if (svc == 2) dev::rng_fill(*(dev::Ctx*)(emat_lds_ctx), lane);
      else if (staged) dev_lds::wave_scan_and_study(*(dev_lds::Ctx*)(emat_lds_ctx));
      else if (prefix) dev_mix::wave_scan_and_study(*(dev_mix::Ctx*)(emat_lds_ctx));
      else dev::wave_scan_and_study(*(dev::Ctx*)(emat_lds_ctx));
      __syncthreads();
    }
    if (lane == 0) {
      if (raise_prio) __builtin_amdgcn_s_setprio(0);
      const dev::Ctx& c = *(const dev::Ctx*)(emat_lds_ctx);
      dev::rng_leave_leg(c, *H);
      H->alg_bytes += c.bytes; H->alg_write16 += (uint32_t)((c.bytes_w + 8) >> 4);
      const int64_t dt = (int64_t)(wall_clock64() - tick0);
      H->device_ticks += dt;
      st_ticks(ld_ticks() + dt);
      if (!(chunk > 0 && ld_status() != 0)) st_status(H->status);
      int again = 0;
      if (staged) {
        H->heap_end = hbm_heap_end;
        if (H->status == k_part_need_space && lds_heap_end < hbm_heap_end && H->heap_top <= hbm_heap_end) { H->status = 0; st_status(0); again = 1; }
        else if (H->status == k_part_overflow && lds_heap_end < hbm_heap_end) { st_status(0); again = 2; }
        else if (H->status == k_part_cell_overflow && leg == 0) { st_status(k_part_need_cells); again = 3; }
        else if (H->status == k_part_overflow) { st_status(k_part_need_space); again = 3; }
      } else if (snap != nullptr && (H->status == k_part_overflow || H->status == k_part_cell_overflow)) {
        st_status(H->status == k_part_cell_overflow ? k_part_need_cells : k_part_need_space); again = 4;
      }
      *lds_flag = again;
    }
    __syncthreads();
    const int again_all = *lds_flag;
    if (again_all < 2) {
      const uint32_t out_bytes = staged ? ((const SlabHeader*)emat_lds_hdr)->heap_top : (prefix ? staged_bytes : 0u);
      if (out_bytes && a.chunks > 1 && !single) { wave_copy8_through(gslab, emat_lds_hdr, (uint32_t)sizeof(SlabHeader), lane); wave_copy8_through(gslab + sizeof(SlabHeader), lds_slab, out_bytes - (uint32_t)sizeof(SlabHeader), lane); }
      else if (out_bytes) { wave_copy16(gslab, emat_lds_hdr, (uint32_t)sizeof(SlabHeader), lane); wave_copy16(gslab + sizeof(SlabHeader), lds_slab, out_bytes - (uint32_t)sizeof(SlabHeader), lane); }
    }
    if (again_all == 4) { wave_copy16(gslab, snap, (((const SlabHeader*)snap)->heap_top + 15u) & ~15u, lane); break; }
    if (again_all == 0 || again_all == 3) break;
    allow_whole = false;
  }
  if (lane == 0 && chunk < k_ticket_log) a.part_ticks[(size_t)(3 + 2 * chunk) * a.num_parts + part] = (int64_t)wall_clock64();
  if (a.chunks > 1 && !single) {
    __syncthreads();
    if (lane == 0) {
      if (plain_hbm_writes || a.full_release) __hip_atomic_store(&a.chunk_done[part], chunk + 1, __ATOMIC_RELEASE, __HIP_MEMORY_SCOPE_AGENT);
      else { __builtin_amdgcn_fence(__ATOMIC_RELEASE, "workgroup"); __builtin_amdgcn_s_waitcnt(0); __hip_atomic_store(&a.chunk_done[part], (chunk + 1) | 0x100 | (xcc_id() << 12), __ATOMIC_RELAXED, __HIP_MEMORY_SCOPE_AGENT); }
    }
  }
}
__global__ void __launch_bounds__(k_wave) EMAT_OCCUPANCY EMAT_NOTAIL k_run_moves(KernelArgs a) { run_moves_body<false>(a); }
__global__ void __launch_bounds__(k_wave) EMAT_OCCUPANCY EMAT_NOTAIL k_run_moves_side(KernelArgs a) { run_moves_body<true>(a); }
__global__ void k_wait_side_start(const int32_t* started, int32_t expected) {
  if (threadIdx.x != 0) return;
  const uint64_t w0 = wall_clock64();
  while (__hip_atomic_load(started, __ATOMIC_RELAXED, __HIP_MEMORY_SCOPE_AGENT) < expected && wall_clock64() - w0 < 200000ull) __builtin_amdgcn_s_sleep(8);
}

constexpr int k_max_stats_partitions = 4;
constexpr int k_stats_row = k_max_stats_partitions * (4 + 16) + 1;
__global__ void __launch_bounds__(k_wave) k_global_stats(KernelArgs a) {
  __shared__ double sh_T[k_wave][k_max_stats_partitions * 4];
  __shared__ int sh_M[k_wave][k_max_stats_partitions * 16];
  const int lane = threadIdx.x;
  const int part = blockIdx.x;
  uint8_t* slab = a.slabs + a.slab_off[part];
  dev::Ctx c;
  init_ctx(c, slab, slab, a, nullptr);
  const int P = a.evo.num_partitions, W = 4 * P;
  const int n = c.H->n_nodes, root = c.H->root;
  double* D = (double*)(slab + c.H->scratch_begin);
  for (int i = lane; i < n; i += k_wave) {
    double* d = D + (size_t)i * W;
    for (int k = 0; k < W; ++k) d[k] = 0.0;
    const IvRec* iv = dev::miss_of(c, i);
    for (int j = 0; j < (int)c.N[i].miss.cnt; ++j) {
      const double* hi = a.cum_nu + (size_t)iv[j].end * W; const double* lo = a.cum_nu + (size_t)iv[j].start * W;
      for (int k = 0; k < W; ++k) d[k] -= hi[k] - lo[k];
    }
    const FsRec* fs = dev::mfs_of(c, i);
    for (int j = 0; j < (int)c.N[i].mfs.cnt; ++j) { const int l = fs[j].site, b = c.part[l]; d[4 * b + c.ref[l]] += c.nu[l]; d[4 * b + fs[j].state] -= c.nu[l]; }
    const MutRec* m = dev::muts_of(c, i);
    for (int j = 0; j < dev::nmuts(c, i); ++j) { const int l = m[j].site, b = c.part[l]; d[4 * b + m[j].from] -= c.nu[l]; d[4 * b + m[j].to] += c.nu[l]; }
  }
  __syncthreads();
  if (lane == 0) {
    const double* ref_row = a.cum_nu + (size_t)c.L * W;
    for (int k = 0; k < W; ++k) D[(size_t)root * W + k] += ref_row[k];
    int cur = root;
    while (cur != dev::k_no_node) {
      if (!dev::is_tip(c, cur)) {
        for (int kk = 0; kk < 2; ++kk) {
          const int ch = kk == 0 ? c.N[cur].child0 : c.N[cur].child1;
          for (int k = 0; k < W; ++k) D[(size_t)ch * W + k] += D[(size_t)cur * W + k];
        }
        cur = c.N[cur].child0;
      } else {
        int prev = cur; cur = c.N[cur].parent;
        while (cur != dev::k_no_node && c.N[cur].child1 == prev) { prev = cur; cur = c.N[cur].parent; }
        if (cur != dev::k_no_node) cur = c.N[cur].child1;
      }
    }
  }
  __syncthreads();
  for (int k = 0; k < W; ++k) sh_T[lane][k] = 0.0;
  for (int k = 0; k < 4 * W; ++k) sh_M[lane][k] = 0;
  for (int i = lane; i < n; i += k_wave) {
    if (i == root) continue;
    const double t_P = c.N[c.N[i].parent].t, len = c.N[i].t - t_P;
    const double* d = D + (size_t)i * W;
    for (int k = 0; k < W; ++k) sh_T[lane][k] += d[k] * len;
    const MutRec* m = dev::muts_of(c, i);
    for (int j = dev::nmuts(c, i) - 1; j >= 0; --j) {
      const int l = m[j].site, b = c.part[l];
      sh_T[lane][4 * b + m[j].to] -= c.nu[l] * (m[j].t - t_P);
      sh_T[lane][4 * b + m[j].from] += c.nu[l] * (m[j].t - t_P);
      sh_M[lane][16 * b + 4 * m[j].from + m[j].to] += 1;
    }
  }
  __syncthreads();
  double* out = a.stats_out + (size_t)part * k_stats_row;
  for (int k = lane; k < W; k += k_wave) { double sum = 0.0; for (int r = 0; r < k_wave; ++r) sum += sh_T[r][k]; out[k] = sum; }
  for (int k = lane; k < 4 * W; k += k_wave) { long long sum = 0; for (int r = 0; r < k_wave; ++r) sum += sh_M[r][k]; out[k_max_stats_partitions * 4 + k] = (double)sum; }
  if (lane == 0) {
    long long nm = 0;
    for (int k = 0; k < 4 * W; ++k) for (int r = 0; r < k_wave; ++r) nm += sh_M[r][k];
    out[k_stats_row - 1] = (double)nm;
  }
}

template <bool kCheck> __device__ __forceinline__ void recalc_derived_body(const KernelArgs& a, double* check_out) {
  __shared__ __attribute__((aligned(16))) double lds_tables[k_lds_tables_bytes / 8];
  const int lane = threadIdx.x;
  const int part = blockIdx.x;
  uint8_t* slab = a.slabs + a.slab_off[part];
// ... 359 lines not shown
```

Before: 538.6 million moves/s.

## Pin move frames to a fixed LDS slot with address-space-3 typed access

The per-move CoreFrame and Spr1Frame records are no longer allocated from the scratch arena on each move in the LDS variants. They now sit in a fixed 16-byte-aligned slot carved out after the staged heap, and they are accessed through address_space(3) references so the compiler can emit direct LDS instructions instead of generic flat loads and stores. A shared plan_leg helper decides the staging plan and reserves the frame slot, shrinking the heap room or falling back when there is not enough space. The risks are that slightly fewer parts get fully staged and that the added address-space qualifiers may change code generation in the graft and study routines.

```diff
diff --git a/delphy_amd/csrc/emat_debug_host.hpp b/delphy_amd/csrc/emat_debug_host.hpp
--- a/delphy_amd/csrc/emat_debug_host.hpp
+++ b/delphy_amd/csrc/emat_debug_host.hpp
@@ -181,7 +181,8 @@
   for (auto& ph : h->parts) {
     const SlabHeader* H = (const SlabHeader*)(h->h_slabs.data() + ph.slab_off);
     const bool can = tables && area != 0 && H->off_nodes == (uint32_t)sizeof(SlabHeader);
-    if (can && (H->heap_end <= area || H->heap_top + k_lds_heap_room <= area)) ++out3[0]; else if (can && H->heap_begin <= area) ++out3[1]; else ++out3[2];
+    const LegPlan plan = plan_leg(can, true, H->heap_begin, H->heap_top, H->heap_end, area, h->cfg.use_lds ? h->cfg_lds_scratch : 0u);
+    if (plan.staged) ++out3[0]; else if (plan.prefix) ++out3[1]; else ++out3[2];
   }
   return EMAT_OK;
 }
@@ -220,10 +221,8 @@
   for (size_t p = 0; p < h->parts.size(); ++p) {
     const SlabHeader* H = (const SlabHeader*)(h->h_slabs.data() + h->parts[p].slab_off);
     if (h->class_of[p] != h->num_classes - 1) { out_n[p] = -1; continue; }
-    const uint32_t want = (H->heap_top + k_lds_heap_room + 15u) & ~15u;
-    uint32_t used;
-    if (H->heap_end <= area) used = std::min(H->heap_end, want); else if (want <= area) used = want; else used = (H->heap_begin + 15u) & ~15u;
-    out_n[p] = used <= area ? (int32_t)(area - ((used + 15u) & ~15u)) : 0;
+    const LegPlan plan = plan_leg(area != 0, true, H->heap_begin, H->heap_top, H->heap_end, area, 0u);
+    out_n[p] = (plan.staged || plan.prefix) ? (int32_t)(area - plan.used - k_frame_bytes) : 0;
   }
   return EMAT_OK;
 }
diff --git a/delphy_amd/csrc/emat_device_core.hpp b/delphy_amd/csrc/emat_device_core.hpp
--- a/delphy_amd/csrc/emat_device_core.hpp
+++ b/delphy_amd/csrc/emat_device_core.hpp
@@ -128,6 +128,14 @@
 EMAT_DF const double* pi_of(const Ctx& c) { return c.pi; }
 EMAT_DF const double* q_of(const Ctx& c) { return c.q; }
 #endif
+#undef EMAT_FRAME_AS
+#if EMAT_VARIANT_LDS && defined(__HIP_DEVICE_COMPILE__)
+#define EMAT_FRAME_AS __attribute__((address_space(3)))
+template <class F> EMAT_DF EMAT_FRAME_AS F& frame_of(const Ctx& c) { return *(EMAT_FRAME_AS F*)(uintptr_t)(uint32_t)(uintptr_t)c.frame; }
+#else
+#define EMAT_FRAME_AS
+template <class F> EMAT_DF F& frame_of(const Ctx& c) { return *(F*)c.frame; }
+#endif
 
 EMAT_D void fail_at(Ctx& c, int status, int line) {
   if (!c.failed) { c.failed = true; if (hdr_of(c)->status == 0) { hdr_of(c)->status = status; hdr_of(c)->fail_line = line; } }
diff --git a/delphy_amd/csrc/emat_device_moves.hpp b/delphy_amd/csrc/emat_device_moves.hpp
--- a/delphy_amd/csrc/emat_device_moves.hpp
+++ b/delphy_amd/csrc/emat_device_moves.hpp
@@ -31,9 +31,19 @@
   double new_t, alpha_ratio, old_t_P, d_prior, log_mh;
   Graft old_graft, new_graft;
 };
-#ifndef EMAT_CF
-#define EMAT_CF(c) (*(CoreFrame*)(c).frame)
-#endif
+#undef EMAT_CF
+#define EMAT_CF(c) (frame_of<CoreFrame>(c))
+constexpr uint32_t k_frame_bytes = (uint32_t)(((sizeof(Spr1Frame) > sizeof(CoreFrame) ? sizeof(Spr1Frame) : sizeof(CoreFrame)) + 15u) & ~(size_t)15u);
+static_assert(alignof(Spr1Frame) <= 16 && alignof(CoreFrame) <= 16, "the frame slot is 16-byte aligned");
+template <class F> EMAT_DF bool frame_begin(Ctx& c) {
+  static_assert(sizeof(F) <= k_frame_bytes, "the move's frame outgrew its slot");
+#if !EMAT_VARIANT_LDS
+  uint8_t* f = sc_alloc(c, (uint32_t)sizeof(F));
+  if (c.failed) return false;
+  c.frame = f;
+#endif
+  return true;
+}
 EMAT_NOTAIL EMAT_DN void spr_move_core(Ctx& c, int X, int new_branch, double new_t, double alpha_ratio) { EMAT_TIMED(2);
   if (X == hdr_of(c)->root) return;
   if (!c.includes_run_root) if (nodes_of(c)[X].parent == hdr_of(c)->root || new_branch == hdr_of(c)->root) return;
@@ -43,11 +53,10 @@
     const double new_t_P = new_t;
     if (new_t_P == t_X || new_t_P == nodes_of(c)[new_branch].t || (P != hdr_of(c)->root && new_t_P == nodes_of(c)[nodes_of(c)[P].parent].t)) return;
     if (coal_needs_cells(c, new_t_P)) { stop_for_cells(c, c.tr_kind); return; }
-    CoreFrame* f = (CoreFrame*)sc_alloc(c, (uint32_t)sizeof(CoreFrame));
-    if (c.failed) return;
-    c.frame = (uint8_t*)f;
-    f->X = X; f->new_branch = new_branch; f->P = P; f->old_S = sibling_of(c, P, X);
-    f->new_t = new_t; f->alpha_ratio = alpha_ratio; f->old_t_P = nodes_of(c)[P].t;
+    if (!frame_begin<CoreFrame>(c)) return;
+    EMAT_FRAME_AS CoreFrame& f = EMAT_CF(c);
+    f.X = X; f.new_branch = new_branch; f.P = P; f.old_S = sibling_of(c, P, X);
+    f.new_t = new_t; f.alpha_ratio = alpha_ratio; f.old_t_P = nodes_of(c)[P].t;
   }
   c.mu_prop = nodes_of(c)[hdr_of(c)->root].lambda / (c.L - nodes_of(c)[hdr_of(c)->root].n_missing);
   EMAT_PHASE_BEGIN();
@@ -61,7 +70,7 @@
   if (c.failed) return;
   EMAT_CF(c).d_prior = coal_delta_displace_coalescence(c, EMAT_CF(c).old_t_P, EMAT_CF(c).new_t);
   {
-    const CoreFrame& f = EMAT_CF(c);
+    const EMAT_FRAME_AS CoreFrame& f = EMAT_CF(c);
     EMAT_CF(c).log_mh = (f.new_graft.delta_log_G - f.new_graft.log_alpha_mut) - (f.old_graft.delta_log_G - f.old_graft.log_alpha_mut) + m_log(f.alpha_ratio) + f.d_prior;
   }
   if (c.failed) return;
@@ -422,10 +431,8 @@
   const bool pruning_changes_root = P == hdr_of(c)->root;
   if (pruning_changes_root && !c.includes_run_root) return;
   EMAT_PHASE_BEGIN();
-  Spr1Frame* frp = (Spr1Frame*)sc_alloc(c, (uint32_t)sizeof(Spr1Frame));
-  if (c.failed) return;
-  Spr1Frame& fr = *frp;
-  c.frame = (uint8_t*)frp;
+  if (!frame_begin<Spr1Frame>(c)) return;
+  EMAT_FRAME_AS Spr1Frame& fr = frame_of<Spr1Frame>(c);
   fr.X = X; fr.t_X = nodes_of(c)[X].t; fr.P = P; fr.old_t_P = nodes_of(c)[P].t; fr.old_S = sibling_of(c, P, X); fr.old_G = nodes_of(c)[P].parent;
   fr.limit = limit; fr.f = 0.8 ; fr.t_max_tip = c.t_max_tip; fr.can_change_root = c.includes_run_root;
   {
@@ -451,11 +458,11 @@
   spr1_park(c, 1);
 }
 EMAT_NOTAIL EMAT_DN void spr1_move_propose(Ctx& c) { EMAT_TIMED(2);
-  Spr1Frame& fr = *(Spr1Frame*)c.frame;
+  EMAT_FRAME_AS Spr1Frame& fr = frame_of<Spr1Frame>(c);
   c.phase = 0;
   if (c.failed) return;
   EMAT_PHASE_BEGIN();
-  const Study& pre = fr.study;
+  const EMAT_FRAME_AS Study& pre = fr.study;
   const int X = fr.X, P = fr.P;
   int new_region; double new_t_P;
   { EMAT_TIMED(2);
@@ -487,11 +494,11 @@
   spr1_park(c, 2);
 }
 EMAT_NOTAIL EMAT_DN void spr1_move_finish(Ctx& c) { EMAT_TIMED(2);
-  Spr1Frame& fr = *(Spr1Frame*)c.frame;
+  EMAT_FRAME_AS Spr1Frame& fr = frame_of<Spr1Frame>(c);
   c.phase = 0;
   if (c.failed) return;
   EMAT_PHASE_BEGIN();
-  const Study& post = fr.study;
+  const EMAT_FRAME_AS Study& post = fr.study;
   const int X = fr.X;
   const int old_region = study_find_region(post, fr.old_S, fr.old_t_P);
   EMAT_CHECK(c, old_region != -1);
diff --git a/delphy_amd/csrc/emat_device_spr.hpp b/delphy_amd/csrc/emat_device_spr.hpp
--- a/delphy_amd/csrc/emat_device_spr.hpp
+++ b/delphy_amd/csrc/emat_device_spr.hpp
@@ -443,7 +443,7 @@
   return r;
 }
 
-EMAT_DN void start_rooty_graft_analysis(Ctx& c, int X, Graft& g) { EMAT_TIMED(1);
+EMAT_DN void start_rooty_graft_analysis(Ctx& c, int X, EMAT_FRAME_AS Graft& g) { EMAT_TIMED(1);
   g.X = X; g.rooty = true; g.delta_log_G = g.log_alpha_mut = 0.0;
   const int P = nodes_of(c)[X].parent, S = sibling_of(c, P, X);
   const double t_X = nodes_of(c)[X].t, t_P = nodes_of(c)[P].t, t_S = nodes_of(c)[S].t;
@@ -499,7 +499,7 @@
   bi.pl_A = bi.pl_X;
   for (int i = bi.hot_muts.n - 1; i >= 0; --i) bi.pl_A += dq(c, bi.hot_muts.p[i].site, bi.hot_muts.p[i].to, bi.hot_muts.p[i].from);
 }
-EMAT_DN void propose_new_rooty_graft_mutations(Ctx& c, Graft& g) { EMAT_TIMED(1);
+EMAT_DN void propose_new_rooty_graft_mutations(Ctx& c, EMAT_FRAME_AS Graft& g) { EMAT_TIMED(1);
   const int X = g.X, P = nodes_of(c)[X].parent, S = sibling_of(c, P, X);
   for (int idx = 0; idx < g.nbi && !c.failed; ++idx) {
     BranchInfo& bi = g.bi[idx];
@@ -517,7 +517,7 @@
   }
 }
 EMAT_D double log_pi_ratio(const Ctx& c, const MutRec& m) { return m_log(pi_a(c, m.site, m.from) / pi_a(c, m.site, m.to)); }
-EMAT_DN void finish_rooty_graft_analysis(Ctx& c, Graft& g) { EMAT_TIMED(1);
+EMAT_DN void finish_rooty_graft_analysis(Ctx& c, EMAT_FRAME_AS Graft& g) { EMAT_TIMED(1);
   if (c.failed) return;
   const int X = g.X, P = nodes_of(c)[X].parent, S = sibling_of(c, P, X);
   const double t_X = nodes_of(c)[X].t, t_P = nodes_of(c)[P].t, t_S = nodes_of(c)[S].t;
@@ -541,7 +541,7 @@
     g.log_alpha_mut += log_alpha_mut_term(c.mu_prop, iv_num_sites(bi.hot.p, bi.hot.n), bi.T_to_X, bi.hot_muts.n, bi.is_open, bi.hot_deltas.n);
   }
 }
-EMAT_DN void peel_rooty_graft(Ctx& c, const Graft& g) { EMAT_TIMED(1);
+EMAT_DN void peel_rooty_graft(Ctx& c, const EMAT_FRAME_AS Graft& g) { EMAT_TIMED(1);
   if (c.failed) return;
   const int X = g.X, P = nodes_of(c)[X].parent, S = sibling_of(c, P, X);
   const double t_X = nodes_of(c)[X].t, t_P = nodes_of(c)[P].t;
@@ -565,7 +565,7 @@
   nodes_of(c)[P].lambda = calc_lambda_at_node(c, P);
   sc_release(c, mark);
 }
-EMAT_DN void apply_rooty_graft(Ctx& c, const Graft& g) { EMAT_TIMED(1);
+EMAT_DN void apply_rooty_graft(Ctx& c, const EMAT_FRAME_AS Graft& g) { EMAT_TIMED(1);
   if (c.failed) return;
   const int X = g.X, P = nodes_of(c)[X].parent, S = sibling_of(c, P, X);
   const double t_X = nodes_of(c)[X].t, t_P = nodes_of(c)[P].t, t_S = nodes_of(c)[S].t;
@@ -599,7 +599,7 @@
   sc_release(c, mark);
 }
 
-EMAT_DN void start_inner_graft_analysis(Ctx& c, int X, Graft& g) { EMAT_TIMED(1);
+EMAT_DN void start_inner_graft_analysis(Ctx& c, int X, EMAT_FRAME_AS Graft& g) { EMAT_TIMED(1);
   g.X = X; g.rooty = false; g.delta_log_G = g.log_alpha_mut = 0.0; g.nbi = 0; g.bi = nullptr;
   const int P = nodes_of(c)[X].parent;
   EMAT_CHECK(c, X != hdr_of(c)->root && P != hdr_of(c)->root);
@@ -728,7 +728,7 @@
   } }
   return;
 }
-EMAT_DF void propose_new_inner_graft_mutations(Ctx& c, Graft& g) { EMAT_TIMED(1);
+EMAT_DF void propose_new_inner_graft_mutations(Ctx& c, EMAT_FRAME_AS Graft& g) { EMAT_TIMED(1);
   const int X = g.X;
   for (int idx = 0; idx < g.nbi && !c.failed; ++idx) {
     BranchInfo& bi = g.bi[idx];
@@ -750,7 +750,7 @@
     recompute_open_pl_A(c, bi);
   }
 }
-EMAT_DF void finish_inner_graft_analysis(Ctx& c, Graft& g) { EMAT_TIMED(1);
+EMAT_DF void finish_inner_graft_analysis(Ctx& c, EMAT_FRAME_AS Graft& g) { EMAT_TIMED(1);
   if (c.failed || g.nbi == 0) return;
   const int X = g.X; const double t_X = nodes_of(c)[X].t;
   g.delta_log_G = 0.0;
@@ -765,11 +765,11 @@
     g.log_alpha_mut += log_alpha_mut_term(c.mu_prop, Ls, bi.T_to_X, bi.hot_muts.n, bi.is_open, bi.hot_deltas.n);
   }
 }
-EMAT_D void recalc_lambda_along_hot_path(Ctx& c, const Graft& g) {
+EMAT_D void recalc_lambda_along_hot_path(Ctx& c, const EMAT_FRAME_AS Graft& g) {
   for (int i = 0; i + 1 < g.nbi; ++i) { int A = g.bi[i].A, B = g.bi[i].B; nodes_of(c)[A].lambda = nodes_of(c)[B].lambda - delta_lambda_across_branch(c, B); }
 }
 EMAT_D void erase_marked_muts(Ctx& c, int node) { MutRec* m = muts_of(c, node); int n = nmuts(c, node), w = 0; for (int i = 0; i < n; ++i) if (m[i].site != -1) m[w++] = m[i]; set_list_cnt(c, nodes_of(c)[node].muts, w); }
-EMAT_DF void peel_inner_graft(Ctx& c, const Graft& g) { EMAT_TIMED(1);
+EMAT_DF void peel_inner_graft(Ctx& c, const EMAT_FRAME_AS Graft& g) { EMAT_TIMED(1);
   if (c.failed || g.nbi == 0) return;
   const int X = g.X, P = nodes_of(c)[X].parent, root = hdr_of(c)->root;
   const double t_X = nodes_of(c)[X].t, t_P = nodes_of(c)[P].t;
@@ -818,7 +818,7 @@
   recalc_lambda_along_hot_path(c, g);
   sc_release(c, mark);
 }
-EMAT_DF void apply_inner_graft(Ctx& c, const Graft& g) { EMAT_TIMED(1);
+EMAT_DF void apply_inner_graft(Ctx& c, const EMAT_FRAME_AS Graft& g) { EMAT_TIMED(1);
   if (c.failed || g.nbi == 0) return;
   const int X = g.X, root = hdr_of(c)->root;
   const BranchInfo& fin = g.bi[g.nbi - 1];
@@ -860,21 +860,21 @@
 }
 
 EMAT_D bool is_rooty(const Ctx& c, int X) { return nodes_of(c)[X].parent == hdr_of(c)->root; }
-EMAT_D void analyze_graft(Ctx& c, int X, Graft& g) {
+EMAT_D void analyze_graft(Ctx& c, int X, EMAT_FRAME_AS Graft& g) {
   if (is_rooty(c, X)) { start_rooty_graft_analysis(c, X, g); finish_rooty_graft_analysis(c, g); }
   else { start_inner_graft_analysis(c, X, g); finish_inner_graft_analysis(c, g); }
 }
-EMAT_D void propose_new_graft(Ctx& c, int X, Graft& g) {
+EMAT_D void propose_new_graft(Ctx& c, int X, EMAT_FRAME_AS Graft& g) {
   if (is_rooty(c, X)) { start_rooty_graft_analysis(c, X, g); if (!c.failed) propose_new_rooty_graft_mutations(c, g); finish_rooty_graft_analysis(c, g); }
   else { start_inner_graft_analysis(c, X, g); if (!c.failed) propose_new_inner_graft_mutations(c, g); finish_inner_graft_analysis(c, g); }
 }
-EMAT_D void peel_graft(Ctx& c, const Graft& g) { if (is_rooty(c, g.X)) peel_rooty_graft(c, g); else peel_inner_graft(c, g); }
-EMAT_D void apply_graft(Ctx& c, const Graft& g) { if (is_rooty(c, g.X)) apply_rooty_graft(c, g); else apply_inner_graft(c, g); }
-EMAT_D int count_min_mutations(const Ctx& c, const Graft& g) {
+EMAT_D void peel_graft(Ctx& c, const EMAT_FRAME_AS Graft& g) { if (is_rooty(c, g.X)) peel_rooty_graft(c, g); else peel_inner_graft(c, g); }
+EMAT_D void apply_graft(Ctx& c, const EMAT_FRAME_AS Graft& g) { if (is_rooty(c, g.X)) apply_rooty_graft(c, g); else apply_inner_graft(c, g); }
+EMAT_D int count_min_mutations(const Ctx& c, const EMAT_FRAME_AS Graft& g) {
   if (g.rooty) return g.bi[k_SPX].hot_deltas.n;
   int r = 0; for (int i = 0; i < g.nbi; ++i) if (!g.bi[i].is_open) r += g.bi[i].hot_deltas.n; return r;
 }
-EMAT_DF SVec<SdRec> summarize_closed_mutations(Ctx& c, const Graft& g, int extra) { EMAT_TIMED(1);
+EMAT_DF SVec<SdRec> summarize_closed_mutations(Ctx& c, const EMAT_FRAME_AS Graft& g, int extra) { EMAT_TIMED(1);
   int tot = 0;
   if (g.rooty) tot = g.bi[k_SPX].hot_deltas.n; else for (int i = 0; i < g.nbi; ++i) if (!g.bi[i].is_open) tot += g.bi[i].hot_deltas.n;
   SVec<SdRec> r = sc_vec<SdRec>(c, tot + extra + 1);
@@ -897,12 +897,13 @@
 EMAT_D double region_t_min(Ctx& c, int b, int mi) { if (b == hdr_of(c)->root) return k_neg_dbl_max; if (mi == 0) return nodes_of(c)[nodes_of(c)[b].parent].t; return muts_of(c, b)[mi - 1].t; }
 EMAT_D double region_t_max(Ctx& c, int b, int mi) { if (b == hdr_of(c)->root) return nodes_of(c)[b].t; if (mi == nmuts(c, b)) return nodes_of(c)[b].t; return muts_of(c, b)[mi].t; }
 
-EMAT_DN SVec<Region> study_seed_fill(Ctx& c, int X, double t_X, const SVec<IvRec>& missing_at_X_in, int max_muts_from_start,
-                                    int init_branch, int init_mut_idx, SVec<SdRec>& deltas_in, bool can_change_root, HotBlock hot) {
+EMAT_DN SVec<Region> study_seed_fill(Ctx& c, int X, double t_X, const EMAT_FRAME_AS SVec<IvRec>& missing_at_X_in, int max_muts_from_start,
+                                    int init_branch, int init_mut_idx, EMAT_FRAME_AS SVec<SdRec>& deltas_frame, bool can_change_root, HotBlock hot) {
   SVec<Region> res; res.p = nullptr; res.n = 0; res.cap = 0;
   if (c.failed) return res;
   SVec<IvRec> missing_at_X = missing_at_X_in;
-  SVec<SdRec> deltas_local = deltas_in;
+  SVec<SdRec> deltas = deltas_frame;
+  const SVec<SdRec> deltas_in = deltas;
   const bool local_scan = (max_muts_from_start == 1);
   ScSpan span;
   uint32_t front = 0;
@@ -913,11 +914,10 @@
       IvRec* mi = (IvRec*)hot.p; for (int i = 0; i < missing_at_X_in.n; ++i) mi[i] = missing_at_X_in.p[i];
       front = ((uint32_t)missing_at_X_in.n * (uint32_t)sizeof(IvRec) + 15u) & ~15u;
       SdRec* di = (SdRec*)(hot.p + front); for (int i = 0; i < deltas_in.n; ++i) di[i] = deltas_in.p[i];
-      missing_at_X.p = mi; deltas_local.p = di; deltas_local.cap = deltas_in.n;
+      missing_at_X.p = mi; deltas.p = di; deltas.cap = deltas_in.n;
       front = need; in_block = true;
     }
   }
-  SVec<SdRec>& deltas = in_block ? deltas_local : deltas_in;
   if (in_block) { span.lo = hot.p + front; span.hi = hot.p + (hot.bytes & ~15u); span.lds = true; span.reserved = true; }
   else span = local_scan ? sc_span(c, 1024) : sc_span_hbm(c);
 #ifdef EMAT_PROFILE_PHASES
@@ -1082,10 +1082,11 @@
   }
   res.n = w; res.cap = w;
   sc_span_commit(c, span, (uint32_t)w * (uint32_t)sizeof(Region));
+  if (!in_block) deltas_frame = deltas;
   return res;
 }
 struct RootRegionParams { double f, t_S, s_min, s_max, x_min, x_max; int m; };
-EMAT_D RootRegionParams root_region_params(Ctx& c, const Study& st, const Region& r) {
+EMAT_D RootRegionParams root_region_params(Ctx& c, const EMAT_FRAME_AS Study& st, const Region& r) {
   RootRegionParams p; p.f = st.f; p.m = r.min_muts; p.t_S = nodes_of(c)[r.branch].t;
   p.s_min = fabs(st.t_X - p.t_S);
   double t_early = st.t_X < p.t_S ? st.t_X : p.t_S;
@@ -1101,7 +1102,7 @@
   return m_log(Q_hi - Q_lo);
 }
 constexpr double k_ln2 = 0.693147180559945309417232121458176568;
-EMAT_DN double root_region_log_weight(Ctx& c, const Study& st, const Region& r) {
+EMAT_DN double root_region_log_weight(Ctx& c, const EMAT_FRAME_AS Study& st, const Region& r) {
   const double f = st.f, lambda_X = st.lambda_X;
   const int m = r.min_muts;
   RootRegionParams p = root_region_params(c, st, r);
@@ -1111,6 +1112,7 @@
   }
   return -k_ln2 + f * m * m_log(st.mu / (3 * lambda_X * f)) + lgamma(f * m + 1) + safe_log_gamma_integral(c, f * m + 1, p.x_min, p.x_max);
 }
+#if !EMAT_VARIANT_LDS
 EMAT_DN Study make_study(Ctx& c, SVec<Region> regions, int num_missing_at_X, double lambda_X, double f, double t_X, double t_max_tip) { EMAT_TIMED(1);
   Study st; st.regions = regions; st.lambda_X = lambda_X; st.f = f; st.t_X = t_X; st.t_max_tip = t_max_tip; st.log_Wmax = 0.0; st.sum_W = 0.0;
   st.mu = lambda_X / (c.L - num_missing_at_X);
@@ -1139,12 +1141,13 @@
   c.bytes += 2 * 48 * (int64_t)regions.n; c.bytes_w += 48 * (int64_t)regions.n;
   return st;
 }
-EMAT_D int study_pick_nexus_region(Ctx& c, const Study& st) {
+#endif
+EMAT_D int study_pick_nexus_region(Ctx& c, const EMAT_FRAME_AS Study& st) {
   double r = uniform_co(c, 0.0, st.sum_W);
   for (int i = 0; i < st.regions.n; ++i) { if (st.regions.p[i].W >= r) return i; r -= st.regions.p[i].W; }
   return 0;
 }
-EMAT_DF double study_pick_time_in_region(Ctx& c, const Study& st, int idx) {
+EMAT_DF double study_pick_time_in_region(Ctx& c, const EMAT_FRAME_AS Study& st, int idx) {
   const Region& r = st.regions.p[idx];
   if (r.t_min != k_neg_dbl_max) return uniform_oc(c, r.t_min, r.t_max);
   RootRegionParams p = root_region_params(c, st, r);
@@ -1168,11 +1171,11 @@
   double lo = r.t_max < rand_t ? r.t_max : rand_t;
   return r.t_min > lo ? r.t_min : lo;
 }
-EMAT_D int study_find_region(const Study& st, int branch, double t) {
+EMAT_D int study_find_region(const EMAT_FRAME_AS Study& st, int branch, double t) {
   for (int i = 0; i < st.regions.n; ++i) { const Region& r = st.regions.p[i]; if (r.branch == branch && r.t_min < t && t <= r.t_max) return i; }
   return -1;
 }
-EMAT_DF double study_log_alpha_in_region(Ctx& c, const Study& st, int idx, double t) {
+EMAT_DF double study_log_alpha_in_region(Ctx& c, const EMAT_FRAME_AS Study& st, int idx, double t) {
   const Region& r = st.regions.p[idx];
   double log_p_region = r.logW - m_log(st.sum_W);
   if (r.t_min != k_neg_dbl_max) return log_p_region - m_log(r.t_max - r.t_min);
@@ -1202,9 +1205,9 @@
 EMAT_DF int wave_lane() { return (int)__builtin_amdgcn_mbcnt_hi(~0u, __builtin_amdgcn_mbcnt_lo(~0u, 0u)); }
 EMAT_DF double wave_bcast(double x, int src) { return __shfl(x, src, 64); }
 
-EMAT_D void wave_make_study(Ctx& c, Spr1Frame& fr, SVec<Region> regions) {
+EMAT_D void wave_make_study(Ctx& c, EMAT_FRAME_AS Spr1Frame& fr, SVec<Region> regions) {
   const int lane = wave_lane();
-  Study& st = fr.study;
+  EMAT_FRAME_AS Study& st = fr.study;
   if (lane == 0) {
     st.regions = regions; st.lambda_X = fr.lambda_X; st.f = fr.f; st.t_X = fr.t_X; st.t_max_tip = fr.t_max_tip; st.log_Wmax = 0.0; st.sum_W = 0.0;
     st.mu = fr.lambda_X / (c.L - fr.n_missing_at_X);
@@ -1249,7 +1252,7 @@
 };
 static_assert(sizeof(ScanItem) == 32, "ScanItem must be two 16-byte groups");
 
-EMAT_D bool wave_local_scan(Ctx& c, Spr1Frame& fr) {
+EMAT_D bool wave_local_scan(Ctx& c, EMAT_FRAME_AS Spr1Frame& fr) {
   const int lane = wave_lane();
   const uint64_t below = lane == 0 ? 0ull : (~0ull >> (64 - lane));
   const int X = fr.X, root = hdr_of(c)->root;
@@ -1378,7 +1381,7 @@
     __syncthreads();
   }
   const int V = items[0].sz;
-  SVec<Region>* shared = &fr.study.regions;
+  EMAT_FRAME_AS SVec<Region>* shared = &fr.study.regions;
   if (lane == 0) {
     SVec<Region> r; r.n = 0; r.cap = 0; r.p = nullptr;
     if (hbm_lo != nullptr) {
@@ -1435,8 +1438,9 @@
   }
   __syncthreads();
   if (lane == 0) {
-    shared->n = w;
-    sc_trim(c, *shared);
+    SVec<Region> r = *shared; r.n = w;
+    sc_trim(c, r);
+    *shared = r;
     c.bytes += (int64_t)(64 + 16) * V;
   }
   __syncthreads();
@@ -1444,9 +1448,9 @@
 }
 
 EMAT_DN void wave_scan_and_study(Ctx& c) {
-  Spr1Frame& fr = *(Spr1Frame*)c.frame;
+  EMAT_FRAME_AS Spr1Frame& fr = frame_of<Spr1Frame>(c);
   const int lane = wave_lane();
-  SVec<Region>* shared = &fr.study.regions;
+  EMAT_FRAME_AS SVec<Region>* shared = &fr.study.regions;
 #ifdef EMAT_PROFILE_PHASES
   const long long ph0 = clock64();
 #endif
diff --git a/delphy_amd/csrc/emat_part_kernels.hpp b/delphy_amd/csrc/emat_part_kernels.hpp
--- a/delphy_amd/csrc/emat_part_kernels.hpp
+++ b/delphy_amd/csrc/emat_part_kernels.hpp
@@ -114,6 +114,33 @@
 #endif
 #define EMAT_OCCUPANCY __attribute__((amdgpu_waves_per_eu(EMAT_WAVES_PER_EU, EMAT_WAVES_PER_EU)))
 constexpr uint32_t k_lds_heap_room = 1024;
+constexpr uint32_t k_frame_bytes = dev_lds::k_frame_bytes;
+static_assert(dev_mix::k_frame_bytes == k_frame_bytes && dev::k_frame_bytes == k_frame_bytes && k_frame_bytes % 16 == 0, "one frame slot for the three code variants, in 16-byte units");
+constexpr uint32_t k_lds_heap_floor = 512;
+static_assert(k_frame_bytes + k_lds_heap_floor <= k_lds_heap_room, "a part that fits the area with its heap room must hold the frame slot");
+struct LegPlan { uint32_t lds_heap_end, used; bool staged, prefix; };
+__host__ __device__ inline LegPlan plan_leg(bool can_stage, bool allow_whole, uint32_t heap_begin, uint32_t heap_top, uint32_t heap_end, uint32_t area, uint32_t extra_arena) {
+  LegPlan p; p.lds_heap_end = 0; p.used = 0; p.staged = false; p.prefix = false;
+  if (!can_stage) return p;
+  if (allow_whole) {
+    const uint32_t want = (heap_top + k_lds_heap_room + 15u) & ~15u;
+    uint32_t end = 0;
+    if (heap_end <= area) end = heap_end < want ? heap_end : want;
+    else if (want <= area) end = want;
+    if (end != 0) {
+      uint32_t used = (end + 15u) & ~15u;
+      const uint32_t left = area + extra_arena - used;
+      if (left < k_frame_bytes) {
+        const uint32_t lack = k_frame_bytes - left;
+        if (used >= lack && used - lack >= ((heap_top + k_lds_heap_floor + 15u) & ~15u)) { used -= lack; end = used; } else end = 0;
+      }
+      if (end != 0) { p.lds_heap_end = end; p.used = used; p.staged = true; return p; }
+    }
+  }
+  const uint32_t used = (heap_begin + 15u) & ~15u;
+  if (heap_begin <= area && area + extra_arena - used >= k_frame_bytes) { p.used = used; p.prefix = true; }
+  return p;
+}
 
 __device__ __forceinline__ int xcc_id() { return (int)(__builtin_amdgcn_s_getreg(20 | (0 << 6) | ((4 - 1) << 11)) & 15u); }
 __global__ void k_probe_xcc(int32_t* out) { if (threadIdx.x == 0) out[blockIdx.x] = xcc_id(); }
@@ -180,15 +207,11 @@
   for (int leg = 0; leg < 2; ++leg) {
     __syncthreads();
     const uint32_t hbm_heap_end = gh->heap_end;
-    uint32_t lds_heap_end = 0;
-    if (can_stage && allow_whole) {
-      const uint32_t want = (gh->heap_top + k_lds_heap_room + 15u) & ~15u;
-      if (hbm_heap_end <= area) lds_heap_end = hbm_heap_end < want ? hbm_heap_end : want;
-      else if (want <= area) lds_heap_end = want;
-    }
-    const bool staged = lds_heap_end != 0;
+    const LegPlan plan = plan_leg(can_stage, allow_whole, gh->heap_begin, gh->heap_top, hbm_heap_end, area, a.lds_scratch_bytes);
+    const uint32_t lds_heap_end = plan.lds_heap_end;
+    const bool staged = plan.staged;
     if (!staged) plain_hbm_writes = true;
-    const bool prefix = can_stage && !staged && gh->heap_begin <= area;
+    const bool prefix = plan.prefix;
     const uint32_t staged_bytes = staged ? gh->heap_top : (prefix ? gh->heap_begin : 0u);
     if (staged_bytes) { wave_copy16(emat_lds_hdr, gslab, (uint32_t)sizeof(SlabHeader), lane); wave_copy16(lds_slab, gslab + sizeof(SlabHeader), staged_bytes - (uint32_t)sizeof(SlabHeader), lane); }
     uint8_t* const snap = (!staged && a.snaps != nullptr) ? a.snaps + a.slab_off[part] : nullptr;
@@ -204,14 +227,14 @@
         init_ctx(c, gslab, gslab, a, lds_tables, lds_hdr);
         H->heap_end = lds_heap_end;
         dev_lds::begin_leg(c);
-        const uint32_t used = (lds_heap_end + 15u) & ~15u;
-        c.A = lds_slab + (used - (uint32_t)sizeof(SlabHeader)); c.a_end = area + a.lds_scratch_bytes - used;
+        c.frame = lds_slab + (plan.used - (uint32_t)sizeof(SlabHeader));
+        c.A = c.frame + k_frame_bytes; c.a_end = area + a.lds_scratch_bytes - plan.used - k_frame_bytes;
       } else if (prefix) {
         dev_mix::Ctx& c = *(dev_mix::Ctx*)(emat_lds_ctx);
         init_ctx(c, gslab, gslab, a, lds_tables, lds_hdr);
         dev_mix::begin_leg(c);
-        const uint32_t used = (gh->heap_begin + 15u) & ~15u;
-        c.A = lds_slab + (used - (uint32_t)sizeof(SlabHeader)); c.a_end = area + a.lds_scratch_bytes - used;
+        c.frame = lds_slab + (plan.used - (uint32_t)sizeof(SlabHeader));
+        c.A = c.frame + k_frame_bytes; c.a_end = area + a.lds_scratch_bytes - plan.used - k_frame_bytes;
       } else {
         dev::Ctx& c = *(dev::Ctx*)(emat_lds_ctx);
         init_ctx(c, gslab, gslab, a, tables_staged ? lds_tables : nullptr);
```

New measurement: 543.7 million moves/s (median of 6 runs). No clear change (+0.9%).
